# CarbonMatrixLab/AbX

Hardware: AMD Instinct MI355X
Metric: diffusion-steps/sec (100 samples, ~350-res complex) (higher is better)
Workload: dtype f32; 1 GPU; L352: L=352 (Lab 228 + antigen 124), 100 samples of one complex over 1 GPU(s), 1 step = ScoreNetwork (3 passes) + get_prev + reverse, seeded random weights, ESM off; L=352, samples_total=100, chunk=auto, parallelism=sample-shard x1, no collective in the step

## Files before the change

abx_amd/_lib.py:

```python
import ctypes as C
import os

_HERE = os.path.dirname(os.path.abspath(__file__))
LIB_PATH = os.environ.get('ABX_HIP_LIB') or os.path.join(_HERE, 'csrc', 'libabx_hip.so')

c_f = C.c_void_p
LL = C.c_longlong
I = C.c_int
F = C.c_float


class AbxGemm(C.Structure):
    _fields_ = [
        ('A', c_f), ('sAb', LL), ('sAm', LL), ('sAk', LL),
        ('B', c_f), ('sBb', LL), ('sBk', LL), ('sBn', LL),
        ('C', c_f), ('sCb', LL), ('sCm', LL),
        ('M', I), ('N', I), ('K', I), ('batch', I),
        ('c_transposed', I),
        ('ln_stats', c_f), ('sSb', LL),
        ('ln_csum', c_f),
        ('ln_eps', F),
        ('a_relu', I),
        ('bias', c_f),
        ('alpha', F),
        ('act', I),
        ('rowscale', c_f), ('sRSb', LL),
        ('gate', c_f), ('sGb', LL), ('sGm', LL), ('gate_sigmoid', I),
        ('resid', c_f), ('sRb', LL), ('sRm', LL),
        ('B_split', C.c_void_p), ('sB3p', LL), ('sB3n', LL), ('sB3k', LL), ('sB3b', LL),
        ('A_split', C.c_void_p), ('sA3p', LL), ('sA3m', LL), ('sA3k', LL), ('sA3b', LL),
        ('batch_inner', I), ('sA3i', LL), ('sB3i', LL),
        ('c_split_tile', I),
        ('c_split_nA', I),
        ('C_split', C.c_void_p), ('sCp', LL), ('sCk', LL), ('c_split_L', I),
        ('glu', I),
        ('a_pair_transpose', I),
        ('pair_L', I), ('pair_Lp', I), ('a_pair', I), ('c_pair', I),
        ('A2', c_f), ('sA2b', LL), ('sA2m', LL), ('K2', I),
        ('B2_split', C.c_void_p), ('sB23p', LL), ('sB23n', LL), ('sB23k', LL),
        ('ln2_csum', c_f), ('bias2', c_f),
        ('mlp', I), ('N2', I),
        ('out_ln_w', c_f), ('out_ln_b', c_f), ('out_ln_eps', F),
        ('exact', I),
        ('b_f16', I), ('b_exp', I), ('b2_exp', I),
        ('tune', I),
        ('c_planes_from', I), ('c_planes_group', I),
        ('range_flag', c_f), ('range_tag', I),
        ('clock_probe', c_f),
        ('a_vec_ok', I), ('b_vec_ok', I), ('fast_ok', I),
        ('c_vec_ok', I), ('g_vec_ok', I), ('r_vec_ok', I), ('rs_vec_ok', I),
    ]


class AbxIpaTail(C.Structure):
    _fields_ = [
        ('feat', c_f), ('s_feat', LL),
        ('s', c_f), ('s_s', LL),
        ('M', I), ('K1', I), ('C', I),
        ('W_final', C.c_void_p), ('e_final', I), ('b_final', c_f),
        ('ln1_w', c_f), ('ln1_b', c_f),
        ('W_t0', C.c_void_p), ('e_t0', I), ('b_t0', c_f),
        ('W_t2', C.c_void_p), ('e_t2', I), ('b_t2', c_f),
        ('W_t4', C.c_void_p), ('e_t4', I), ('b_t4', c_f),
        ('ln2_w', c_f), ('ln2_b', c_f),
        ('ln_eps', F),
        ('W_aff', c_f), ('b_aff', c_f),
        ('fixed', c_f), ('init_q', c_f), ('init_t', c_f),
        ('cur_q', c_f), ('cur_t', c_f), ('cur_R', c_f), ('delta_q', c_f), ('pscale', F),
        ('range_flag', c_f), ('range_tag', I),
        ('partial', c_f), ('n_partial', I), ('s_partial', LL),
    ]


class AbxHeadsTail(C.Structure):
    _fields_ = [
        ('s', c_f), ('s_s', LL), ('s0', c_f), ('s_s0', LL), ('M', I),
        ('W_act', C.c_void_p), ('e_act', I), ('b_act', c_f),
        ('W_init', C.c_void_p), ('e_init', I), ('b_init', c_f),
        ('W_r0', C.c_void_p), ('e_r0', I), ('b_r0', c_f),
        ('W_r1', C.c_void_p), ('e_r1', I), ('b_r1', c_f),
        ('W_r2', C.c_void_p), ('e_r2', I), ('b_r2', c_f),
        ('W_r3', C.c_void_p), ('e_r3', I), ('b_r3', c_f),
        ('W_proj', C.c_void_p), ('e_proj', I), ('b_proj', c_f),
        ('un', c_f),
        ('lns_w', c_f), ('lns_b', c_f),
        ('W_s1', C.c_void_p), ('e_s1', I), ('b_s1', c_f),
        ('W_s3', C.c_void_p), ('e_s3', I), ('b_s3', c_f),
        ('W_s5', C.c_void_p), ('e_s5', I), ('b_s5', c_f),
        ('logits', c_f),
        ('lnp_w', c_f), ('lnp_b', c_f),
        ('W_p1', C.c_void_p), ('e_p1', I), ('b_p1', c_f),
        ('W_p3', C.c_void_p), ('e_p3', I), ('b_p3', c_f),
        ('W_p5', C.c_void_p), ('e_p5', I), ('b_p5', c_f),
        ('pl', c_f),
        ('ln_eps', F),
        ('range_flag', c_f), ('range_tag', I),
    ]


class AbxTriAttn(C.Structure):
    _fields_ = [
        ('q', c_f), ('k', c_f), ('v', c_f), ('gate', c_f),
        ('sb', LL), ('ss', LL), ('sl', LL),
# ... 180 lines not shown
    'abx_tri_rowpack_bytes': (LL, []),
    'abx_tri_rowpack': (I, [C.POINTER(AbxLinearPack), c_f, C.POINTER(AbxTriRowPack), _S]),
    'abx_tri_attn_rowfused_ok': (I, [I]),
    'abx_tri_attn_rowfused_fwd': (I, [C.POINTER(AbxTriAttn), c_f, LL, LL, LL, C.POINTER(AbxTriRowPack), I, _S]),
    'abx_seq_attn_fwd': (I, [c_f, c_f, c_f, c_f, c_f, I, I, I, I, F, _S]),
    'abx_ipa_pack': (I, [c_f, c_f, c_f, c_f, c_f, c_f, I, I, F, _S]),
    'abx_ipa_attn': (I, [c_f, c_f, c_f, c_f, c_f, c_f, c_f, c_f, c_f, c_f, c_f, I, I, _S]),
    'abx_debug_poison_lds': (I, [C.c_uint, _S]),
    'abx_ipa_weights': (I, [c_f, c_f, c_f, c_f, c_f, c_f, c_f, c_f, c_f, c_f, I, I, _S]),
    'abx_ipa_pair': (I, [c_f, c_f, c_f, I, I, _S]),
    'abx_ipa_attn_workspace_bytes': (C.c_longlong, [I, I]),
    'abx_ipa_qpack_bytes': (C.c_longlong, [I, I]),
    'abx_timestep_embedding': (I, [c_f, c_f, I, I, c_f, _S]),
    'abx_assemble_seq': (I, [c_f, LL, c_f, c_f, I, c_f, c_f, c_f, c_f, c_f, I, I, I, I, _S]),
    'abx_assemble_pair': (I, [c_f, LL, c_f, c_f, c_f, c_f, c_f, c_f, c_f, c_f, I, I, I, I, _S]),
    'abx_opm_features': (I, [c_f, c_f, LL, c_f, I, I, I, _S]),
    'abx_opm_out_fwd': (I, [c_f, LL, c_f, c_f, c_f, I, I, c_f, I, _S]),
    'abx_assemble_pair_bias': (I, [c_f, LL, c_f, c_f, c_f, c_f, c_f, c_f, c_f, C.c_void_p, I, c_f, c_f, F, c_f, I, I, c_f, I, _S]),
    'abx_pair_mask': (I, [c_f, c_f, I, I, I, _S]),
    'abx_transpose_last2': (I, [c_f, c_f, I, I, I, I, _S]),
    'abx_pair_embed_features': (I, [c_f, c_f, c_f, c_f, c_f, c_f, c_f, c_f, c_f, c_f, c_f, c_f, I, I, _S]),
    'abx_relpos_block': (I, [c_f, c_f, c_f, I, I, I, I, I, _S]),
    'abx_gather_rows': (I, [c_f, c_f, c_f, c_f, LL, LL, I, _S]),
    'abx_frames_init': (I, [c_f, I, c_f, c_f, c_f, c_f, c_f, c_f, I, F, _S]),
    'abx_rigid_update': (I, [c_f, c_f, c_f, c_f, c_f, c_f, c_f, c_f, I, F, _S]),
    'abx_scores': (I, [C.POINTER(AbxScoreArgs), _S]),
    'abx_torsion_finalize': (I, [c_f, c_f, c_f, c_f, I, _S]),
    'abx_seq_head_atoms': (I, [c_f, c_f, c_f, c_f, c_f, c_f, c_f, c_f, c_f, c_f, c_f, c_f, I, _S]),
    'abx_prev_pos': (I, [c_f, c_f, I, c_f, I, I, _S]),
    'abx_plddt': (I, [c_f, c_f, I, I, _S]),
    'abx_igso3_tables': (I, [c_f, c_f, I, I, I, c_f, c_f, c_f, _S]),
    'abx_reverse_step': (I, [C.POINTER(AbxReverseArgs), _S]),
    'abx_clash_grad_workspace_bytes': (LL, [I, I]),
    'abx_clash_grad': (I, [C.POINTER(AbxGuidanceArgs), c_f, _S]),
    'abx_design_scores_workspace_bytes': (LL, [I, I]),
    'abx_design_scores': (I, [C.POINTER(AbxDesignScoreArgs), c_f, _S]),
    'abx_relax_workspace_bytes': (LL, [I, I, I]),
    'abx_relax_lds_bytes': (LL, [I, I]),
    'abx_relax': (I, [C.POINTER(AbxRelaxArgs), c_f, _S]),
    'abx_interface_scores_workspace_bytes': (LL, [I, I, I]),
    'abx_interface_scores': (I, [C.POINTER(AbxInterfaceArgs), c_f, _S]),
    'abx_ensemble_pairs_workspace_bytes': (LL, [I, I]),
    'abx_ensemble_pairs': (I, [C.POINTER(AbxEnsemblePairsArgs), c_f, _S]),
    'abx_ensemble_cluster': (I, [C.POINTER(AbxEnsembleClusterArgs), _S]),
    'abx_pack_linear_bytes': (LL, [I, I]),
    'abx_pack_linear': (I, [C.POINTER(AbxLinearSrc), I, I, c_f, c_f, I, c_f, C.POINTER(AbxLinearPack), _S]),
    'abx_transition_workspace_bytes': (LL, [LL, I, I]),
    'abx_transition_fwd': (I, [C.POINTER(AbxLinearPack), C.POINTER(AbxLinearPack), c_f, LL, I, c_f, c_f, I, _S]),
    'abx_tri_mul_workspace_bytes': (LL, [I, I]),
    'abx_tri_mul_workspace_init': (I, [c_f, I, I, _S]),
    'abx_tri_mul_fwd': (I, [C.POINTER(AbxTriMulPack), c_f, c_f, c_f, I, I, I, c_f, c_f, I, _S]),
    'abx_tri_attn_block_workspace_bytes': (LL, [I, I]),
    'abx_tri_attn_block_fwd': (I, [C.POINTER(AbxTriAttnPack), c_f, c_f, I, I, I, I, c_f, c_f, I, _S]),
}

EXPORTED = tuple(_PROTOS)
_lib = None


class AbxHipError(RuntimeError):
    pass


def library_path():
    return LIB_PATH


def load():
    global _lib
    if _lib is not None:
        return _lib
    if not os.path.exists(LIB_PATH):
        raise AbxHipError(f'{LIB_PATH} not found: build it with `make -C abx_amd/csrc` (no CPU fallback exists)')
    lib = C.CDLL(LIB_PATH)
    for name, (res, args) in _PROTOS.items():
        fn = getattr(lib, name)
        fn.restype = res
        fn.argtypes = args
    if lib.abx_version() != 1:
        raise AbxHipError('libabx_hip ABI version mismatch')
    _lib = lib
    return lib


def check(rc, what):
    if rc != 0:
        msg = load().abx_last_error_string()
        raise AbxHipError(f'{what} failed (rc={rc}): {msg.decode() if msg else ""}')
```

abx_amd/csrc/blocks.hip:

```cpp
#include <math.h>
#include <string.h>

#include <stdlib.h>

#include "common.h"
#include "abx_hip.h"

namespace {

constexpr long long ALIGN = 256;
inline long long up(long long x) { return (x + ALIGN - 1) / ALIGN * ALIGN; }

__global__ void pack_rows_kernel(const float* __restrict__ W, const float* __restrict__ b, int rows, int K, int c0, int glu,
                                 float* __restrict__ Wcat, float* __restrict__ bcat) {
    const long long idx = (long long)blockIdx.x * blockDim.x + threadIdx.x;
    if (idx >= (long long)rows * K) return;
    const int r = (int)(idx / K), k = (int)(idx - (long long)r * K);
    const int c = c0 + r;
    const int dst = glu ? (c / 32) * 64 + (glu == 2 ? 32 : 0) + c % 32 : c;
    Wcat[(long long)dst * K + k] = W[idx];
    if (k == 0) bcat[dst] = b ? b[r] : 0.f;
}

__global__ void fold_kernel(const float* __restrict__ Wcat, const float* __restrict__ bcat, const float* __restrict__ gamma,
                            const float* __restrict__ beta, int N, int K, float* __restrict__ Wt, float* __restrict__ csum,
                            float* __restrict__ bias, unsigned* __restrict__ amax) {
    const int n = blockIdx.x * blockDim.x + threadIdx.x;
    if (n >= N) return;
    double cs = 0.0, bs = 0.0;
    float mx = 0.f;
    bool bad = false;
    for (int k = 0; k < K; ++k) {
        const double w = (double)Wcat[(long long)n * K + k];
        const double ws = gamma ? (double)gamma[k] * w : w;
        const float wf = (float)ws;
        Wt[(long long)k * N + n] = wf;
        cs += ws;
        if (beta) bs += (double)beta[k] * w;
        mx = fmaxf(mx, fabsf(wf));
        bad |= !(fabsf(wf) <= 3.0e38f);
    }
    csum[n] = (float)cs;
    bias[n] = (float)(bs + (double)bcat[n]);
    atomicMax(amax, bad ? 0x7f800000u : __float_as_uint(mx));
}

__global__ void permute_k16_kernel(const float* __restrict__ Wt, int K, int N, float* __restrict__ out) {
    const long long idx = (long long)blockIdx.x * blockDim.x + threadIdx.x;
    if (idx >= (long long)K * N) return;
    const int k = (int)(idx / N), n = (int)(idx - (long long)k * N);
    const int j = k & 15;
    const int src = (k & ~15) | ((j & 3) | ((j & 4) << 1) | ((j & 8) >> 1));
    out[idx] = Wt[(long long)src * N + n];
}

inline void set_weights(AbxGemm& g, const AbxLinearPack& p, bool ln, int exact) {
    g.B = p.Wt; g.sBb = 0; g.sBk = p.N; g.sBn = 1;
    g.N = p.N; g.K = p.K;
    g.bias = p.bias;
    if (ln) { g.ln_csum = p.csum; g.ln_eps = 1e-5f; }
    g.B_split = p.planes; g.sB3k = 2LL * p.N * 16; g.sB3p = (long long)p.N * 16; g.sB3n = 16; g.sB3b = 0;
    g.b_f16 = 1; g.b_exp = p.b_exp;
    g.exact = exact ? 1 : 2;
    g.alpha = 1.0f;
}
inline void set_range(AbxGemm& g, int* flag, int tag, int exact) {
    if (!exact) { g.range_flag = flag; g.range_tag = tag; }
}

}

extern "C" long long abx_pack_linear_bytes(int K, int N) {
    if (K <= 0 || N <= 0) return -1;
    const long long Kp = (K + 15) / 16 * 16;
    return up(4LL * K * N) + 2 * up(4LL * N) + up(2LL * Kp * 2 * N) + up(4LL * K * N) + up(4LL * N) + up(4);
}

extern "C" int abx_pack_linear(const AbxLinearSrc* src, int nsrc, int K, const float* gamma, const float* beta, int flags, void* buf,
                               AbxLinearPack* out, hipStream_t st) {
    ABX_REQUIRE(src && nsrc > 0 && nsrc <= 8 && K > 0 && buf && out, "abx_pack_linear: bad args");
    ABX_REQUIRE((reinterpret_cast<uintptr_t>(buf) & (ALIGN - 1)) == 0, "abx_pack_linear: buf must be 256-byte aligned");
    ABX_REQUIRE((gamma == nullptr) == (beta == nullptr), "abx_pack_linear: gamma and beta come together");
    int N = 0, nv = 0, ng = 0;
    bool any_b = false;
    for (int i = 0; i < nsrc; ++i) {
        ABX_REQUIRE(src[i].W && src[i].rows > 0 && src[i].glu >= 0 && src[i].glu <= 2, "abx_pack_linear: bad source");
        N += src[i].rows;
        nv += src[i].glu == 1 ? src[i].rows : 0;
        ng += src[i].glu == 2 ? src[i].rows : 0;
        any_b |= src[i].b != nullptr;
    }
    ABX_REQUIRE((nv == 0 && ng == 0) || (nv == ng && nv + ng == N && nv % 32 == 0),
                "abx_pack_linear: glu sources need as many value as gate rows, in multiples of 32, and nothing else");
    ABX_REQUIRE(!(flags & ABX_PACK_PERMUTE_K16) || K % 16 == 0, "abx_pack_linear: ABX_PACK_PERMUTE_K16 needs K % 16 == 0");
    const long long Kp = (K + 15) / 16 * 16;
    char* p = static_cast<char*>(buf);
    float* Wt = reinterpret_cast<float*>(p); p += up(4LL * K * N);
    float* csum = reinterpret_cast<float*>(p); p += up(4LL * N);
    float* bias = reinterpret_cast<float*>(p); p += up(4LL * N);
    unsigned short* planes = reinterpret_cast<unsigned short*>(p); p += up(2LL * Kp * 2 * N);
    float* Wcat = reinterpret_cast<float*>(p); p += up(4LL * K * N);
    float* bcat = reinterpret_cast<float*>(p); p += up(4LL * N);
    unsigned* amax = reinterpret_cast<unsigned*>(p);
    int cv = 0, cg = 0, c0 = 0;
    for (int i = 0; i < nsrc; ++i) {
        const long long tot = (long long)src[i].rows * K;
        const int base = src[i].glu == 1 ? cv : (src[i].glu == 2 ? cg : c0);
        hipLaunchKernelGGL(pack_rows_kernel, dim3((unsigned)((tot + 255) / 256)), dim3(256), 0, st, src[i].W, src[i].b, src[i].rows, K, base,
                           src[i].glu, Wcat, bcat);
        (src[i].glu == 1 ? cv : (src[i].glu == 2 ? cg : c0)) += src[i].rows;
    }
    if (hipMemsetAsync(amax, 0, 4, st) != hipSuccess) { abx_set_error("abx_pack_linear: memset failed"); return ABX_ERR_ARG; }
    hipLaunchKernelGGL(fold_kernel, dim3((N + 63) / 64), dim3(64), 0, st, Wcat, bcat, gamma, beta, N, K, Wt, csum, bias, amax);
    if (int rc = abx_check_launch("abx_pack_linear")) return rc;
    unsigned bits = 0;
    if (hipMemcpyAsync(&bits, amax, 4, hipMemcpyDeviceToHost, st) != hipSuccess || hipStreamSynchronize(st) != hipSuccess) {
        abx_set_error("abx_pack_linear: reading max |w| failed");
        return ABX_ERR_ARG;
    }
    float mx;
    memcpy(&mx, &bits, 4);
// ... 38 lines not shown
        g.mlp = 1; g.N2 = C; g.b2_exp = l2->b_exp;
        g.B2_split = l2->planes; g.sB23k = 2LL * C * 16; g.sB23p = (long long)C * 16; g.sB23n = 16;
        g.bias2 = l2->bias;
        g.resid = z; g.sRm = C;
        set_range(g, range_flag, range_tag, 0);
        return abx_gemm(&g, st);
    }
    ABX_REQUIRE(workspace, "abx_transition_fwd: the exact path needs its workspace (abx_transition_workspace_bytes)");
    float* hid = static_cast<float*>(workspace);
    AbxGemm g = {};
    g.A = z; g.sAm = C; g.sAk = 1;
    g.C = hid; g.sCm = Hd;
    g.M = (int)M; g.batch = 1;
    set_weights(g, *l1, true, 1);
    g.act = 1;
    if (int rc = abx_gemm(&g, st)) return rc;
    AbxGemm h = {};
    h.A = hid; h.sAm = Hd; h.sAk = 1;
    h.C = z; h.sCm = C;
    h.M = (int)M; h.batch = 1;
    set_weights(h, *l2, false, 1);
    h.B_split = nullptr; h.b_f16 = 0;
    h.resid = z; h.sRm = C;
    return abx_gemm(&h, st);
}

namespace {
struct TriMulWs { unsigned short* lrp; float* pm; float* tt; long long lrp_bytes; };
inline TriMulWs tri_mul_ws(void* ws, int B, int L) {
    const long long Lp = (L + 3) / 4 * 4, KT = (Lp + 15) / 16;
    TriMulWs w;
    char* p = static_cast<char*>(ws);
    w.lrp_bytes = 2LL * B * 256 * KT * 2 * L * 16;
    w.lrp = reinterpret_cast<unsigned short*>(p); p += up(w.lrp_bytes);
    w.pm = reinterpret_cast<float*>(p); p += up(4LL * B * L * Lp);
    w.tt = reinterpret_cast<float*>(p);
    return w;
}
}

extern "C" long long abx_tri_mul_workspace_bytes(int B, int L) {
    if (B <= 0 || L <= 0) return -1;
    const long long Lp = (L + 3) / 4 * 4, KT = (Lp + 15) / 16;
    return up(2LL * B * 256 * KT * 2 * L * 16) + up(4LL * B * L * Lp) + up(4LL * B * 128 * L * Lp);
}

extern "C" int abx_tri_mul_workspace_init(void* workspace, int B, int L, hipStream_t st) {
    ABX_REQUIRE(workspace && B > 0 && L > 0, "abx_tri_mul_workspace_init: bad args");
    const TriMulWs w = tri_mul_ws(workspace, B, L);
    if (hipMemsetAsync(w.lrp, 0, (size_t)w.lrp_bytes, st) != hipSuccess) { abx_set_error("abx_tri_mul_workspace_init: memset failed"); return ABX_ERR_ARG; }
    return ABX_OK;
}

extern "C" int abx_tri_mul_fwd(const AbxTriMulPack* wp, const float* z_in, float* z_out, const float* mask, int B, int L, int outgoing,
                               void* workspace, int* range_flag, int range_tag, hipStream_t st) {
    ABX_REQUIRE(wp && z_in && z_out && z_in != z_out && mask && workspace && B > 0 && L > 0, "abx_tri_mul_fwd: bad args (z_out must not alias z_in)");
    const AbxLinearPack &glu = wp->glu, &out = wp->out, &gate = wp->gate;
    ABX_REQUIRE(glu.csum && out.csum && gate.csum && glu.N == 512 && out.K == 128 && gate.K == glu.K && out.N == gate.N && glu.K == out.N,
                "abx_tri_mul_fwd: packs: glu = LN-folded C -> 2 x 256 (value, gate) pairs, out = LN-folded 128 -> C, gate = LN-folded C -> C");
    const int C = glu.K;
    const long long LL = (long long)L * L;
    const int Lp = (L + 3) / 4 * 4, KT = (Lp + 15) / 16;
    const long long LLp = (long long)L * Lp;
    const TriMulWs w = tri_mul_ws(workspace, B, L);
    if (int rc = abx_pair_mask(mask, w.pm, B, L, Lp, st)) return rc;
    {
        AbxGemm g = {};
        g.A = z_in; g.sAb = LL * C; g.sAm = C; g.sAk = 1;
        g.M = (int)(((long long)(L + 7) / 8 * 8) * ((long long)(Lp + 15) / 16 * 16));
        g.batch = B;
        set_weights(g, glu, true, 0);
        g.C_split = w.lrp; g.sCb = 256LL * KT * 2 * L * 16; g.sCm = (long long)KT * 2 * L * 16; g.sCk = 2LL * L * 16; g.sCp = (long long)L * 16;
        g.c_split_L = Lp; g.c_transposed = 1; g.c_split_nA = 128; g.c_split_tile = 1;
        g.pair_L = L; g.pair_Lp = Lp; g.a_pair = 1; g.a_pair_transpose = outgoing ? 0 : L;
        g.glu = 1;
        g.rowscale = w.pm; g.sRSb = LLp;
        set_range(g, range_flag, range_tag, 0);
        if (int rc = abx_gemm(&g, st)) return rc;
    }
    {
        AbxGemm g = {};
        const long long per_ch = (long long)KT * 2 * L * 16;
        g.A_split = w.lrp; g.sA3b = 256 * per_ch; g.sA3i = per_ch; g.sA3k = 2LL * L * 16; g.sA3p = (long long)L * 16; g.sA3m = 16;
        g.B_split = w.lrp + 128 * per_ch; g.sB3b = 256 * per_ch; g.sB3i = per_ch; g.sB3k = 2LL * L * 16; g.sB3p = (long long)L * 16; g.sB3n = 16;
        g.batch_inner = 128;
        g.C = w.tt; g.sCb = LLp; g.sCm = Lp;
        g.M = L; g.N = L; g.K = KT * 16; g.batch = B * 128;
        g.exact = 2; g.alpha = 1.0f;
        set_range(g, range_flag, range_tag, 0);
        if (int rc = abx_gemm(&g, st)) return rc;
    }
    {
        AbxGemm g = {};
        g.A = w.tt; g.sAb = 128 * LLp; g.sAm = 1; g.sAk = LLp;
        g.M = (int)LLp; g.batch = B;
        set_weights(g, out, true, 0);
        g.C = z_out; g.sCb = LL * C; g.sCm = C;
        if (Lp != L) { g.pair_L = L; g.pair_Lp = Lp; g.c_pair = 1; }
        g.A2 = z_in; g.sA2b = LL * C; g.sA2m = C; g.K2 = C;
        g.B2_split = gate.planes; g.sB23k = 2LL * gate.N * 16; g.sB23p = (long long)gate.N * 16; g.sB23n = 16; g.b2_exp = gate.b_exp;
        g.ln2_csum = gate.csum; g.bias2 = gate.bias;
        g.resid = z_in; g.sRb = LL * C; g.sRm = C;
        set_range(g, range_flag, range_tag, 0);
        return abx_gemm(&g, st);
    }
}

namespace {
struct TriAttnWs { float* qkv; float* hid; float* bT; float* bT2; float* o; };
inline TriAttnWs tri_attn_ws(void* ws, int B, int L) {
    const long long LL = (long long)L * L, Lp = (L + 3) / 4 * 4;
    TriAttnWs w;
    char* p = static_cast<char*>(ws);
    w.qkv = reinterpret_cast<float*>(p);
    w.hid = w.qkv + (long long)B * LL * 576;
    p += up(4LL * B * LL * 768);
    w.bT = reinterpret_cast<float*>(p); p += up(4LL * B * 4 * LL);
    w.bT2 = reinterpret_cast<float*>(p); p += up(4LL * B * 4 * L * Lp);
    w.o = reinterpret_cast<float*>(p);
    return w;
}
}

extern "C" long long abx_tri_attn_block_workspace_bytes(int B, int L) {
    if (B <= 0 || L <= 0) return -1;
    const long long LL = (long long)L * L, Lp = (L + 3) / 4 * 4;
    return up(4LL * B * LL * 768) + up(4LL * B * 4 * LL) + up(4LL * B * 4 * L * Lp) + up(4LL * B * LL * 192);
}

extern "C" int abx_tri_attn_block_fwd(const AbxTriAttnPack* wp, float* z, const float* mask, int B, int L, int per_row, int exact,
                                      void* workspace, int* range_flag, int range_tag, hipStream_t st) {
    ABX_REQUIRE(wp && z && mask && workspace && B > 0 && L > 0, "abx_tri_attn_block_fwd: bad args");
    const AbxLinearPack &qkv = wp->qkv, &gate = wp->gate, &pair = wp->pair, &out = wp->out;
    ABX_REQUIRE(qkv.csum && gate.csum && pair.csum && qkv.N == 576 && gate.N == 192 && pair.N == 4 && qkv.K == 192 && gate.K == 192 && pair.K == 192 &&
                    out.K == 192 && out.N == 192,
                "abx_tri_attn_block_fwd: packs: qkv = LN-folded 192 -> 576, gate = LN-folded 192 -> 192, pair = LN-folded 192 -> 4, out = 192 -> 192 "
                "(ABX_PACK_PERMUTE_K16)");
    const long long LL = (long long)L * L, M2 = (long long)B * LL;
    ABX_REQUIRE(M2 < (1LL << 31), "abx_tri_attn_block_fwd: too many pair rows for one launch");
    ABX_REQUIRE(exact >= 0 && exact <= 3, "abx_tri_attn_block_fwd: exact is a 2-bit field");
    const int attn_exact = (exact >> 1) & 1;
    exact &= 1;
    const int Lp = (L + 3) / 4 * 4, C = 192;
    const TriAttnWs w = tri_attn_ws(workspace, B, L);
    static const bool kv_planes_on = getenv("ABX_KV_PLANES") != nullptr;
    const int planes = (kv_planes_on && !exact && !attn_exact && abx_gemm_planes_ok(M2)) ? 1 : 0;
    const bool rowfused = !exact && !attn_exact && !planes && wp->row.planes && abx_tri_attn_rowfused_ok(L);
    if (rowfused) {
        AbxGemm s2 = {};
        s2.A = z; s2.sAb = LL * C; s2.sAm = C; s2.sAk = 1;
        s2.C = w.bT; s2.sCb = 4 * LL; s2.sCm = LL; s2.c_transposed = 1;
        s2.M = (int)LL; s2.batch = B;
        set_weights(s2, pair, true, 0);
        set_range(s2, range_flag, range_tag, 0);
        s2.alpha = ABX_TRI_BIAS_LOG2;
        if (int rc = abx_gemm(&s2, st)) return rc;
    } else {
        AbxGemm g = {};
        g.A = z; g.sAm = C; g.sAk = 1;
        g.C = w.qkv; g.sCm = 576;
        g.M = (int)M2; g.batch = 1;
        set_weights(g, qkv, true, exact);
        set_range(g, range_flag, range_tag, exact);
        if (planes) { g.c_planes_from = 192; g.c_planes_group = 48; }
        AbxGemm s2 = {};
        s2.A = z; s2.sAb = LL * C; s2.sAm = C; s2.sAk = 1;
        s2.C = w.bT; s2.sCb = 4 * LL; s2.sCm = LL; s2.c_transposed = 1;
        s2.M = (int)LL; s2.batch = B;
        set_weights(s2, pair, true, exact);
        set_range(s2, range_flag, range_tag, exact);
        if (!attn_exact) s2.alpha = ABX_TRI_BIAS_LOG2;
        if (int rc = abx_gemm_side(&g, &s2, st)) return rc;
    }
    const float* bias = w.bT;
    if (!per_row || Lp != L) {
        if (int rc = abx_transpose_last2(w.bT, w.bT2, B * 4, L, Lp, per_row ? 0 : 1, st)) return rc;
        bias = w.bT2;
    }
    {
        AbxTriAttn a = {};
        a.q = w.qkv; a.k = w.qkv + 192; a.v = w.qkv + 384; a.gate = nullptr;
        a.sb = LL * 576;
        a.ss = per_row ? (long long)L * 576 : 576;
        a.sl = per_row ? 576 : (long long)L * 576;
        a.bias = bias; a.bias_sb = 4LL * L * Lp; a.bias_sh = (long long)L * Lp; a.bias_sq = Lp; a.bias_sk = 1;
        a.keymask = mask; a.km_sb = L;
        a.out = w.o; a.ob = LL * C;
        a.os = per_row ? (long long)L * C : C;
        a.ol = per_row ? C : (long long)L * C;
        a.B = B; a.S = L; a.L = L; a.H = 4; a.D = 48;
        a.scale = 0.14433756729740643f;
        a.exact = attn_exact;
        a.bias_log2 = attn_exact ? 0 : 1;
        a.kv_planes = planes;
        if (!attn_exact) { a.range_flag = range_flag; a.range_tag = range_tag; }
        if (rowfused) {
            if (int rc = abx_tri_attn_rowfused_fwd(&a, z, LL * C, per_row ? (long long)L * C : C, per_row ? C : (long long)L * C, &wp->row, -1, st)) return rc;
        } else if (int rc = abx_tri_attn_fwd(&a, st)) return rc;
    }
    if (!exact) {
        AbxGemm g = {};
        g.A = z; g.sAm = C; g.sAk = 1;
        g.C = z; g.sCm = C;
        g.M = (int)M2; g.batch = 1;
        set_weights(g, gate, true, 0);
        g.act = 2;
        g.gate = w.o; g.sGm = C;
        g.mlp = 2; g.N2 = C; g.b2_exp = out.b_exp;
        g.B2_split = out.planes; g.sB23k = 2LL * C * 16; g.sB23p = (long long)C * 16; g.sB23n = 16;
        g.bias2 = out.bias;
        g.resid = z; g.sRm = C;
        set_range(g, range_flag, range_tag, 0);
        return abx_gemm(&g, st);
    }
    {
        AbxGemm g = {};
        g.A = z; g.sAm = C; g.sAk = 1;
        g.C = w.hid; g.sCm = C;
        g.M = (int)M2; g.batch = 1;
        set_weights(g, gate, true, 1);
        g.act = 2;
        g.gate = w.o; g.sGm = C; g.gate_sigmoid = 0;
        if (int rc = abx_gemm(&g, st)) return rc;
    }
    {
        AbxGemm g = {};
        g.A = w.hid; g.sAm = C; g.sAk = 1;
        g.C = z; g.sCm = C;
        g.M = (int)M2; g.batch = 1;
        set_weights(g, out, false, 1);
        g.B_split = nullptr; g.b_f16 = 0;
        g.resid = z; g.sRm = C;
        return abx_gemm(&g, st);
    }
}
```

abx_amd/csrc/gemm.hip:

```cpp
#include <stdlib.h>
#include "common.h"
#include "abx_hip.h"
#include "gemm_epilogue.h"

int abx_gemm3_dispatch(const AbxGemm& g, hipStream_t st, int* rc);

namespace {

template <int BMN, int BK, bool KC, bool EDGE>
struct TileLoader {
    static constexpr int NVEC = BMN * BK / 4;
    static constexpr int NV = (NVEC + 255) / 256;
    static constexpr int LD = BMN + 4;
    f32x4 v[NV];

    __device__ __forceinline__ void load(const float* __restrict__ base, long long s_mn, long long s_k, int mn0, int k0,
                                         int MN, int K, bool vec_ok) {
        const int tid = threadIdx.x;
#pragma unroll
        for (int i = 0; i < NV; ++i) {
            const int idx = tid + i * 256;
            f32x4 r = {0.f, 0.f, 0.f, 0.f};
            if (NVEC % 256 == 0 || idx < NVEC) {
                if (KC) {
// ... 397 lines not shown
    ABX_REQUIRE(!on[A_SPLIT] || (!g.ln_csum && !g.a_relu), "abx_gemm: a_split (plane x plane contraction) takes no LayerNorm and no relu-on-load");
    return ABX_OK;
}

static int gemm_prepare(const AbxGemm* gp, AbxGemm& g) {
    if (int rc = abx_gemm_check_modes(gp)) return rc;
    g = *gp;
    ABX_REQUIRE((g.A || g.A_split) && (g.B || g.B_split) && (g.C || g.C_split), "abx_gemm: null operand");
    ABX_REQUIRE(!g.glu || (g.c_transposed && g.N % 128 == 0 && !g.gate), "abx_gemm: glu needs a transposed store, N % 128 == 0, no gate");
    const long long tile_rows = ((long long)(g.pair_L + 7) / 8 * 8) * ((long long)(g.pair_Lp + 15) / 16 * 16);
    ABX_REQUIRE(!g.c_split_tile || (g.C_split && g.a_pair && g.pair_Lp > 0 && g.M == tile_rows && !g.gate && !g.resid),
                "abx_gemm: c_split_tile needs C_split, a_pair, pair_L / pair_Lp, M == ceil8(pair_L) * ceil16(pair_Lp), no gate / resid");
    ABX_REQUIRE(!g.C_split || (g.c_transposed && g.c_split_L > 0 && g.c_split_L % 4 == 0 && (g.c_split_tile || g.M % g.c_split_L == 0)),
                "abx_gemm: C_split needs the transposed store of a (padded) pair tensor (M = rows * c_split_L, c_split_L % 4 == 0)");
    ABX_REQUIRE(g.M > 0 && g.N > 0 && g.K > 0 && g.batch > 0, "abx_gemm: empty problem");
    ABX_REQUIRE(g.pair_Lp == 0 || (g.pair_L > 0 && g.pair_Lp >= g.pair_L && g.pair_Lp % 4 == 0 &&
                                   (g.c_split_tile || g.M == (long long)g.pair_L * g.pair_Lp) && (!g.C_split || g.c_split_L == g.pair_Lp)),
                "abx_gemm: padded pair rows need M == pair_L * pair_Lp, pair_Lp % 4 == 0 (and c_split_L == pair_Lp)");
    ABX_REQUIRE((!g.a_pair && !g.c_pair) || g.pair_Lp > 0, "abx_gemm: a_pair / c_pair need pair_L / pair_Lp");
    ABX_REQUIRE(!g.A || g.sAk == 1 || g.sAm == 1, "abx_gemm: A must be k- or m-contiguous");
    ABX_REQUIRE(!g.B || g.sBn == 1 || g.sBk == 1, "abx_gemm: B must be n- or k-contiguous");
    ABX_REQUIRE(!g.ln_stats || g.ln_csum, "abx_gemm: LayerNorm needs the column sums of the gamma-scaled weights");
    ABX_REQUIRE(!(g.ln_csum && g.a_relu), "abx_gemm: LayerNorm and relu-on-load are exclusive");
    if (g.ln_csum && !g.ln_stats && g.ln_eps <= 0.f) g.ln_eps = 1e-5f;
    if (g.out_ln_w && g.out_ln_eps <= 0.f) g.out_ln_eps = 1e-5f;
    const bool akc = g.sAk == 1;
    auto al16 = [](const void* p) { return (reinterpret_cast<uintptr_t>(p) & 15) == 0; };
    g.a_vec_ok = al16(g.A) && (g.sAb % 4 == 0) && (akc ? (g.sAm % 4 == 0) : (g.sAk % 4 == 0));
    g.b_vec_ok = al16(g.B) && (g.sBb % 4 == 0) && (g.sBn == 1 ? (g.sBk % 4 == 0) : (g.sBn % 4 == 0));
    g.fast_ok = g.a_vec_ok && g.b_vec_ok;
    g.c_vec_ok = g.C_split ? ((reinterpret_cast<uintptr_t>(g.C_split) & 7) == 0 && g.sCb % 4 == 0 && g.sCm % 4 == 0 && g.sCp % 4 == 0)
                           : (al16(g.C) && (g.sCb % 4 == 0) && (g.sCm % 4 == 0));
    g.g_vec_ok = g.gate && al16(g.gate) && (g.sGb % 4 == 0) && (g.sGm % 4 == 0);
    g.r_vec_ok = g.resid && al16(g.resid) && (g.sRb % 4 == 0) && (g.sRm % 4 == 0);
    g.rs_vec_ok = g.rowscale && al16(g.rowscale) && (g.sRSb % 4 == 0);
    ABX_REQUIRE(g.c_planes_from == 0 || (g.c_planes_from > 0 && g.c_planes_from % 4 == 0 && g.c_planes_group > 0 && g.c_planes_group % 4 == 0 &&
                                         g.N % 4 == 0 && g.c_planes_from < g.N && (g.N - g.c_planes_from) % g.c_planes_group == 0 && g.C && g.c_vec_ok &&
                                         !g.c_transposed && !g.C_split && !g.glu && !g.gate && !g.resid && !g.mlp && !g.A2 && !g.out_ln_w && !g.c_pair &&
                                         g.act == 0 && g.exact != 1),
                "abx_gemm: c_planes_from needs a plain, 16-byte aligned fp32 store without gate / resid / activation on the split-f16 path, from, "
                "group and N multiples of 4, (N - from) % group == 0");
    return ABX_OK;
}

int abx_gemm3_side_dispatch(const AbxGemm& g, const AbxGemm& s2, hipStream_t st, int* rc);
int abx_gemm_as_dispatch(const AbxGemm& g, const AbxGemm* side, hipStream_t st, int* rc);

extern "C" int abx_gemm_planes_ok(long long M) {
    static const bool off = getenv("ABX_NO_GEMM_AS") != nullptr || getenv("ABX_NO_GEMM_SIDE") != nullptr;
    return (!off && (M + 63) / 64 >= 1024) ? 1 : 0;
}

extern "C" int abx_gemm_side(const AbxGemm* main_gemm, const AbxGemm* side_gemm, hipStream_t st) {
    ABX_REQUIRE(main_gemm && side_gemm, "abx_gemm_side: null descriptor");
    AbxGemm g, s2;
    if (int rc = gemm_prepare(main_gemm, g)) return rc;
    if (int rc = gemm_prepare(side_gemm, s2)) return rc;
    int rc = 0;
    static const bool off = getenv("ABX_NO_GEMM_SIDE") != nullptr;
    if (!off && !abx_gemm_as_dispatch(g, &s2, st, &rc)) return rc;
    ABX_REQUIRE(g.c_planes_from == 0, "abx_gemm_side: c_planes_from is served by the A-stationary kernel only (>= 65 536 rows, K = 192, N % 128 == 64, "
                                      "planes in groups of 48 from a multiple of 32, a side projection): ask abx_gemm_planes_ok first");
    if (!off && !abx_gemm3_side_dispatch(g, s2, st, &rc)) return rc;
    if (int r1 = abx_gemm(main_gemm, st)) return r1;
    return abx_gemm(side_gemm, st);
}

extern "C" int abx_gemm(const AbxGemm* gp, hipStream_t st) {
    AbxGemm g;
    if (int rc = gemm_prepare(gp, g)) return rc;
    ABX_REQUIRE(g.c_planes_from == 0, "abx_gemm: c_planes_from is served through abx_gemm_side by the A-stationary kernel only (abx_gemm_planes_ok)");
    auto al16 = [](const void* p) { return (reinterpret_cast<uintptr_t>(p) & 15) == 0; };
    (void)al16;
    const bool akc = g.sAk == 1;
    if (g.exact != 1) {
        int rc = 0;
        if (!abx_gemm_as_dispatch(g, nullptr, st, &rc)) return rc;
        if (!abx_gemm3_dispatch(g, st, &rc)) return rc;
    }
    g.range_flag = nullptr;
    ABX_REQUIRE(g.A && g.B, "abx_gemm: split-f16 operands given but the problem does not qualify for the split kernels "
                            "(K % 16, alignment, size) and no fp32 operands were passed for the exact kernel");
    ABX_REQUIRE(g.a_pair_transpose <= 0 && g.pair_Lp == 0, "abx_gemm: pair-row remapping is served by the split-f16 kernels only");
    ABX_REQUIRE(g.batch <= 65535, "abx_gemm: batch > 65535 (exact fp32 kernels)");
    ABX_REQUIRE(!g.glu, "abx_gemm: glu is served by the split-f16 kernels only (large problems, K % 16 == 0)");
    ABX_REQUIRE(!g.A2, "abx_gemm: the dual GEMM is served by the split-f16 kernels only");
    ABX_REQUIRE(!g.out_ln_w, "abx_gemm: out_ln is served by the split-f16 kernels only");
    ABX_REQUIRE(!g.mlp, "abx_gemm: the fused transition (mlp) is served by the split-f16 kernels only (exact = 2, K % 16 == 0)");
    const long long mt128 = ((long long)g.M + 127) / 128;
    if (g.N <= 32) return launch_cfg<128, 32, 32, 32>(g, st);
    if (g.N <= 64) return launch_cfg<128, 64, 32, 64>(g, st);
    if (mt128 * (((long long)g.N + 127) / 128) * g.batch < 512) return launch_cfg<64, 64, 32, 32>(g, st);
    if (g.tune >> 1) {
        ABX_REQUIRE(!g.c_transposed && akc && g.sBn == 1, "abx_gemm: tuning variants exist for the plain weight GEMM only");
        switch (g.tune >> 1) {
            case 1: return launch_main_variant<16, 2>(g, st);
            case 2: return launch_main_variant<16, 4>(g, st);
            case 3: return launch_cfg<128, 128, 64, 64, 16, 3>(g, st);
            default: break;
        }
    }
    const long long pad128 = ((g.N + 127) / 128) * 128, pad192 = ((g.N + 191) / 192) * 192;
    if (pad192 <= pad128 && !(g.tune >> 1)) return launch_cfg<128, 192, 64, 96, 16, 2>(g, st);
    return launch_cfg<128, 128, 64, 64>(g, st);
}

extern "C" int abx_row_stats(const float* x, long long s_b, long long s_row, long long s_k, int batch, int rows, int K,
                             float eps, float* stats, hipStream_t st) {
    ABX_REQUIRE(x && stats && rows > 0 && K > 0 && batch > 0, "abx_row_stats: bad args");
    if (s_k == 1) {
        ABX_REQUIRE(batch == 1 || s_b == (long long)rows * s_row, "abx_row_stats: k-contiguous rows must be dense over batch");
        const long long total = (long long)batch * rows;
        hipLaunchKernelGGL(row_stats_kc, dim3((unsigned)((total + 3) / 4)), dim3(256), 0, st, x, s_row, (int)total, K, eps, stats);
    } else {
        ABX_REQUIRE(s_row == 1, "abx_row_stats: rows must be contiguous when k is strided");
        hipLaunchKernelGGL(row_stats_mc, dim3((unsigned)((rows + 255) / 256), (unsigned)batch), dim3(256), 0, st, x, s_b, s_k,
                           rows, K, eps, stats);
    }
    return abx_check_launch("abx_row_stats");
}

extern "C" int abx_layernorm(const float* x, long long s_row, long long rows, int K, const float* gamma, const float* beta,
                             float eps, float* out, long long s_out, const float* res, long long s_res, hipStream_t st) {
    ABX_REQUIRE(x && out && gamma && beta && rows > 0 && K > 0, "abx_layernorm: bad args");
    auto al16v = [](const void* p) { return (reinterpret_cast<uintptr_t>(p) & 15) == 0; };
    if (K == 128 && s_row % 4 == 0 && s_out % 4 == 0 && al16v(x) && al16v(out) && al16v(gamma) && al16v(beta) &&
        (!res || (al16v(res) && s_res % 4 == 0))) {
// ... 9 lines not shown
```

abx_amd/csrc/gemm3.hip:

```cpp
#include "common.h"
#include "abx_hip.h"
#include "gemm_epilogue.h"
#include "rigid_dev.h"

namespace {

constexpr int BK = 16;
#ifndef ABX_SPLIT_MIN_TILES
#define ABX_SPLIT_MIN_TILES 256
#endif
typedef __attribute__((address_space(3))) void* lds_ptr_t;
typedef const __attribute__((address_space(1))) void* glb_ptr_t;

__device__ __forceinline__ void glds16(const void* src, char* dst_wave_base) {
    __builtin_amdgcn_global_load_lds((glb_ptr_t)src, (lds_ptr_t)dst_wave_base, 16, 0, 0);
}

__device__ __forceinline__ unsigned vgpr32(unsigned o) {
    asm volatile("" : "+v"(o));
    return o;
}

template <int N> __device__ __forceinline__ void wait_vm_and_barrier() {
    asm volatile("s_waitcnt vmcnt(%0) lgkmcnt(0)\n\ts_barrier" ::"n"(N) : "memory");
// ... 750 lines not shown
                }
                const char* ws = W2s + (kg & 1) * B2_IMG + offB2;
                if (rows_live && kg * 16 < g.N) {
#pragma unroll
                    for (int t0 = 0; t0 < TN2; t0 += TG2) {
                        u32x4 wb[TG2][2];
#pragma unroll
                        for (int t = 0; t < TG2; ++t)
#pragma unroll
                            for (int p = 0; p < 2; ++p) wb[t][p] = *reinterpret_cast<const u32x4*>(ws + (t0 + t) * 1024 + p * (BN2 * 32));
                        constexpr int TA[3] = {1, 0, 0}, TB[3] = {0, 1, 0};
#pragma unroll
                        for (int term = 0; term < 3; ++term)
#pragma unroll
                            for (int t = 0; t < TG2; ++t)
                                acc2[0][t0 + t] = mfma_split(hf[TA[term]], wb[t][TB[term]], acc2[0][t0 + t]);
                    }
                }
                if (kl + 1 < KC && (kg + 1) * 16 < g.N) wait_vm_and_barrier<2>();
                else wait_vm_and_barrier<0>();
            }
        }
    }
    {
        const float cs2 = __builtin_ldexpf(1.0f, -4 - g.b2_exp);
#pragma unroll
        for (int t = 0; t < TN2; ++t) acc2[0][t] *= cs2;
    }
    AbxGemm g2 = g;
    g2.N = g.N2; g2.bias = g.bias2; g2.ln_csum = nullptr; g2.ln_stats = nullptr; g2.act = 0; g2.alpha = 1.0f; g2.gate = nullptr;
    __syncthreads();
    gemm_epilogue<BM, BN2, WM, BN2, EDGE, false>(g2, smem, smem + 2 * BM, acc2, mt * BM, 0, b, false);
}

constexpr int GT_LDS = 2 * 128 * 64 + 2 * 2 * 96 * 32 + 2 * 2 * 192 * 32 + 3 * 128 * 64 + 2 * GT_NG * 4;

__global__ __launch_bounds__(256, 2) void gemm3_gtail2w_kernel(const AbxGemm g) {
    extern __shared__ __attribute__((aligned(16))) float gt_smem[];
    const int ntm = (g.M + 127) / 128;
    const unsigned nwg = gridDim.x, bid = blockIdx.x;
    const unsigned q = nwg >> 3, r = nwg & 7, xcd = bid & 7, loc = bid >> 3;
    const unsigned wgid = (xcd < r ? xcd * (q + 1) : r * (q + 1) + (xcd - r) * q) + loc;
    const int b = (int)(wgid / (unsigned)ntm), mt = (int)(wgid - (unsigned)b * (unsigned)ntm);
    const ClockProbe probe(g.clock_probe);
    if ((mt + 1) * 128 <= g.M && g.N2 == 192) gemm3_gtail2w_block<false>(g, gt_smem, mt, b);
    else gemm3_gtail2w_block<true>(g, gt_smem, mt, b);
    probe.finish();
}

constexpr int GT1_G1 = 2 * 128 * 64 + 2 * 2 * 192 * 32;
constexpr int GT1_W2 = 2 * 96 * 32;
constexpr int GT1_OFF_G = GT1_G1, GT1_OFF_W2 = GT1_OFF_G + 3 * 128 * 64, GT1_OFF_CST = GT1_OFF_W2 + 2 * GT1_W2;
constexpr int GT1_LDS = GT1_OFF_CST + 2 * GT_NG * 4;
template <bool EDGE>
__device__ __forceinline__ void gemm3_gtail_block(const AbxGemm& g, float* smem, int mt, int b) {
    constexpr int BM = 128, BN = 192, WM = 32, BH = 96, TH = BH / 32, NKT = BN / 16;
    char* lds = reinterpret_cast<char*>(smem);
    char* Gs = lds + GT1_OFF_G;
    char* W2s = lds + GT1_OFF_W2;
    float* cst = reinterpret_cast<float*>(lds + GT1_OFF_CST);
    for (int i = threadIdx.x; i < GT_NG; i += 256) {
        cst[i] = i < g.N ? g.ln_csum[i] : 0.f;
        cst[GT_NG + i] = (i < g.N && g.bias) ? g.bias[i] : 0.f;
    }
    const int lane = threadIdx.x & 63, wave = __builtin_amdgcn_readfirstlane(threadIdx.x >> 6), h = lane >> 5;
    const int m0 = mt * BM;
    unsigned offs2[2][2];
#pragma unroll
    for (int half = 0; half < 2; ++half) plane_sources<BH, 2>(g.sB23p, g.sB23n, half * BH, g.N2, offs2[half]);
    const char* base2 = reinterpret_cast<const char*>(g.B2_split);
    const long long step2 = g.sB23k * 2;
    auto issue_w2 = [&](int half, int ktile) {
        if (wave == 3) return;
        char* dst = W2s + (ktile & 1) * GT1_W2 + wave * 2048;
        const char* src = base2 + ktile * step2;
#pragma unroll
        for (int i = 0; i < 2; ++i) glds16(src + vgpr32(offs2[half][i]), dst + i * 1024);
    };
    unsigned offsG[2];
    const char* baseG = reinterpret_cast<const char*>(g.gate + (long long)b * g.sGb + (long long)m0 * g.sGm);
#pragma unroll
    for (int i = 0; i < 2; ++i) {
        const int r = (wave * 2 + i) * 16 + (lane >> 2), p = lane & 3;
        const int kq = p ^ ((r >> 2) & 3);
        const int gri = min(m0 + r, g.M - 1) - m0;
        offsG[i] = (unsigned)(((long long)gri * g.sGm + kq * 4) * 4);
    }
    const int nkt2 = g.N / 16;
    auto issue_g = [&](int ktile) {
        const int kt = min(ktile, nkt2 - 1);
        char* dg = Gs + (ktile % 3) * (BM * 64) + wave * 2048;
        const char* sg = baseG + kt * 64;
#pragma unroll
        for (int i = 0; i < 2; ++i) glds16(sg + vgpr32(offsG[i]), dg + i * 1024);
    };
    const int offB2 = plane_off<BH>(0, lane & 31, h);
    const int grow = wave * WM + (lane & 31), gx = (grow >> 2) & 3;
    const int offG0 = grow * 64 + ((h ^ gx) << 4), offG1 = grow * 64 + (((2 + h) ^ gx) << 4);
    const bool rows_live = m0 + wave * WM < g.M;

    issue_w2(0, 0);
    issue_g(0);
    issue_g(1);
    float ls[1], lq[1], lsh[1] = {0.f};
    f32x16 acc1[1][BN / 32];
    gemm3_mainloop<BM, BN, WM, BN, 0, true, true>(g, smem, mt, 0, b, acc1, ls, lq, lsh);
    const float invK = 1.0f / (float)g.K;
    const float sm = ls[0] + __shfl_xor(ls[0], 32, 64), sq = lq[0] + __shfl_xor(lq[0], 32, 64);
    const float dmean = sm * invK;
    const float rstd = 1.0f / sqrtf(fmaxf(sq * invK - dmean * dmean, 0.f) + g.ln_eps);

    AbxGemm g2 = g;
    g2.N = g.N2; g2.bias = g.bias2; g2.ln_csum = nullptr; g2.ln_stats = nullptr; g2.act = 0; g2.alpha = 1.0f; g2.gate = nullptr;
    const float cs2 = __builtin_ldexpf(1.0f, -4 - g.b2_exp);
    u32x4 hfa[NKT][2];
    constexpr int TA[3] = {1, 0, 0}, TB[3] = {0, 1, 0};
#pragma unroll
    for (int half = 0; half < 2; ++half) {
        f32x16 acc2[1][TH];
#pragma unroll
        for (int t = 0; t < TH; ++t)
#pragma unroll
            for (int r = 0; r < 16; ++r) acc2[0][t][r] = 0.f;
        if (half == 1) issue_w2(1, 0);
#pragma unroll
        for (int kg = 0; kg < NKT; ++kg) {
            const bool more = (kg + 1) * 16 < g.N && kg + 1 < NKT;
            if (half == 1 && kg == 0) wait_vm_and_barrier<0>();
            if (more) {
                issue_w2(half, kg + 1);
                if (half == 0) issue_g(kg + 2);
            }
            if (half == 0) {
                const int j = kg >> 1, s2 = kg & 1;
                const char* gs = Gs + (kg % 3) * (BM * 64);
                const f32x4 o0 = *reinterpret_cast<const f32x4*>(gs + offG0), o1 = *reinterpret_cast<const f32x4*>(gs + offG1);
                float v[8];
#pragma unroll
                for (int q = 0; q < 2; ++q) {
                    const int hc = j * 32 + 8 * (2 * s2 + q) + 4 * h;
                    const int hcl = min(hc, GT_NG - 4);
                    const f32x4 cs = *reinterpret_cast<const f32x4*>(cst + hcl), bi = *reinterpret_cast<const f32x4*>(cst + GT_NG + hcl);
                    const f32x4 ov = q ? o1 : o0;
#pragma unroll
                    for (int e = 0; e < 4; ++e) {
                        const float x = rstd * (acc1[0][j][8 * s2 + 4 * q + e] - dmean * cs[e]) + bi[e];
                        v[4 * q + e] = (hc + e < g.N) ? ov[e] * sigmoidf_(x) : 0.f;
                    }
                }
                unsigned q0[4], q1[4];
#pragma unroll
                for (int e = 0; e < 4; ++e) split2b(v[2 * e], v[2 * e + 1], q0[e], q1[e]);
                hfa[kg][0] = u32x4{q0[0], q0[1], q0[2], q0[3]};
                hfa[kg][1] = u32x4{q1[0], q1[1], q1[2], q1[3]};
            }
            const char* ws = W2s + (kg & 1) * GT1_W2 + offB2;
            if (rows_live && kg * 16 < g.N) {
                u32x4 wb[TH][2];
#pragma unroll
                for (int t = 0; t < TH; ++t)
#pragma unroll
                    for (int p = 0; p < 2; ++p) wb[t][p] = *reinterpret_cast<const u32x4*>(ws + t * 1024 + p * (BH * 32));
#pragma unroll
                for (int term = 0; term < 3; ++term)
#pragma unroll
                    for (int t = 0; t < TH; ++t) acc2[0][t] = mfma_split(hfa[kg][TA[term]], wb[t][TB[term]], acc2[0][t]);
            }
            if (more && half == 0) wait_vm_and_barrier<2>();
            else wait_vm_and_barrier<0>();
        }
#pragma unroll
        for (int t = 0; t < TH; ++t) acc2[0][t] *= cs2;
        gemm_epilogue<BM, BH, WM, BH, EDGE, false>(g2, smem, smem + 2 * BM, acc2, m0, half * BH, b, false);
        if (half == 0) __syncthreads();
    }
}

__global__ __launch_bounds__(256, 2) void gemm3_gtail_kernel(const AbxGemm g) {
    extern __shared__ __attribute__((aligned(16))) float gt_smem[];
    const int ntm = (g.M + 127) / 128;
    const unsigned nwg = gridDim.x, bid = blockIdx.x;
    const unsigned q = nwg >> 3, r = nwg & 7, xcd = bid & 7, loc = bid >> 3;
    const unsigned wgid = (xcd < r ? xcd * (q + 1) : r * (q + 1) + (xcd - r) * q) + loc;
    const int b = (int)(wgid / (unsigned)ntm), mt = (int)(wgid - (unsigned)b * (unsigned)ntm);
    const ClockProbe probe(g.clock_probe);
    if ((mt + 1) * 128 <= g.M && g.N2 == 192 && g.N == 192) gemm3_gtail_block<false>(g, gt_smem, mt, b);
    else gemm3_gtail_block<true>(g, gt_smem, mt, b);
    probe.finish();
}

constexpr int IT_C = 256;
constexpr int IT_ASTR = IT_C * 4 + 16;
constexpr int IT_RING = 4;
constexpr int IT_OPER = IT_RING * (4096 + 2 * IT_C * 32);
constexpr int IT_LDS = IT_OPER + 2 * 32 * IT_ASTR + 2 * 4 * 32 * 4;

__global__ __launch_bounds__(256, 1) void ipa_tail_kernel(const AbxIpaTail a) {
    constexpr int BM = 32, BN = IT_C, WM = 32, WN = 64, TN = 2;
    extern __shared__ __attribute__((aligned(16))) float it_smem[];
    char* lds = reinterpret_cast<char*>(it_smem);
    char* act[2] = {lds + IT_OPER, lds + IT_OPER + 32 * IT_ASTR};
    float* red = reinterpret_cast<float*>(lds + IT_OPER + 2 * 32 * IT_ASTR);
    const int mt = blockIdx.x, m0 = mt * BM;
    const int lane = threadIdx.x & 63, wave = threadIdx.x >> 6, h = lane >> 5, row = lane & 31;
    const int grc = min(m0 + row, a.M - 1);
    const int colb = wave * WN + 4 * h;

    AbxGemm g = {};
    g.M = a.M; g.N = IT_C; g.batch = 1; g.b_f16 = 1;
    g.sB3k = 2 * IT_C * 16; g.sB3p = IT_C * 16; g.sB3n = 16;
    f32x16 acc[1][TN];
    float ls[1], lq[1], lsh[1];
    float x[TN][16];

    auto for_groups = [&](auto&& fn) {
#pragma unroll
        for (int j = 0; j < TN; ++j)
#pragma unroll
            for (int q = 0; q < 4; ++q) fn(j, q, colb + j * 32 + 8 * q);
    };
    auto layer_norm = [&](const float* gamma, const float* beta) {
        float sm = 0.f;
#pragma unroll
        for (int j = 0; j < TN; ++j)
#pragma unroll
            for (int r = 0; r < 16; ++r) sm += x[j][r];
        sm += __shfl_xor(sm, 32, 64);
        if (h == 0) red[wave * 32 + row] = sm;
// ... 232 lines not shown
            bias_to(br[2 * blk + 1], false, true, x);
            to_lds(T1, HT_HSTR, x);
            __syncthreads();
        }
    }
    run(a.W_proj, a.e_proj, HT_H, T1, HT_HSTR, 1);
    bias_to(a.b_proj, false, false, y);
    store_cols(a.un, 14, y);
    layer_norm_s(a.lns_w, a.lns_b);
    __syncthreads();
    head(a.W_s1, a.e_s1, a.b_s1, a.W_s3, a.e_s3, a.b_s3, a.W_s5, a.e_s5, a.b_s5, a.logits, 20);
    if (a.W_p1) {
        layer_norm_s(a.lnp_w, a.lnp_b);
        __syncthreads();
        head(a.W_p1, a.e_p1, a.b_p1, a.W_p3, a.e_p3, a.b_p3, a.W_p5, a.e_p5, a.b_p5, a.pl, 50);
    }
    if (a.range_flag && __any(bad) && lane == 0) atomicOr(a.range_flag, a.range_tag);
}

template <int BM, int BN, int WM, int WN, int MINW>
int launch3(const AbxGemm& g, hipStream_t st) {
    const long long mt = ((long long)g.M + BM - 1) / BM, ntn = ((long long)g.N + BN - 1) / BN;
    dim3 grid((unsigned)(mt * ntn * g.batch), 1, 1), block(256);
#ifdef ABX_PERSIST
    if ((g.tune & 256) && grid.x > 256u * MINW) grid.x = 256u * MINW;
#endif
    const int amode = g.A_split ? 2 : (g.sAk == 1 ? 0 : 1);
    if (g.c_transposed) {
        if (amode != 0) { abx_set_error("abx_gemm: transposed store needs a k-contiguous fp32 A"); return ABX_ERR_ARG; }
        hipLaunchKernelGGL((gemm3_kernel<BM, BN, WM, WN, 0, true, MINW>), grid, block, 0, st, g);
    } else if (amode == 0) hipLaunchKernelGGL((gemm3_kernel<BM, BN, WM, WN, 0, false, MINW>), grid, block, 0, st, g);
    else if (amode == 1) hipLaunchKernelGGL((gemm3_kernel<BM, BN, WM, WN, 1, false, MINW>), grid, block, 0, st, g);
    else hipLaunchKernelGGL((gemm3_kernel<BM, BN, WM, WN, 2, false, MINW>), grid, block, 0, st, g);
    return abx_check_launch("abx_gemm");
}

__global__ __launch_bounds__(256) void split_weights_f16_kernel(const float* __restrict__ w, long long s_n, long long s_k, int N, int K,
                                                                int Kp, float scale, unsigned short* __restrict__ out) {
    const long long idx = (long long)blockIdx.x * 256 + threadIdx.x;
    if (idx >= (long long)N * Kp) return;
    const int n = (int)(idx / Kp), k = (int)(idx % Kp);
    const float x = k < K ? w[n * s_n + k * s_k] * scale : 0.f;
    const _Float16 h0 = (_Float16)x;
    const _Float16 h1 = (_Float16)(x - (float)h0);
    const long long o = ((long long)(k >> 4) * 2 * N + n) * 16 + (k & 15);
    out[o] = __builtin_bit_cast(unsigned short, h0);
    out[o + (long long)N * 16] = __builtin_bit_cast(unsigned short, h1);
}

}

int abx_gemm3_dispatch(const AbxGemm& g, hipStream_t st, int* rc) {
    auto al16 = [](const void* p) { return (reinterpret_cast<uintptr_t>(p) & 15) == 0; };
    const bool narrow = g.B_split && g.N <= 32 && !g.A_split && g.sAk == 1 && !g.glu && !g.C_split && !g.A2 && !g.out_ln_w &&
                        g.a_pair_transpose <= 0 && g.pair_Lp == 0;
    if (!g.B_split || g.K % 16 != 0 || (g.N <= 64 && !narrow)) return 1;
    if ((g.A_split != nullptr) == (g.b_f16 != 0) || g.b_exp < -100 || g.b_exp > 100 || g.b2_exp < -100 || g.b2_exp > 100) {
        abx_set_error("abx_gemm: B_split must be float16 weight planes (abx_split_weights_f16, b_f16 = 1, |b_exp| <= 100) with an fp32 A "
                      "and activation images (b_f16 = 0) with A_split");
        *rc = ABX_ERR_ARG;
        return 0;
    }
    const long long mt128 = ((long long)g.M + 127) / 128;
    if (g.exact != 2 && mt128 * (((long long)g.N + 127) / 128) * g.batch < ABX_SPLIT_MIN_TILES) return 1;
    if (!al16(g.B_split) || g.sB3n % 8 != 0 || g.sB3p % 8 != 0 || g.sB3b % 8 != 0 || g.sB3k % 8 != 0) return 1;
    if (g.A_split) {
        if (!al16(g.A_split) || g.sA3m % 8 != 0 || g.sA3p % 8 != 0 || g.sA3b % 8 != 0 || g.sA3k % 8 != 0 || g.c_transposed) return 1;
        if (g.batch_inner > 0 && (g.sA3i % 8 != 0 || g.sB3i % 8 != 0)) return 1;
    } else if (g.sAk == 1) {
        if (!al16(g.A) || g.sAm % 4 != 0 || g.sAb % 4 != 0) return 1;
        if (g.a_pair_transpose > 0 && !g.a_pair && (long long)g.a_pair_transpose * g.a_pair_transpose != g.M) return 1;
    } else {
        if (!al16(g.A) || g.sAk % 4 != 0 || g.sAb % 4 != 0 || g.M % 4 != 0 || g.M < 4 || g.a_pair_transpose > 0) return 1;
    }
    if (!g.A_split && g.sAk == 1 && ((g.a_pair_transpose > 0 || g.a_pair) ? (long long)g.M * g.sAm : 128LL * g.sAm) >= (1LL << 30)) return 1;
    if (g.pair_Lp > 0 && g.c_pair && g.c_transposed) return 1;
    if (g.a_pair && (g.A_split || g.sAk != 1)) return 1;
    if (!g.A_split && g.sAk != 1 && 16LL * g.sAk + g.M >= (1LL << 30)) return 1;
    if (((long long)g.M + 127) / 128 * (((long long)g.N + 127) / 128) * g.batch >= (1LL << 31)) return 1;
    if (g.A_split && (long long)(g.K / 16) * g.sA3k >= (1LL << 31)) return 1;
    if ((long long)(g.K / 16) * g.sB3k >= (1LL << 31)) return 1;
    if (g.out_ln_w) {
        if (g.N > 128 || g.c_transposed || g.C_split || g.A2 || g.A_split || g.sAk != 1 || !g.out_ln_b) {
            abx_set_error("abx_gemm: out_ln needs N <= 128, a k-contiguous fp32 A and a plain store (split-f16 path)");
            *rc = ABX_ERR_ARG;
            return 0;
        }
        const long long mt = ((long long)g.M + 127) / 128;
        hipLaunchKernelGGL((gemm3_oln_kernel<128, 128, 32, 128, 4>), dim3((unsigned)(mt * g.batch)), dim3(256), 0, st, g);
        *rc = abx_check_launch("abx_gemm(out_ln)");
        return 0;
    }
    if (g.mlp == 2) {
        if (g.A_split || g.sAk != 1 || g.c_transposed || g.C_split || g.glu || g.A2 || g.out_ln_w || !g.B2_split || g.N2 <= 0 || g.N2 > 192 ||
            g.N % 16 != 0 || g.N > GT_NG || g.act != 2 || g.alpha != 1.0f || g.rowscale || !g.gate || !g.ln_csum || g.ln_stats || g.a_relu ||
            g.a_pair_transpose > 0 || g.pair_Lp > 0 || !al16(g.B2_split) || g.sB23n % 8 != 0 || g.sB23p % 8 != 0 || g.sB23k % 8 != 0 ||
            (long long)(g.N / 16) * g.sB23k >= (1LL << 31) || !al16(g.ln_csum) || (g.bias && !al16(g.bias)) || !al16(g.gate) || g.sGm % 4 != 0 ||
            g.sGb % 4 != 0 || 128LL * g.sGm >= (1LL << 30)) {
            abx_set_error("abx_gemm: mlp = 2 (gated tail) needs a k-contiguous fp32 A with folded LayerNorm, act = 2, a 16-byte aligned gate "
                          "operand [M][N], N % 16 == 0, N2 <= 192, plain store, B2_split planes in the permuted k order");
            *rc = ABX_ERR_ARG;
            return 0;
        }
        const long long mt = ((long long)g.M + 127) / 128;
        if (g.tune & 64) {
            if (int e = abx_ensure_dynamic_lds(reinterpret_cast<const void*>(&gemm3_gtail2w_kernel), GT_LDS, "abx_gemm(gated tail)")) { *rc = e; return 0; }
            hipLaunchKernelGGL(gemm3_gtail2w_kernel, dim3((unsigned)(mt * g.batch)), dim3(256), GT_LDS, st, g);
            *rc = abx_check_launch("abx_gemm(gated tail, two walks)");
            return 0;
        }
        if (int e = abx_ensure_dynamic_lds(reinterpret_cast<const void*>(&gemm3_gtail_kernel), GT1_LDS, "abx_gemm(gated tail)")) { *rc = e; return 0; }
        hipLaunchKernelGGL(gemm3_gtail_kernel, dim3((unsigned)(mt * g.batch)), dim3(256), GT1_LDS, st, g);
        *rc = abx_check_launch("abx_gemm(gated tail)");
        return 0;
    }
    if (g.mlp) {
        if (g.A_split || g.sAk != 1 || g.c_transposed || g.C_split || g.glu || g.A2 || g.out_ln_w || !g.B2_split || g.N2 <= 0 || g.N2 > 192 ||
            g.N % 16 != 0 || g.N > MLP_NH || g.act != 1 || g.alpha != 1.0f || g.rowscale || g.gate || !g.ln_csum || g.ln_stats || g.a_relu ||
            g.a_pair_transpose > 0 || g.pair_Lp > 0 || !al16(g.B2_split) || g.sB23n % 8 != 0 || g.sB23p % 8 != 0 || g.sB23k % 8 != 0 ||
            (long long)(g.N / 16) * g.sB23k >= (1LL << 31) || !al16(g.ln_csum) || (g.bias && !al16(g.bias))) {
            abx_set_error("abx_gemm: mlp needs a k-contiguous fp32 A with folded LayerNorm, relu, N % 16 == 0, N <= 768, N2 <= 192, plain store, "
                          "B2_split planes in the permuted k order");
            *rc = ABX_ERR_ARG;
            return 0;
        }
        const long long mt = ((long long)g.M + 127) / 128;
        if ((g.tune >> 5) & 1) {
            if (int e = abx_ensure_dynamic_lds(reinterpret_cast<const void*>(&gemm3_mlp3_kernel), MLP3_LDS, "abx_gemm(mlp)")) { *rc = e; return 0; }
            hipLaunchKernelGGL(gemm3_mlp3_kernel, dim3((unsigned)(mt * g.batch)), dim3(256), MLP3_LDS, st, g);
        } else if ((g.tune >> 4) & 1) hipLaunchKernelGGL(gemm3_mlp_kernel<1>, dim3((unsigned)(mt * g.batch)), dim3(256), 0, st, g);
        else hipLaunchKernelGGL(gemm3_mlp_kernel<2>, dim3((unsigned)(mt * g.batch)), dim3(256), 0, st, g);
        *rc = abx_check_launch("abx_gemm(mlp)");
        return 0;
    }
    if (g.A2) {
        if (g.A_split || g.c_transposed || g.glu || !g.B2_split || g.K2 % 16 != 0 || !al16(g.A2) || g.sA2m % 4 != 0 || g.sA2b % 4 != 0 ||
            !al16(g.B2_split) || g.sB23n % 8 != 0 || g.sB23p % 8 != 0 || g.sB23k % 8 != 0 || !g.ln2_csum ||
            (g.pair_Lp > 0 ? (long long)g.pair_L * g.pair_L * g.sA2m : 128LL * g.sA2m) >= (1LL << 30) ||
            (long long)(g.K2 / 16) * g.sB23k >= (1LL << 31)) {
            abx_set_error("abx_gemm: dual (A2 / B2_split) operands do not qualify for the split-f16 dual kernel");
            *rc = ABX_ERR_ARG;
            return 0;
        }
        const long long mt = ((long long)g.M + 127) / 128, ntn = ((long long)g.N + 95) / 96;
        if (g.N > 96 && g.N <= 192 && (g.tune & 128)) hipLaunchKernelGGL(gemm3_dual1_kernel, dim3((unsigned)(mt * g.batch)), dim3(256), 0, st, g);
        else if (g.tune & 1024) hipLaunchKernelGGL((gemm3_dual_kernel<128, 96, 32, 96, 4>), dim3((unsigned)(mt * ntn * g.batch)), dim3(256), 0, st, g);
        else hipLaunchKernelGGL((gemm3_dual_kernel<128, 96, 32, 96, 3>), dim3((unsigned)(mt * ntn * g.batch)), dim3(256), 0, st, g);
        *rc = abx_check_launch("abx_gemm(dual)");
        return 0;
    }
    if (narrow) {
        const long long mt = ((long long)g.M + 127) / 128;
        dim3 grid((unsigned)(mt * g.batch), 1, 1), block(256);
        if ((g.tune >> 9) & 3) {
            const int v = (g.tune >> 9) & 3;
            if (g.c_transposed) { if (v == 1) hipLaunchKernelGGL((gemm3_narrow_ring_kernel<true, 3, 4>), grid, block, 0, st, g); else hipLaunchKernelGGL((gemm3_narrow_ring_kernel<true, 4, 3>), grid, block, 0, st, g); }
            else { if (v == 1) hipLaunchKernelGGL((gemm3_narrow_ring_kernel<false, 3, 4>), grid, block, 0, st, g); else hipLaunchKernelGGL((gemm3_narrow_ring_kernel<false, 4, 3>), grid, block, 0, st, g); }
            *rc = abx_check_launch("abx_gemm(narrow, ring)");
            return 0;
        }
        if (g.c_transposed) hipLaunchKernelGGL((gemm3_kernel<128, 32, 32, 32, 0, true, 6>), grid, block, 0, st, g);
// ... 102 lines not shown
```

abx_amd/csrc/gemm_as.hip:

```cpp
#include <stdlib.h>

#include <type_traits>

#include "common.h"
#include "abx_hip.h"

namespace {

typedef __attribute__((address_space(3))) void* lds_ptr_t;
typedef const __attribute__((address_space(1))) void* glb_ptr_t;

constexpr int AS_BM = 64, AS_BN = 128, AS_NK = 12, AS_RING = 3;
constexpr int AS_KT = 4096;
constexpr int AS_A = AS_NK * AS_KT;
constexpr int AS_STAGE = 2 * AS_BN * 32;
constexpr int AS_HALF = AS_KT / 2;
constexpr int AS_OFF_RING = AS_A;
constexpr int AS_OFF_ST = AS_OFF_RING + AS_RING * AS_STAGE;
constexpr int AS_OFF_CONST = AS_OFF_ST + 4 * 64 * 4;
constexpr int AS_LDS = AS_OFF_CONST + 2 * 1024;

__device__ __forceinline__ void as_glds16(const void* src, char* dst_wave_base) {
    __builtin_amdgcn_global_load_lds((glb_ptr_t)src, (lds_ptr_t)dst_wave_base, 16, 0, 0);
}
// ... 508 lines not shown
        else if (SIDE || !ragged || role == 0) {
            read_consts();
            if constexpr (EPI == AS_EPI_PLAIN) as_static_for<0, 8>([&](auto q_) { plain_slice(q_); });
            else {
                as_static_for<0, 4>([&](auto q_) { glu_value(q_); });
                as_static_for<0, 2>([&](auto q_) { glu_round(q_); });
            }
        }
    };
    if (wn == 0) walk(IC<0>{});
    else walk(IC<1>{});
    if (g.range_flag && __any(bad) && lane == 0) atomicOr(g.range_flag, g.range_tag);
#ifdef ABX_AS_STAMP
    if (g.clock_probe && threadIdx.x == 0) {
        asm volatile("s_waitcnt vmcnt(0)" ::: "memory");
        const unsigned long long t_end = __builtin_amdgcn_s_memtime();
        unsigned long long* rec = g.clock_probe + 16 + (size_t)blockIdx.x * 8;
        rec[0] = t_wait; rec[1] = t_walk1 - t_walk0; rec[2] = t_walk0 - t_begin; rec[3] = t_end - t_walk1;
        rec[4] = t_issued - t_begin; rec[5] = as_t_landed - t_issued; rec[6] = t_end - t_begin; rec[7] = 1ull;
    }
    if (g.clock_probe && threadIdx.x == 64) {
        unsigned long long* rec = g.clock_probe + 16 + ((size_t)gridDim.x + blockIdx.x) * 8;
        rec[0] = t_vm; rec[1] = t_bar; rec[7] = 1ull;
    }
#endif
}

template <int EPI, bool SIDE, int ABL = 0, bool PL = false>
__global__ __launch_bounds__(256, 2) void gemm_as_kernel(const AbxGemm g, const AbxGemm s2) {
    extern __shared__ __attribute__((aligned(16))) float as_smem[];
    char* lds = reinterpret_cast<char*>(as_smem);
    const ClockProbe probe(g.clock_probe);
    const unsigned ntm = (unsigned)((g.M + AS_BM - 1) / AS_BM);
    const unsigned nwg = gridDim.x, bid = blockIdx.x;
    const unsigned q = nwg >> 3, r = nwg & 7, xcd = bid & 7, loc = bid >> 3;
    const unsigned wgid = (xcd < r ? xcd * (q + 1) : r * (q + 1) + (xcd - r) * q) + loc;
    const int b = (int)(wgid / ntm), mt = (int)(wgid - (unsigned)b * ntm);
    bool edge = (mt + 1) * AS_BM > g.M;
    if (EPI == AS_EPI_GLU) edge = edge || (g.pair_L & 7) != 0 || (g.c_split_L & 15) != 0;
    if (edge) as_block<EPI, SIDE, true, ABL, PL>(g, s2, lds, mt, b);
    else as_block<EPI, SIDE, false, ABL, PL>(g, s2, lds, mt, b);
    probe.finish();
}


constexpr int AD_BN = 192, AD_NK2 = 12, AD_NK1 = 8, AD_NS = AD_NK2 + AD_NK1;
constexpr int AD_PLANE = AD_BN * 32;
constexpr int AD_STAGE = 2 * AD_PLANE;
constexpr int AD_OFF_RING = AS_A;
constexpr int AD_OFF_ST = AD_OFF_RING + 2 * AD_STAGE;
constexpr int AD_OFF_CONST = AD_OFF_ST + 4 * 64 * 4;
constexpr int AD_LDS = AD_OFF_CONST + 4 * AD_BN * 4;
static_assert(AD_LDS <= 81920, "two blocks per CU");
constexpr int AD_P0 = 4;
constexpr int ad_wslot(int t) { return t < 4 ? AD_OFF_RING + (t & 1) * AD_STAGE : ((t - 4) % 3 == 0 ? AD_OFF_RING : ((t - 4) % 3 == 1 ? 0 : AD_OFF_RING + AD_STAGE)); }

__device__ __forceinline__ void ad_issue_z(const AbxGemm& g, char* lds, int m0, int b, int wm) {
    const int lane = threadIdx.x & 63;
    const bool remap = g.pair_Lp > 0;
    const long long row0 = remap ? 0 : m0;
    const char* baseA = reinterpret_cast<const char*>(g.A2 + (long long)b * g.sA2b + row0 * g.sA2m);
    unsigned offA[2];
#pragma unroll
    for (int i = 0; i < 2; ++i) {
        const int r = 16 * i + (lane >> 2), p = lane & 3;
        const int kq = p ^ ((r >> 2) & 3);
        const int gri = min(m0 + wm * 32 + r, g.M - 1);
        long long gr = gri;
        if (remap) {
            const int pi = gri / g.pair_Lp, pj = min(gri - pi * g.pair_Lp, g.pair_L - 1);
            gr = (long long)pi * g.pair_L + pj;
        }
        offA[i] = (unsigned)(((gr - row0) * g.sA2m + kq * 4) * 4);
    }
    char* dst = lds + wm * AS_HALF;
#pragma unroll
    for (int kt = 0; kt < AD_NK2; ++kt)
#pragma unroll
        for (int i = 0; i < 2; ++i) as_glds16(baseA + kt * 64 + as_vgpr32(offA[i]), dst + kt * AS_KT + i * 1024);
}

template <bool FIRST>
__device__ __forceinline__ void ad_conv_ptile(AsConv& c, char* img) {
    const int lane = threadIdx.x & 63, r = lane & 31, h = lane >> 5;
    float xv[8];
#pragma unroll
    for (int e = 0; e < 8; ++e) xv[e] = *reinterpret_cast<const float*>(img + (8 * h + e) * 128 + r * 4);
    as_conv_values<FIRST>(c, xv, img);
}

__device__ __forceinline__ void ad_rendezvous(u32x4 (&fa)[2], u32x4 (&fb)[3][2]) {
    asm volatile("s_waitcnt lgkmcnt(0)\n\ts_barrier"
                 : "+v"(fa[0]), "+v"(fa[1]), "+v"(fb[0][0]), "+v"(fb[0][1]), "+v"(fb[1][0]), "+v"(fb[1][1]), "+v"(fb[2][0]), "+v"(fb[2][1])
                 :
                 : "memory");
}
template <int N>
__device__ __forceinline__ void ad_rendezvous_vm(u32x4 (&fa)[2], u32x4 (&fb)[3][2]) {
    asm volatile("s_waitcnt vmcnt(%8) lgkmcnt(0)\n\ts_barrier"
                 : "+v"(fa[0]), "+v"(fa[1]), "+v"(fb[0][0]), "+v"(fb[0][1]), "+v"(fb[1][0]), "+v"(fb[1][1]), "+v"(fb[2][0]), "+v"(fb[2][1])
                 : "n"(N)
                 : "memory");
}

template <bool EDGE>
__device__ __forceinline__ void as_dual_block(const AbxGemm& g, char* lds, int mt, int b) {
    const int lane = threadIdx.x & 63, wave = __builtin_amdgcn_readfirstlane(threadIdx.x >> 6);
    const int wm = wave >> 1, wn = wave & 1, h = lane >> 5;
    const int m0 = mt * AS_BM;
    float* st = reinterpret_cast<float*>(lds + AD_OFF_ST);
    const float* cc = reinterpret_cast<const float*>(lds + AD_OFF_CONST);

    const char* wbase2 = reinterpret_cast<const char*>(g.B2_split);
    const char* wbase1 = reinterpret_cast<const char*>(g.B_split + (long long)b * g.sB3b);
    const long long wk2 = g.sB23k * 2, wk1 = g.sB3k * 2;
    const unsigned wchunk2 = (unsigned)(32 * g.sB23n * 2), wchunk1 = (unsigned)(32 * g.sB3n * 2);
    unsigned woff2, woff1;
    {
        const int row = lane >> 1, half = (lane & 1) ^ ((row >> 3) & 1);
        woff2 = (unsigned)((wm * g.sB23p + (long long)row * g.sB23n + 8 * half) * 2);
        woff1 = (unsigned)((wm * g.sB3p + (long long)row * g.sB3n + 8 * half) * 2);
    }
    auto issue_w = [&](auto s_) __attribute__((always_inline)) {
        constexpr int s = decltype(s_)::value;
        char* dst = lds + ad_wslot(s) + wm * AD_PLANE;
        if constexpr (s < AD_NK2) {
            const char* src = wbase2 + s * wk2;
#pragma unroll
            for (int i = 0; i < 6; ++i) as_glds16(src + i * wchunk2 + as_vgpr32(woff2), dst + i * 1024);
        } else {
            const char* src = wbase1 + (s - AD_NK2) * wk1;
#pragma unroll
            for (int i = 0; i < 6; ++i) as_glds16(src + i * wchunk1 + as_vgpr32(woff1), dst + i * 1024);
        }
    };

    const char* pbase = reinterpret_cast<const char*>(g.A + (long long)b * g.sAb + m0);
    const long long pk = 16LL * g.sAk * 4;
    unsigned poff[2];
#pragma unroll
    for (int i = 0; i < 2; ++i) {
        const int kl = 8 * i + (lane >> 3);
        const int gm = min(m0 + wm * 32 + 4 * (lane & 7), g.M - 4) - m0;
        poff[i] = (unsigned)(((long long)kl * g.sAk + gm) * 4);
    }
    auto issue_p = [&](int kt) __attribute__((always_inline)) {
        char* dst = lds + (AD_P0 + kt) * AS_KT + wm * AS_HALF;
        const char* src = pbase + kt * pk;
#pragma unroll
        for (int i = 0; i < 2; ++i) as_glds16(src + as_vgpr32(poff[i]), dst + i * 1024);
    };

    const float cs2 = __builtin_ldexpf(1.0f, -ABX_F16_A_EXP - g.b2_exp), inv_cs2 = __builtin_ldexpf(1.0f, ABX_F16_A_EXP + g.b2_exp);
    const float cs1 = __builtin_ldexpf(1.0f, -ABX_F16_A_EXP - g.b_exp), inv_cs1 = __builtin_ldexpf(1.0f, ABX_F16_A_EXP + g.b_exp);
    AsConv cz, cp;
    char* a_half = lds + wm * AS_HALF;
    if (wn == 0) {
        ad_issue_z(g, lds, m0, b, wm);
        as_conv_init(cz, g);
        cz.ln = true;
        cz.relu = false;
        cp = cz;
        as_wait_vm<20>();
        as_conv_ktile<true>(cz, a_half);
        as_conv_ktile<false>(cz, a_half + AS_KT);
    } else {
        const float* c0 = wm ? g.ln_csum : g.ln2_csum;
        const float* c1 = wm ? g.bias : g.bias2;
#pragma unroll
        for (int a = 0; a < 2; ++a)
#pragma unroll
            for (int i = 0; i < 3; ++i) {
                char* dst = lds + AD_OFF_CONST + (2 * wm + a) * (AD_BN * 4) + i * 256;
                __builtin_amdgcn_global_load_lds((glb_ptr_t)((a ? c1 : c0) + i * 64 + lane), (lds_ptr_t)dst, 4, 0, 0);
            }
        issue_w(IC<0>{});
        issue_w(IC<1>{});
        as_wait_vm<6>();
    }
    __syncthreads();

    const int offAf = wm * AS_HALF + as_plane_off<32>(0, lane & 31, h);
    const int offBf = as_plane_off<AD_BN>(0, wn * 96 + (lane & 31), h);
    u32x4 fa[2][2], fb[2][3][2];
    auto read_frags = [&](int set, int kt, int wslot) __attribute__((always_inline)) {
#pragma unroll
        for (int p = 0; p < 2; ++p) fa[set][p] = *reinterpret_cast<const u32x4*>(lds + kt * AS_KT + offAf + p * 1024);
#pragma unroll
        for (int j = 0; j < 3; ++j)
#pragma unroll
            for (int p = 0; p < 2; ++p) fb[set][j][p] = *reinterpret_cast<const u32x4*>(lds + offBf + wslot + p * AD_PLANE + j * 1024);
    };

    f32x16 gatev[3], acc[3];
    const float* st_w = st + wm * 32 + 4 * h;
    auto gate_values = [&]() __attribute__((always_inline)) {
#pragma unroll
        for (int j = 0; j < 3; ++j) {
            const int n = wn * 96 + j * 32 + (lane & 31);
            const float csum2 = cc[n] * inv_cs2, bias2 = cc[AD_BN + n];
#pragma unroll
            for (int rq = 0; rq < 4; ++rq) {
                const f32x4 dm4 = *reinterpret_cast<const f32x4*>(st_w + 8 * rq), rs4 = *reinterpret_cast<const f32x4*>(st_w + 64 + 8 * rq);
#pragma unroll
                for (int c = 0; c < 4; ++c) {
                    const float gv = rs4[c] * (gatev[j][4 * rq + c] - dm4[c] * csum2) + bias2;
                    gatev[j][4 * rq + c] = sigmoidf_(gv);
                }
            }
        }
    };

    f32x4 rv[4][3];
    long long row_off_c[4];
    bool row_ok[4];
    auto load_resid = [&]() __attribute__((always_inline)) {
        const float* rd = g.resid + (long long)b * g.sRb;
#pragma unroll
        for (int rq = 0; rq < 4; ++rq) {
            const int m = m0 + wm * 32 + 8 * rq + 4 * h + (lane & 3);
            bool ok = !EDGE || m < g.M;
            long long mo = m;
            if (g.c_pair) {
                const int pi = m / g.pair_Lp, pj = m - pi * g.pair_Lp;
                ok = ok && pj < g.pair_L;
                mo = (long long)pi * g.pair_L + pj;
            }
            row_ok[rq] = ok;
            row_off_c[rq] = mo * g.sCm;
#pragma unroll
            for (int j = 0; j < 3; ++j) {
                const int n = wn * 96 + j * 32 + ((lane & 31) >> 2) * 4;
                rv[rq][j] = (f32x4){0.f, 0.f, 0.f, 0.f};
                if (ok) rv[rq][j] = *reinterpret_cast<const f32x4*>(rd + mo * g.sRm + n);
            }
        }
    };

    auto step = [&](auto s_, auto role_) __attribute__((always_inline)) {
        constexpr int s = decltype(s_)::value, role = decltype(role_)::value, set = s & 1;
        if constexpr (role == 0) ad_rendezvous(fa[set], fb[set]);
        else ad_rendezvous_vm<(s >= 3 && s + 2 < AD_NS) ? 6 : 0>(fa[set], fb[set]);
        if constexpr (role == 1) {
            if constexpr (s < 2) issue_w(IC<s + 2>{});
            else if constexpr (s == 2) { issue_w(IC<4>{}); issue_w(IC<5>{}); }
            else if constexpr (s + 3 < AD_NS) issue_w(IC<s + 3>{});
        } else {
            constexpr int np = s < AD_P0 ? 0 : (s - AD_P0 + 1 < AD_NK1 ? s - AD_P0 + 1 : AD_NK1);
            if constexpr (s >= AD_P0 && s < AD_P0 + AD_NK1) issue_p(s - AD_P0);
            if constexpr (s < AD_NK2 - 2) {
                as_wait_vm<(24 - 2 * (s + 3)) + 2 * np>();
                as_conv_ktile<false>(cz, a_half + (s + 2) * AS_KT);
                if constexpr (s == AD_NK2 - 3) as_conv_finish(cz, st, wm, g.ln_eps, cs2);
            } else if constexpr (s < AD_NK2) {
                as_wait_vm<2 * (np - 1 - (s - 10))>();
                ad_conv_ptile<s == 10>(cp, a_half + (AD_P0 + s - 10) * AS_KT);
            } else if constexpr (s - AD_NK2 + 2 < AD_NK1) {
                constexpr int kp = s - AD_NK2 + 2;
                as_wait_vm<2 * (AD_NK1 - 1 - kp)>();
                ad_conv_ptile<false>(cp, a_half + (AD_P0 + kp) * AS_KT);
                if constexpr (kp == AD_NK1 - 1) as_conv_finish(cp, st + 128, wm, g.ln_eps, cs1, 1.0f / (float)(AD_NK1 * 16));
            }
        }
        if constexpr (s + 1 < AD_NS) read_frags((s + 1) & 1, (s + 1) < AD_NK2 ? s + 1 : s + 1 - AD_NK2 + AD_P0, ad_wslot(s + 1));
        u32x4 p2[3];
#pragma unroll
        for (int j = 0; j < 3; ++j) p2[j] = f16x8_lo(fb[set][j][0]);
        if constexpr (s < AD_NK2) {
            if constexpr (s == 0) {
                const f32x16 z = {0.f, 0.f, 0.f, 0.f, 0.f, 0.f, 0.f, 0.f, 0.f, 0.f, 0.f, 0.f, 0.f, 0.f, 0.f, 0.f};
#pragma unroll
                for (int j = 0; j < 3; ++j) gatev[j] = mfma_split(fa[set][1], p2[j], z);
            } else {
#pragma unroll
                for (int j = 0; j < 3; ++j) gatev[j] = mfma_split(fa[set][1], p2[j], gatev[j]);
            }
#pragma unroll
            for (int j = 0; j < 3; ++j) gatev[j] = mfma_split(fa[set][0], fb[set][j][1], gatev[j]);
#pragma unroll
            for (int j = 0; j < 3; ++j) gatev[j] = mfma_split(fa[set][0], fb[set][j][0], gatev[j]);
        } else {
            if constexpr (s == AD_NK2) {
                const f32x16 z = {0.f, 0.f, 0.f, 0.f, 0.f, 0.f, 0.f, 0.f, 0.f, 0.f, 0.f, 0.f, 0.f, 0.f, 0.f, 0.f};
#pragma unroll
                for (int j = 0; j < 3; ++j) acc[j] = mfma_split(fa[set][1], p2[j], z);
            } else {
#pragma unroll
                for (int j = 0; j < 3; ++j) acc[j] = mfma_split(fa[set][1], p2[j], acc[j]);
            }
#pragma unroll
            for (int j = 0; j < 3; ++j) acc[j] = mfma_split(fa[set][0], fb[set][j][1], acc[j]);
#pragma unroll
            for (int j = 0; j < 3; ++j) acc[j] = mfma_split(fa[set][0], fb[set][j][0], acc[j]);
        }
        if constexpr (s == AD_NK2) gate_values();
    };

    read_frags(0, 0, ad_wslot(0));
    auto walk = [&](auto role_) __attribute__((always_inline)) { as_static_for<0, AD_NS>([&](auto s_) { step(s_, role_); }); };
    if (wn == 0) walk(IC<0>{});
    else walk(IC<1>{});

    float* Cb = g.C + (long long)b * g.sCb;
    bool bad = false;
    load_resid();
#pragma unroll
    for (int j = 0; j < 3; ++j) {
        const int nl = wn * 96 + j * 32 + (lane & 31);
        const float csum1 = cc[2 * AD_BN + nl] * inv_cs1, bias1 = cc[3 * AD_BN + nl];
        const int n = wn * 96 + j * 32 + ((lane & 31) >> 2) * 4;
#pragma unroll
        for (int rq = 0; rq < 4; ++rq) {
            const f32x4 dm4 = *reinterpret_cast<const f32x4*>(st_w + 128 + 8 * rq), rs4 = *reinterpret_cast<const f32x4*>(st_w + 192 + 8 * rq);
            float x[4], o[4];
#pragma unroll
            for (int c = 0; c < 4; ++c) {
                float v = rs4[c] * (acc[j][4 * rq + c] - dm4[c] * csum1);
                v = v + bias1;
                x[c] = v * gatev[j][4 * rq + c];
            }
            as_quad_transpose(x, o);
            f32x4 ov;
#pragma unroll
            for (int c = 0; c < 4; ++c) {
                ov[c] = o[c] + rv[rq][j][c];
                bad |= row_ok[rq] && __builtin_amdgcn_classf(ov[c], 0x207);
            }
            if (row_ok[rq]) *reinterpret_cast<f32x4*>(Cb + row_off_c[rq] + n) = ov;
        }
    }
    if (g.range_flag && __any(bad) && lane == 0) atomicOr(g.range_flag, g.range_tag);
}

__global__ __launch_bounds__(256, 2) void gemm_as_dual_kernel(const AbxGemm g) {
    extern __shared__ __attribute__((aligned(16))) float as_smem[];
    char* lds = reinterpret_cast<char*>(as_smem);
    const ClockProbe probe(g.clock_probe);
    const unsigned ntm = (unsigned)((g.M + AS_BM - 1) / AS_BM);
    const unsigned nwg = gridDim.x, bid = blockIdx.x;
    const unsigned q = nwg >> 3, r = nwg & 7, xcd = bid & 7, loc = bid >> 3;
    const unsigned wgid = (xcd < r ? xcd * (q + 1) : r * (q + 1) + (xcd - r) * q) + loc;
    const int b = (int)(wgid / ntm), mt = (int)(wgid - (unsigned)b * ntm);
    if ((mt + 1) * AS_BM > g.M) as_dual_block<true>(g, lds, mt, b);
    else as_dual_block<false>(g, lds, mt, b);
    probe.finish();
}

int as_dual_dispatch(const AbxGemm& g, hipStream_t st, int* rc) {
    auto al16 = [](const void* p) { return (reinterpret_cast<uintptr_t>(p) & 15) == 0; };
    static const bool off = [] {
        const char* e = getenv("ABX_NO_DUAL_AS");
        return e != nullptr && !(e[0] == '0' && e[1] == 0);
    }();
    if (off) return 1;
    if (g.exact == 1 || g.K != AD_NK1 * 16 || g.K2 != AD_NK2 * 16 || g.N != AD_BN) return 1;
    if (!g.A || g.A_split || g.sAm != 1 || g.M % 4 != 0 || g.M < 4 || !g.B_split || !g.B2_split || !g.b_f16) return 1;
    if (!g.ln_csum || g.ln_stats || !g.ln2_csum || !g.bias || !g.bias2 || !g.resid || !g.C) return 1;
    if (g.act != 0 || g.alpha != 1.0f || g.gate || g.mlp || g.glu || g.rowscale || g.out_ln_w || g.C_split || g.c_transposed || g.a_relu ||
        g.a_pair_transpose > 0 || g.a_pair || g.c_split_tile || g.batch_inner || g.c_planes_from)
        return 1;
    if (!g.c_vec_ok || !g.r_vec_ok) return 1;
    const long long rows_c = g.c_pair ? (long long)g.pair_L * g.pair_L : g.M;
    auto overlaps = [&](const float* p, long long sb, long long sm) {
        const float* c1 = g.C + (g.batch - 1) * g.sCb + (rows_c - 1) * g.sCm + AD_BN;
        const float* p1 = p + (g.batch - 1) * sb + (rows_c - 1) * sm + AD_BN;
        return g.C < p1 && p < c1;
    };
    if (overlaps(g.A2, g.sA2b, g.sA2m) || overlaps(g.resid, g.sRb, g.sRm)) return 1;
    if (!al16(g.A) || g.sAk % 4 != 0 || g.sAb % 4 != 0 || !al16(g.A2) || g.sA2m % 4 != 0 || g.sA2b % 4 != 0) return 1;
    if (!al16(g.B_split) || g.sB3n % 8 != 0 || g.sB3p % 8 != 0 || g.sB3k % 8 != 0 || g.sB3b % 8 != 0) return 1;
    if (!al16(g.B2_split) || g.sB23n % 8 != 0 || g.sB23p % 8 != 0 || g.sB23k % 8 != 0) return 1;
    if (g.b_exp < -100 || g.b_exp > 100 || g.b2_exp < -100 || g.b2_exp > 100) return 1;
    if ((g.pair_Lp > 0 ? (long long)g.pair_L * g.pair_L * g.sA2m : 64LL * g.sA2m) >= (1LL << 30)) return 1;
    if (16LL * g.sAk + g.M >= (1LL << 30)) return 1;
    if (g.sB3p + AD_BN * g.sB3n >= (1LL << 30) || g.sB23p + AD_BN * g.sB23n >= (1LL << 30)) return 1;
    if ((long long)AD_NK1 * g.sB3k >= (1LL << 31) || (long long)AD_NK2 * g.sB23k >= (1LL << 31)) return 1;
    const long long ntm = ((long long)g.M + AS_BM - 1) / AS_BM;
    if (ntm * g.batch >= (1LL << 31)) return 1;
    if (!(g.tune & 16384) && ntm * g.batch < 1024) return 1;
    if (int e = abx_ensure_dynamic_lds(reinterpret_cast<const void*>(&gemm_as_dual_kernel), AD_LDS, "abx_gemm(as, dual)")) {
        *rc = e;
        return 0;
    }
    hipLaunchKernelGGL(gemm_as_dual_kernel, dim3((unsigned)(ntm * g.batch)), dim3(256), AD_LDS, st, g);
    *rc = abx_check_launch("abx_gemm(as, dual)");
    return 0;
}

}

int abx_gemm_as_dispatch(const AbxGemm& g, const AbxGemm* side, hipStream_t st, int* rc) {
    auto al16 = [](const void* p) { return (reinterpret_cast<uintptr_t>(p) & 15) == 0; };
    static const bool off = getenv("ABX_NO_GEMM_AS") != nullptr;
    if (off || (g.tune & 2048)) return 1;
    if (g.A2) return side ? 1 : as_dual_dispatch(g, st, rc);
    if (g.exact == 1 || !g.B_split || !g.b_f16 || g.A_split || !g.A || g.sAk != 1 || g.K != AS_NK * 16) return 1;
    if (g.A2 || g.out_ln_w || g.mlp || g.ln_stats || g.gate || g.resid || g.batch_inner || !g.ln_csum || !g.bias) return 1;
    if (g.act != 0 || g.alpha != 1.0f) return 1;
    if (!al16(g.A) || g.sAm % 4 != 0 || g.sAb % 4 != 0 || !al16(g.B_split) || g.sB3n % 8 != 0 || g.sB3p % 8 != 0 || g.sB3k % 8 != 0) return 1;
    if (g.b_exp < -100 || g.b_exp > 100) return 1;
    if (((g.a_pair_transpose > 0 || g.a_pair) ? (long long)g.M * g.sAm : 64LL * g.sAm) >= (1LL << 30)) return 1;
    if ((long long)(g.K / 16) * g.sB3k >= (1LL << 31)) return 1;
    const long long ntm = ((long long)g.M + AS_BM - 1) / AS_BM;
    if (ntm * g.batch >= (1LL << 31)) return 1;
    if (g.N < 256 || ntm * g.batch < 1024) return 1;
    const bool glu = g.glu != 0;
    if (glu) {
        if (side || !g.C_split || !g.c_split_tile || !g.c_transposed || g.N % 128 != 0 || !g.a_pair || g.pair_Lp <= 0 || g.c_split_L != g.pair_Lp || g.c_split_nA % 32 != 0) return 1;
        if (!g.c_vec_ok || (reinterpret_cast<uintptr_t>(g.C_split) & 15) != 0 || g.sCb % 8 != 0 || g.sCm % 8 != 0 || g.sCk % 8 != 0 || g.sCp % 8 != 0) return 1;
        if (g.sB3b != 0) return 1;
    } else {
        if (g.c_transposed || g.C_split || g.rowscale || g.a_pair_transpose > 0 || g.pair_Lp != 0 || g.batch != 1) return 1;
        if (!g.c_vec_ok || g.N % 64 != 0) return 1;
        if (g.c_planes_from > 0 && (!side || g.c_planes_group != 48 || g.c_planes_from % 32 != 0 || (g.N - g.c_planes_from) % 48 != 0 || g.N >= (1 << 16))) return 1;
        if (side) {
            const AbxGemm& s = *side;
            if (g.N % 128 != 64) return 1;
            if (!s.B_split || !s.b_f16 || s.A_split || s.A != g.A || s.sAk != 1 || s.K != g.K || s.sAm != g.sAm || !s.c_transposed || s.N > 32 ||
                s.exact == 1 || (long long)s.M * s.batch != (long long)g.M || (s.batch > 1 && s.sAb != (long long)s.M * s.sAm) ||
                (s.ln_csum == nullptr) != (g.ln_csum == nullptr) || s.ln_stats || s.gate || s.resid || s.rowscale || s.act != 0 || s.glu || s.C_split ||
                s.A2 || s.out_ln_w || s.mlp || s.a_pair_transpose > 0 || s.pair_Lp != 0 || s.a_relu != g.a_relu ||
                !al16(s.B_split) || s.sB3n % 8 != 0 || s.sB3p % 8 != 0 || s.sB3k % 8 != 0 || s.b_exp < -100 || s.b_exp > 100 ||
                (long long)(s.K / 16) * s.sB3k >= (1LL << 31) || (g.ln_csum && s.ln_eps != g.ln_eps))
                return 1;
        }
    }
    static const AbxGemm none = {};
    const dim3 grid((unsigned)(ntm * g.batch)), block(256);
#define AS_LAUNCH(EPI, SIDE, ABL, ...)                                                                                                   \
    do {                                                                                                                                 \
        if (int e = abx_ensure_dynamic_lds(reinterpret_cast<const void*>(&gemm_as_kernel<EPI, SIDE, ABL, ##__VA_ARGS__>), AS_LDS, "abx_gemm(as)")) { \
            *rc = e;                                                                                                                     \
// ... 20 lines not shown
```

abx_amd/csrc/gemm_epilogue.h:

```cpp
#pragma once
#include "common.h"
#include "abx_hip.h"

template <int BM, int BN, int WM, int WN, bool EDGE, bool TS, bool OLN = false, bool PROBE = true, int TGO = 0>
__device__ __forceinline__ void gemm_epilogue(const AbxGemm& g, const float* __restrict__ st_lds, float* __restrict__ scratch,
                                              f32x16 (&acc)[WM / 32][WN / 32], int m0, int n0, int b, bool stats,
                                              f32x16 (*acc2)[WM / 32][WN / 32] = nullptr, const float* __restrict__ st2_lds = nullptr,
                                              const f32x16 (*gatev)[WM / 32][WN / 32] = nullptr) {
    constexpr int TM = WM / 32, TN = WN / 32;
    constexpr int WAVES_N = BN / WN;
    const int lane = threadIdx.x & 63, wave = threadIdx.x >> 6;
    const int wm = wave / WAVES_N, wn = wave % WAVES_N;
    float* Cb = g.C + (long long)b * g.sCb;
    const float* rs = g.rowscale ? g.rowscale + (long long)b * g.sRSb : nullptr;
    const float* gt = g.gate ? g.gate + (long long)b * g.sGb : nullptr;
    const float* rd = g.resid ? g.resid + (long long)b * g.sRb : nullptr;
    const bool c_vec = g.c_vec_ok != 0, g_vec = g.g_vec_ok != 0, r_vec = g.r_vec_ok != 0, gsig = g.gate_sigmoid != 0;
    bool bad = false;
    float bias[TN], csum[TN], bias2[TN], csum2[TN];
#pragma unroll
    for (int j = 0; j < TN; ++j) {
        const int n = n0 + wn * WN + j * 32 + (lane & 31);
        const bool nok = !EDGE || n < g.N;
        bias[j] = (g.bias && nok) ? g.bias[n] : 0.f;
        csum[j] = (stats && nok) ? g.ln_csum[n] : 0.f;
        bias2[j] = (acc2 && g.bias2 && nok) ? g.bias2[n] : 0.f;
        csum2[j] = (acc2 && nok) ? g.ln2_csum[n] : 0.f;
    }
    auto epi1 = [&](float v, int ml, int j) -> float {
        if (stats) v = st_lds[2 * ml + 1] * (v - st_lds[2 * ml] * csum[j]);
        v = (v + bias[j]) * g.alpha;
        if (g.act == 1) v = relu_keep_nan(v);
        else if (g.act == 2) v = sigmoidf_(v);
        return v;
    };
    auto load4 = [&](const float* p, bool vec, int cnt) -> f32x4 {
        f32x4 r = {0.f, 0.f, 0.f, 0.f};
        if (vec && cnt == 4) r = *reinterpret_cast<const f32x4*>(p);
        else {
#pragma unroll
            for (int c = 0; c < 4; ++c) if (c < cnt) r[c] = p[c];
        }
        return r;
    };
    auto epi2_store = [&](f32x4 v, long long off_c, long long off_g, long long off_r, int cnt, int m_idx, int n_idx) {
        if (gt) {
            f32x4 gv = load4(gt + off_g, g_vec, cnt);
            if (gsig) {
#pragma unroll
                for (int c = 0; c < 4; ++c) gv[c] = sigmoidf_(gv[c]);
            }
#pragma unroll
            for (int c = 0; c < 4; ++c) v[c] *= gv[c];
        }
        if (rd) {
            const f32x4 rv = load4(rd + off_r, r_vec, cnt);
#pragma unroll
            for (int c = 0; c < 4; ++c) v[c] += rv[c];
        }
        if constexpr (PROBE) {
#pragma unroll
            for (int c = 0; c < 4; ++c) bad |= __builtin_amdgcn_classf(v[c], 0x207) && c < cnt;
        }
        if (g.C_split) {
            unsigned a0, a1, b0, b1;
            if (n_idx < g.c_split_nA) {
                split2h(v[0], v[1], a0, a1);
                split2h(v[2], v[3], b0, b1);
            } else {
                split2b(v[0], v[1], a0, a1);
                split2b(v[2], v[3], b0, b1);
            }
            int ii, kk;
            if (g.c_split_tile) {
                pair_tile_decode(m_idx, g.c_split_L, ii, kk);
                if (ii >= g.pair_L || kk >= g.c_split_L) return;
            } else {
                ii = m_idx / g.c_split_L;
                kk = m_idx - ii * g.c_split_L;
            }
            unsigned short* cs = g.C_split + (long long)b * g.sCb + (long long)n_idx * g.sCm + (kk >> 4) * g.sCk + ii * 16 + (kk & 15);
            if (c_vec && cnt == 4) {
                *reinterpret_cast<u32x2*>(cs) = u32x2{a0, b0};
                *reinterpret_cast<u32x2*>(cs + g.sCp) = u32x2{a1, b1};
            } else {
                const unsigned pa[2] = {a0, a1}, pb[2] = {b0, b1};
#pragma unroll
                for (int p = 0; p < 2; ++p) {
                    unsigned short* o = cs + p * g.sCp;
                    if (cnt > 0) o[0] = (unsigned short)(pa[p] & 0xffffu);
                    if (cnt > 1) o[1] = (unsigned short)(pa[p] >> 16);
                    if (cnt > 2) o[2] = (unsigned short)(pb[p] & 0xffffu);
                    if (cnt > 3) o[3] = (unsigned short)(pb[p] >> 16);
                }
            }
        }
#ifdef ABX_EPI_NT_STORE
        else if (c_vec && cnt == 4) __builtin_nontemporal_store(v, reinterpret_cast<f32x4*>(Cb + off_c));
// ... 57 lines not shown
    if constexpr (!TS) {
        constexpr int TG = TGO > 0 ? TGO : (TN > 3 ? (TN % 3 == 0 ? 3 : 2) : TN);
        static_assert(TN % TG == 0, "column groups");
        constexpr int GW = TG * 32, LW = GW + 4, C4 = GW / 4, NQ = 32 * C4 / 64;
        float* wsc = scratch + wave * (32 * LW);
#pragma unroll
        for (int i = 0; i < TM; ++i) {
#pragma unroll
            for (int jg = 0; jg < TN; jg += TG) {
#pragma unroll
                for (int rq = 0; rq < 4; ++rq) {
#pragma unroll
                    for (int c = 0; c < 4; ++c) {
                        const int mloc = 8 * rq + 4 * (lane >> 5) + c;
                        const int ml = wm * WM + i * 32 + mloc;
#pragma unroll
                        for (int j = 0; j < TG; ++j) {
                            float v = pre ? acc[i][jg + j][rq * 4 + c] : epi1(acc[i][jg + j][rq * 4 + c], ml, jg + j);
                            if (acc2 && !pre) {
                                const float gv = st2_lds[2 * ml + 1] * ((*acc2)[i][jg + j][rq * 4 + c] - st2_lds[2 * ml] * csum2[jg + j]) + bias2[jg + j];
                                v *= sigmoidf_(gv);
                            }
                            if (gatev && !pre) v *= (*gatev)[i][jg + j][rq * 4 + c];
                            wsc[mloc * LW + j * 32 + (lane & 31)] = v;
                        }
                    }
                }
                __builtin_amdgcn_fence(__ATOMIC_RELEASE, "wavefront");
                __builtin_amdgcn_wave_barrier();
#pragma unroll 6
                for (int q = 0; q < NQ; ++q) {
                    const int f = lane + 64 * q;
                    const int row = f / C4, c4 = f % C4;
                    const int m = m0 + wm * WM + i * 32 + row;
                    const int n = n0 + wn * WN + jg * 32 + c4 * 4;
                    f32x4 v = *reinterpret_cast<const f32x4*>(&wsc[row * LW + c4 * 4]);
                    int cnt = 4;
                    if (EDGE) {
                        if (m >= g.M || n >= g.N) continue;
                        cnt = min(4, g.N - n);
                    }
                    if (rs) {
                        const float s = rs[m];
#pragma unroll
                        for (int c = 0; c < 4; ++c) v[c] *= s;
                    }
                    long long mo = m;
                    if (g.c_pair) {
                        const int pi = m / g.pair_Lp, pj = m - pi * g.pair_Lp;
                        if (pj >= g.pair_L) continue;
                        mo = (long long)pi * g.pair_L + pj;
                    }
                    epi2_store(v, mo * g.sCm + n, mo * g.sGm + n, mo * g.sRm + n, cnt, m, n);
                }
                __builtin_amdgcn_wave_barrier();
                __builtin_amdgcn_fence(__ATOMIC_ACQUIRE, "wavefront");
            }
        }
    } else {
        constexpr int LWT = WM + 4, M4 = WM / 4, NQ = 32 * M4 / 64;
        float* wsc = scratch + wave * (32 * LWT);
        const bool rs_vec = g.rs_vec_ok != 0;
        const bool glu = g.glu != 0;
        const int jstep = glu ? 2 : 1;
        const int Nout = glu ? g.N / 2 : g.N;
#pragma unroll
        for (int j = 0; j < TN; ++j) {
            if (glu && (j & 1)) continue;
#pragma unroll
            for (int i = 0; i < TM; ++i) {
#pragma unroll
                for (int rq = 0; rq < 4; ++rq) {
                    const int mloc = i * 32 + 8 * rq + 4 * (lane >> 5);
                    f32x4 v;
#pragma unroll
                    for (int c = 0; c < 4; ++c) v[c] = epi1(acc[i][j][rq * 4 + c], wm * WM + mloc + c, j);
                    if (glu) {
                        if constexpr (TN % 2 == 0) {
#pragma unroll
                            for (int c = 0; c < 4; ++c) {
                                const float gv = epi1(acc[i][(j | 1) < TN ? (j | 1) : j][rq * 4 + c], wm * WM + mloc + c, (j | 1) < TN ? (j | 1) : j);
                                v[c] *= sigmoidf_(gv);
                            }
                        }
                    }
                    *reinterpret_cast<f32x4*>(&wsc[(lane & 31) * LWT + mloc]) = v;
                }
            }
            __builtin_amdgcn_fence(__ATOMIC_RELEASE, "wavefront");
            __builtin_amdgcn_wave_barrier();
#pragma unroll
            for (int q = 0; q < NQ; ++q) {
                const int f = lane + 64 * q;
                const int nl = f / M4, m4 = f % M4;
                const int n = (n0 + wn * WN + j * 32) / jstep + nl;
                const int m = m0 + wm * WM + m4 * 4;
                f32x4 v = *reinterpret_cast<const f32x4*>(&wsc[nl * LWT + m4 * 4]);
                int cnt = 4;
                if (EDGE) {
                    if (m >= g.M || n >= Nout) continue;
                    cnt = min(4, g.M - m);
                }
                if (rs) {
                    long long rsi = m;
                    if (g.c_split_tile) {
                        int pi, pj;
// ... 19 lines not shown
```

abx_amd/model/forward.py:

```python
import math

import numpy as np
import torch

from abx_amd import ops
from abx_amd import residue_constants as rc

_NO_ASSEMBLE_BIAS = not bool(__import__('os').environ.get('ABX_ASSEMBLE_BIAS'))
_NO_OPM_FUSED = bool(__import__('os').environ.get('ABX_NO_OPM_FUSED'))
P_SEQF = 'impl.seqformer.'
P_BLK = 'impl.seqformer.seqformer.blocks.0.'
P_IPA = 'impl.diffusion_module.ScoreNetwork.'


class Packed:

    def __init__(self, sd, device):
        f = lambda k: sd[k].detach().to(device=device, dtype=torch.float32).contiguous()
        self.sd = {k: f(k) for k in sd}
        g = self.sd
        self.wt, self.b = {}, {}
        self._ln_cache = {}
        self._split_cache = {}
        self.gemm_mode = 0
# ... 321 lines not shown
                ops.assemble_pair_bias(pstat, temb, prev_pair, *P.ln(P_SEQF + 'prev_pair_norm'), prev_pos, P.sd[P_SEQF + 'proj_prev_pos.weight'],
                                       pair_act, bw3, bcs, bbias, biasT, Bc, L, range_class=P.plain_class)
                fused_bias = True
        if not fused_bias:
            ops.assemble_pair(pstat, temb, prev_pair, *P.ln(P_SEQF + 'prev_pair_norm'), prev_pos,
                              P.sd[P_SEQF + 'proj_prev_pos.weight'], pair_act, Bc, L, CZ, E)
        if st.get('esm_embed') is not None:
            e = st['esm_embed'][b0:b1]
            wl = torch.softmax(P.sd[P_SEQF + 'esm_embed_weights'], dim=-1)
            mixed = torch.einsum('blcn,n->blc', e.to(wl.dtype), wl).reshape(Bc * Lab, -1).contiguous()
            h1 = ws.get('esm_h', (Bc * Lab, CS))
            _ln_lin(P, P_SEQF + 'proj_esm_embed.1', P_SEQF + 'proj_esm_embed.0', None, mixed, h1, act=1)
            tgt = seq_act[:, :Lab, :CS]
            _lin(P, P_SEQF + 'proj_esm_embed.3', h1.view(Bc, Lab, CS), tgt, resid=tgt)
        s2 = seq_act.view(M1, WS_)
        z2 = pair_act.view(M2, WZ)
        z3 = pair_act.view(Bc, LL, WZ)
        if self.block_api:
            attn_ws = self._block_workspace('attn', Bc, L)
            w768 = attn_ws[:M2 * 768 * 4].view(torch.float32).view(M2, 768)
        else:
            w768 = ws.get('w768', (M2, 768))
        w384 = ws.get('w384', (M2 * 384,))
        pmask = ws.get('pmask', (M2,))
        ops.pair_mask(mask_f, pmask, Bc, L)

        pre = P_BLK + 'seq_attn.'
        if not fused_bias:
            _ln_lin(P, pre + 'proj_pair', pre + 'pair_norm', None, z3, biasT.transpose(1, 2), narrow=True)
        qkv = ws.get('s_a', (M1, 3 * WS_))
        sgate = ws.get('s_b', (M1, WS_))
        so = ws.get('s_c', (M1, WS_))
        _ln_lin(P, pre + 'attn.proj_in', pre + 'seq_norm', None, s2, qkv)
        _ln_lin(P, pre + 'attn.gate', pre + 'seq_norm', None, s2, sgate)
        ops.seq_attn(qkv, biasT, mask_f, sgate, so, Bc, L, H, WS_ // H)
        _lin(P, pre + 'attn.proj_out', so, s2, resid=s2)
        pre = P_BLK + 'seq_transition.transition.'
        hid = ws.get('s_a', (M1, 4 * WS_))
        _ln_lin(P, pre + '1', pre + '0', None, s2, hid, act=1)
        _lin(P, pre + '3', hid, s2, resid=s2)
        pre = P_BLK + 'outer_product_mean.'
        lr = ws.get('s_b', (M1, 128))
        _ln_lin(P, pre + 'lr', pre + 'norm', None, s2, lr, rowscale=mask_f.reshape(-1))
        if not P.exact(P.plain_class) and tuple(P.wt[pre + 'out_proj'].shape) == (128, 192) and not _NO_OPM_FUSED:
            ops.opm_out(lr, P.wt[pre + 'out_proj'], P.b.get(pre + 'out_proj'), z2, Bc, L, range_class=P.plain_class)
        else:
            feat = w384[:M2 * 128].view(M2, 128)
            ops.opm_features(lr, feat, Bc, L, 64)
            _lin(P, pre + 'out_proj', feat, z2, resid=z2)
        planes = not P.exact('plane_projection', 'contraction', 'tri_mul_tail')
        Lp = (L + 3) // 4 * 4
        LLp = L * Lp
        pad = (L, Lp) if Lp != L else None
        for name, outgoing in (('triangle_multiplication_outgoing', True), ('triangle_multiplication_incoming', False)):
            pre = P_BLK + name + '.'
            if blocks is not None and planes:
                zb = w768.view(-1)[:Bc * LL * 192].view(Bc, LL, 192)
                zin, zout = (z3, zb) if outgoing else (zb, z3)
                ops.tri_mul_fwd(blocks[name], zin, zout, mask_f, Bc, L, outgoing, self._block_workspace('mul', Bc, L))
                continue
            GT = w768.view(-1)[:Bc * 256 * LL].view(Bc, 256, LL)
            Gf = w768.view(-1)[Bc * 256 * LL:Bc * 448 * LL].view(Bc, LL, 192)
            if planes:
                zb = w768.view(-1)[:Bc * LL * 192].view(Bc, LL, 192)
                zin, zout = (z3, zb) if outgoing else (zb, z3)
                KT = (Lp + 15) // 16
                lrp = ws.get('tm_lr', (Bc, 256, KT, 2, L, 16), torch.int16, zero=(Lp % 16 != 0))
                if pad is None:
                    pm = pmask
                else:
                    pm = ws.get('pmask_p', (Bc * LLp,))
                    ops.pair_mask(mask_f, pm, Bc, L, Lp)
                _ln_lin(P, pre + 'lr_glu', pre + 'norm', None, zin, lrp, rowscale=pm, glu=True, c_split_nA=128, c_split_tile=True,
                        a_pair_transpose=0 if outgoing else L, pair=(L, Lp), a_pair=True)
                tt = w384[:Bc * 128 * LLp].view(Bc, 128, LLp)
                tz = tt.as_strided((Bc * 128, L, L), (LLp, Lp, 1))
                ops.gemm(lrp[:, 0:128], lrp[:, 128:256], tz, exact=2)
                gw, gcs, gb, gw3 = P.ln_linear(pre + 'final_gate', pre + 'norm')
                _ln_lin(P, pre + 'proj_out', pre + 'final_norm', None, tt.transpose(1, 2), zout, resid=zin, pair=pad, c_pair=pad is not None,
                        dual=(zin, gw3, gcs, gb))
            else:
                _ln_lin(P, pre + 'final_gate', pre + 'norm', None, z3, Gf, act=2)
                tt = w384[2 * Bc * 128 * LL:3 * Bc * 128 * LL].view(Bc, 128, LL)
                tz = tt.view(Bc * 128, L, L)
                _ln_lin(P, pre + 'lr_gates', pre + 'norm', None, z3, GT.transpose(1, 2), act=2)
                left = w384[0:Bc * 128 * LL].view(Bc, 128, LL)
                right = w384[Bc * 128 * LL:2 * Bc * 128 * LL].view(Bc, 128, LL)
                _ln_lin(P, pre + 'left_proj', pre + 'norm', None, z3, left.transpose(1, 2), rowscale=pmask,
                        gate=GT[:, 0:128].transpose(1, 2), gate_sigmoid=False)
                _ln_lin(P, pre + 'right_proj', pre + 'norm', None, z3, right.transpose(1, 2), rowscale=pmask,
                        gate=GT[:, 128:256].transpose(1, 2), gate_sigmoid=False)
                lz = left.view(Bc * 128, L, L)
                rz = right.view(Bc * 128, L, L)
                if outgoing:
                    ops.gemm(lz, rz.transpose(1, 2), tz, exact=1)
                else:
                    ops.gemm(lz.transpose(1, 2), rz, tz, exact=1)
                tcm = tt.transpose(1, 2)
                _ln_lin(P, pre + 'proj_out', pre + 'final_norm', None, tcm, z3, gate=Gf, gate_sigmoid=False, resid=z3)
        for name, per_row in (('triangle_attention_starting_node', True), ('triangle_attention_ending_node', False)):
            pre = P_BLK + name + '.'
            ax = P.exact('tri_attn')
            if blocks is not None:
                flagged = bool(P.exact_tags & ops.RANGE_TAGS['tri_attn'])
                ops.tri_attn_block_fwd(blocks[name], z2, mask_f, Bc, L, per_row, attn_ws, exact=ax, attn_exact=ops.GEMM_EXACT or flagged)
                continue
            am = 1 if ax else 2
            ae = True if (P.exact_tags & ops.RANGE_TAGS['tri_attn']) else None
            bT = ws.get('biasT', (Bc, 4, LL))
            qkv = w768.view(-1)[:M2 * 576].view(M2, 576)
            bl2 = not (ops.GEMM_EXACT if ae is None else ae)
            kvp = ops.KV_PLANES and am == 2 and bl2 and ops.kv_planes_ok(M2)
            rowp = getattr(P.block_packs()[name], '_row', None) if (am == 2 and bl2 and not kvp) else None
            if rowp is not None and ops._tri_rowfused_ok(L):
                _ln_lin(P, pre + 'proj_pair', pre + 'norm', None, z3, bT.transpose(1, 2), narrow=True, exact=am, alpha=ops.TRI_BIAS_LOG2,
                        range_class='tri_attn')
            else:
                rowp = None
                ops.gemm_side(_ln_lin(P, pre + 'qkv', pre + 'norm', None, z2, qkv, defer=True, exact=am, range_class='tri_attn',
                                      c_plane_cols=(192, 48) if kvp else None),
                              _ln_lin(P, pre + 'proj_pair', pre + 'norm', None, z3, bT.transpose(1, 2), narrow=True, defer=True, exact=am,
                                      alpha=ops.TRI_BIAS_LOG2 if bl2 else 1.0, range_class='tri_attn'))
            o = w384[:M2 * 192].view(M2, 192)
            if not per_row or Lp != L:
                bT2 = ws.get('biasT2', (Bc, 4, L, Lp))
                ops.transpose_last2(bT.view(Bc * 4, L, L), bT2.view(Bc * 4, L, Lp), transpose=not per_row)
                bT = bT2
            else:
                bT = bT.view(Bc, 4, L, L)
            if rowp is not None:
                ops.tri_attn(z2, bT, mask_f, o, Bc, L, per_row, bias_is_qk=True, exact=ae, bias_log2=True, rowpack=rowp)
            else:
                ops.tri_attn(qkv, bT, mask_f, o, Bc, L, per_row, bias_is_qk=True, exact=ae, bias_log2=bl2, kv_planes=kvp)
            if not ax:
                _ln_lin(P, pre + 'attn.gate', pre + 'norm', None, z2, z2, act=2, gate=o, resid=z2, mlp=P.mlp_second(pre + 'attn.proj_out'), exact=2)
            else:
                hid = w768.view(-1)[M2 * 576:M2 * 768].view(M2, 192)
                _ln_lin(P, pre + 'attn.gate', pre + 'norm', None, z2, hid, act=2, gate=o, gate_sigmoid=False, exact=1)
                _lin(P, pre + 'attn.proj_out', hid, z2, resid=z2, exact=1)
        pre = P_BLK + 'pair_transition.transition.'
        tx = P.exact('pair_transition')
        if blocks is not None:
            ops.transition_fwd(*blocks['pair_transition'], z2, exact=tx, workspace=w768)
        elif not tx:
            _ln_lin(P, pre + '1', pre + '0', None, z2, z2, act=1, resid=z2, mlp=P.mlp_second(pre + '3'), exact=2)
        else:
            _ln_lin(P, pre + '1', pre + '0', None, z2, w768, act=1, exact=1)
            _lin(P, pre + '3', w768, z2, resid=z2, exact=1)

        P.plain_class = 'gemm_late'
        ic = cfg.heads.diffusion_module.IPA
        NC = ic.num_channel
        s_pre = ws.get('i_a', (M1, NC))
        _lin(P, P_IPA + 'proj_init_seq_act', s2, s_pre)
        s0 = ws.get('i_s0', (M1, NC))
        ops.layernorm(s_pre, *P.ln(P_IPA + 'init_seq_layer_norm'), out=s0)
        s = ws.get('i_s', (M1, NC))
        _lin(P, P_IPA + 'proj_seq', s0, s)
        zi = w384[:M2 * 128].view(M2, 128)
        if not P.exact('ipa_pair_init'):
            _lin(P, P_IPA + 'proj_init_pair_act', z2, zi, out_ln=P.ln(P_IPA + 'init_pair_layer_norm'), exact=2)
        else:
            _lin(P, P_IPA + 'proj_init_pair_act', z2, zi, exact=1)
            ops.layernorm(zi, *P.ln(P_IPA + 'init_pair_layer_norm'), out=zi)
        bias2d = w384[M2 * 128:M2 * 140].view(M2, 12)
        _lin(P, P_IPA + 'attention_module.proj_pair', zi, bias2d, alpha=P.ipa_w2d, narrow=True)
        attn_ws = w384[M2 * 140:M2 * 152].view(M2, 12)
        init_q = ws.get('f_iq', (M1, 4)); init_t = ws.get('f_it', (M1, 3))
        cur_q = ws.get('f_q', (M1, 4)); cur_t = ws.get('f_t', (M1, 3)); cur_R = ws.get('f_R', (M1, 9))
        delta_q = ws.get('f_dq', (M1, 4))
        rig_in = st['rigids_t'][b0:b1].contiguous()
        ops.frames_init(rig_in, init_q, init_t, cur_q, cur_t, cur_R, delta_q, M1, ic.position_scale)
        proj = ws.get('i_proj', (M1, 1152))
        qpack = ws.get('i_qp', (ops.ipa_qpack_numel(Bc, L),)); kpack = ws.get('i_kp', (M1 * 12 * 28,)); vpack = ws.get('i_vp', (M1 * 12 * 40,))
        ifeat = ws.get('i_feat', (M1, 2112))
        h1 = ws.get('i_h1', (M1, NC)); h2 = ws.get('i_h2', (M1, NC))
        upd = ws.get('i_upd', (M1, 6))
        tail = None
        if not P.exact('ipa_tail', 'gemm_late') and NC == 256:
            wb = lambda n: (P.split(P_IPA + n), P.b[P_IPA + n])
            tail = (wb('attention_module.final_proj'), P.ln(P_IPA + 'attention_layer_norm'), wb('transition_module.0'),
                    wb('transition_module.2'), wb('transition_module.4'), P.ln(P_IPA + 'transition_layer_norm'))
        for _ in range(ic.num_layer):
            _lin(P, P_IPA + 'attention_module.proj', s, proj)
            ops.ipa_pack(proj, cur_R, cur_t, qpack, kpack, vpack, Bc, L, P.ipa_ws)
            ops.ipa_weights(qpack, kpack, vpack, bias2d, mask_f, cur_R, cur_t, P.ipa_pw, attn_ws, ifeat, Bc, L)
            ops.ipa_pair(attn_ws, zi, ifeat, Bc, L)
            if tail is not None:
# ... 64 lines not shown
```

abx_amd/ops.py:

```python
import ctypes as C
import math

import torch

from abx_amd import _lib
from abx_amd._lib import (AbxGemm, AbxTriAttn, AbxIpaTail, AbxHeadsTail, AbxScoreArgs, AbxReverseArgs, AbxGuidanceArgs, AbxDesignScoreArgs, AbxRelaxArgs, AbxInterfaceArgs, AbxEnsemblePairsArgs, AbxEnsembleClusterArgs, AbxLinearPack, AbxLinearSrc,
                           AbxTriMulPack, AbxTriAttnPack, AbxTriRowPack, check)


def _stream():
    return C.c_void_p(torch.cuda.current_stream().cuda_stream)


def _p(t):
    if t is None:
        return None
    assert t.is_cuda, 'libabx_hip works on device memory only'
    return t.data_ptr()


def _f32(t):
    assert t.dtype == torch.float32, t.dtype
    return t

# ... 121 lines not shown
    b = None
    if bv is not None or bg is not None:
        z = torch.zeros(C_, device=Wv.device, dtype=Wv.dtype)
        b = torch.stack([(bv if bv is not None else z).reshape(C_ // 32, 32), (bg if bg is not None else z).reshape(C_ // 32, 32)],
                        dim=1).reshape(2 * C_).contiguous()
    return W, b


_PERM16 = (0, 1, 2, 3, 8, 9, 10, 11, 4, 5, 6, 7, 12, 13, 14, 15)


def permute_k16(Wt):
    K, N = Wt.shape
    assert K % 16 == 0
    idx = torch.tensor(_PERM16, device=Wt.device)
    return Wt.reshape(K // 16, 16, N)[:, idx, :].reshape(K, N).contiguous()


class WeightPlanes(torch.Tensor):
    w_exp = 0
    __torch_function__ = torch._C._disabled_torch_function_impl


def split_weights(Wt):
    K, N = Wt.shape
    _f32(Wt)
    Kp = (K + 15) // 16 * 16
    amax = float(Wt.abs().max())
    if not math.isfinite(amax):
        raise ValueError('split_weights: non-finite weight')
    w_exp = 14 - math.frexp(amax)[1] if amax > 0 else 0
    w_exp = max(-100, min(100, w_exp))
    out = torch.empty(Kp // 16, 2, N, 16, device=Wt.device, dtype=torch.float16)
    check(_lib.load().abx_split_weights_f16(_p(Wt), Wt.stride(1), Wt.stride(0), N, K, w_exp, _p(out), _stream()), 'abx_split_weights_f16')
    out = out.as_subclass(WeightPlanes)
    out.w_exp = w_exp
    return out


def weights_to_float(w3):
    v = (w3[:, 0].float() + w3[:, 1].float()) * 2.0 ** (-w3.w_exp)
    return v.permute(0, 2, 1).reshape(-1, w3.shape[2])


def _weight_planes(w3, N, K=None, what='B3'):
    assert isinstance(w3, WeightPlanes) and w3.dtype == torch.float16 and w3.is_contiguous() and w3.shape[1:] == (2, N, 16), \
        f'{what}: WeightPlanes (ops.split_weights) of N = {N} expected'
    assert K is None or w3.shape[0] * 16 >= K
    return w3


def gemm(A, B, Cout, *, ln=None, a_relu=False, bias=None, alpha=1.0, act=0, rowscale=None, gate=None, gate_sigmoid=True,
         resid=None, tune=None, B3=None, exact=None, a_pair_transpose=0, glu=False, pair=None, a_pair=False, c_pair=False, dual=None, out_ln=None, clock_probe=None, mlp=None, c_split_nA=0, c_split_tile=False,
         defer=False, range_class=None, c_plane_cols=None):
    lib = _lib.load()
    g = AbxGemm()
    a_planes, b_planes, c_planes = A.dtype == torch.int16, B.dtype == torch.int16, Cout.dtype == torch.int16
    if a_planes and A.dim() == 6:
        assert B.dtype == torch.int16 and B.dim() == 6 and B.shape[:2] == A.shape[:2]
        g.batch_inner, g.sA3i, g.sB3i = A.shape[1], A.stride(1), B.stride(1)
        bo_a, bo_b = A.stride(0), B.stride(0)
        A = A.as_strided((A.shape[0] * A.shape[1],) + tuple(A.shape[2:]), (0,) + tuple(A.stride()[2:]), A.storage_offset())
        B = B.as_strided((B.shape[0] * B.shape[1],) + tuple(B.shape[2:]), (0,) + tuple(B.stride()[2:]), B.storage_offset())
    else:
        bo_a = bo_b = None
    if a_planes:
        assert A.dim() == 5 and A.shape[2] == 2 and A.shape[4] == 16 and A.stride(4) == 1
        nb, KT, _, M, _ = A.shape
        K = KT * 16
        g.A_split, g.sA3b, g.sA3k, g.sA3p, g.sA3m = _p(A), (A.stride(0) if nb > 1 else 0), A.stride(1), A.stride(2), A.stride(3)
        if bo_a is not None:
            g.sA3b = bo_a
    else:
        if A.dim() == 2:
            A = A.unsqueeze(0)
        nb, M, K = A.shape
        _f32(A)
        g.A, g.sAb, g.sAm, g.sAk = _p(A), A.stride(0) if nb > 1 else 0, A.stride(1), A.stride(2)
        if a_pair:
            assert pair is not None and M == pair[0] * pair[0], (A.shape, pair)
            M = pair[0] * pair[1]
            if c_split_tile:
                M = ((pair[0] + 7) // 8 * 8) * ((pair[1] + 15) // 16 * 16)
    if b_planes:
        assert B.dim() == 5 and B.shape[2] == 2 and B.shape[4] == 16 and B.stride(4) == 1 and B.shape[1] * 16 == K and B.shape[0] == nb
        N = B.shape[3]
        g.B_split, g.sB3b, g.sB3k, g.sB3p, g.sB3n = _p(B), (B.stride(0) if nb > 1 else 0), B.stride(1), B.stride(2), B.stride(3)
        if bo_b is not None:
            g.sB3b = bo_b
    else:
        if B.dim() == 2:
            B = B.unsqueeze(0)
        assert B.shape[1] == K, (A.shape, B.shape)
        N = B.shape[2]
        _f32(B)
        g.B, g.sBb, g.sBk, g.sBn = _p(B), (B.stride(0) if B.shape[0] > 1 else 0), B.stride(1), B.stride(2)
    No = N // 2 if glu else N
    if mlp is not None:
        B32m, bias2m = mlp
        No = B32m.shape[2]
        _weight_planes(B32m, No, what='mlp B3_2')
        assert B32m.shape[0] * 16 == N
        g.mlp, g.N2, g.b2_exp = (2 if gate is not None else 1), No, B32m.w_exp
        g.B2_split, g.sB23k, g.sB23p, g.sB23n = _p(B32m), B32m.stride(0), B32m.stride(1), B32m.stride(2)
        g.bias2 = _p(bias2m)
        assert act == (2 if gate is not None else 1) and ln is not None and ln[0] is None
    if c_planes:
# ... 35 lines not shown
    if B3 is not None:
        _weight_planes(B3, N, K)
        assert not a_planes, 'weight planes go with an fp32 A (the plane x plane contraction takes activation images on both sides)'
        g.B_split, g.sB3k, g.sB3p, g.sB3n, g.sB3b = _p(B3), B3.stride(0), B3.stride(1), B3.stride(2), 0
        g.b_f16, g.b_exp = 1, B3.w_exp
    g.tune = GEMM_TUNE if tune is None else tune
    if c_plane_cols is not None:
        g.c_planes_from, g.c_planes_group = int(c_plane_cols[0]), int(c_plane_cols[1])
    if RANGE_CHECK and g.exact != 1:
        g.range_flag = range_ptr(Cout.device)
        g.range_tag = RANGE_TAGS[('tri_attn' if gate is not None else 'pair_transition') if mlp is not None else 'tri_mul_tail' if dual is not None else 'ipa_pair_init' if out_ln is not None
                                 else 'plane_projection' if c_planes else 'contraction' if a_planes else (range_class or 'gemm')]
    if dual is not None:
        A2, B32, csum2, bias2 = dual
        if A2.dim() == 2:
            A2 = A2.unsqueeze(0)
        _f32(A2)
        assert A2.stride(2) == 1 and A2.shape[0] == nb and A2.shape[1] == (pair[0] * pair[0] if pair is not None else M)
        K2 = A2.shape[2]
        _weight_planes(B32, N, what='dual B3_2')
        assert B32.shape[0] * 16 == K2 and csum2.numel() == N
        g.b2_exp = B32.w_exp
        g.A2, g.sA2b, g.sA2m, g.K2 = _p(A2), (A2.stride(0) if nb > 1 else 0), A2.stride(1), K2
        g.B2_split, g.sB23k, g.sB23p, g.sB23n = _p(B32), B32.stride(0), B32.stride(1), B32.stride(2)
        g.ln2_csum, g.bias2 = _p(_f32(csum2)), _p(bias2)
        if g.ln_eps == 0:
            g.ln_eps = 1e-5
    if out_ln is not None:
        assert out_ln[0].numel() == N and out_ln[1].numel() == N
        g.out_ln_w, g.out_ln_b = _p(_f32(out_ln[0])), _p(_f32(out_ln[1]))
        g.out_ln_eps = float(out_ln[2]) if len(out_ln) > 2 else 1e-5
    if clock_probe is not None:
        assert clock_probe.dtype == torch.int64 and clock_probe.numel() >= 2
        g.clock_probe = _p(clock_probe)
    g.bias = _p(bias)
    g.alpha = float(alpha)
    g.act = int(act)
    if rowscale is not None:
        rs_rows = pair[0] * pair[1] if c_split_tile else M
        assert rowscale.numel() == nb * rs_rows and rowscale.is_contiguous()
        g.rowscale, g.sRSb = _p(_f32(rowscale)), rs_rows
    if gate is not None:
        if gate.dim() == 2:
            gate = gate.unsqueeze(0)
        cd, sd = (1, 2) if g.c_transposed else (2, 1)
        assert gate.shape == (nb, M if c_planes else Cout.shape[1], N) and gate.stride(cd) == 1, 'gate must be laid out like Cout (mlp: (M, N) rows)'
        g.gate, g.sGb, g.sGm, g.gate_sigmoid = _p(_f32(gate)), (gate.stride(0) if nb > 1 else 0), gate.stride(sd), int(gate_sigmoid)
    if resid is not None:
        if resid.dim() == 2:
            resid = resid.unsqueeze(0)
        cd, sd = (1, 2) if g.c_transposed else (2, 1)
        assert resid.shape == (nb, M if c_planes else Cout.shape[1], No if mlp is not None else N) and resid.stride(cd) == 1, 'resid must be laid out like Cout'
        g.resid, g.sRb, g.sRm = _p(_f32(resid)), (resid.stride(0) if nb > 1 else 0), resid.stride(sd)
    if defer:
        return g
    check(lib.abx_gemm(C.byref(g), _stream()), 'abx_gemm')
    return Cout


def gemm_side(g_main, g_side):
    check(_lib.load().abx_gemm_side(C.byref(g_main), C.byref(g_side), _stream()), 'abx_gemm_side')


def planes_to_float(p, a_side, dim=0):
    h = p.view(torch.float16).float()
    p0, p1 = h.select(dim, 0), h.select(dim, 1)
    return (p0 + p1 / 2048.0) * 16.0 if a_side else (p0 + p1) / 16.0


def row_stats(x, out=None, eps=1e-5):
    lib = _lib.load()
    _f32(x)
    if x.dim() == 2:
        rows, K = x.shape
        assert x.stride(1) == 1
        if out is None:
            out = torch.empty(rows, 2, device=x.device, dtype=torch.float32)
        check(lib.abx_row_stats(_p(x), 0, x.stride(0), 1, 1, rows, K, eps, _p(out), _stream()), 'abx_row_stats')
    else:
        nb, rows, K = x.shape
        assert x.stride(1) == 1, 'channel-major layout expected'
        if out is None:
            out = torch.empty(nb * rows, 2, device=x.device, dtype=torch.float32)
        check(lib.abx_row_stats(_p(x), x.stride(0), 1, x.stride(2), nb, rows, K, eps, _p(out), _stream()), 'abx_row_stats')
    return out


def layernorm(x, gamma, beta, out=None, res=None, eps=1e-5):
    lib = _lib.load()
    rows, K = x.shape
    assert x.stride(1) == 1
    if out is None:
        out = torch.empty(rows, K, device=x.device, dtype=torch.float32)
    check(lib.abx_layernorm(_p(_f32(x)), x.stride(0), rows, K, _p(gamma), _p(beta), eps, _p(out), out.stride(0),
                            _p(res), res.stride(0) if res is not None else 0, _stream()), 'abx_layernorm')
    return out


def transpose_last2(x, out, transpose=True):
    L, Lp = x.shape[-1], out.shape[-1]
    assert x.shape[-2] == L and x.is_contiguous() and out.is_contiguous() and out.shape[:-1] == x.shape[:-1] and Lp >= L
    check(_lib.load().abx_transpose_last2(_p(_f32(x)), _p(out), x.numel() // (L * L), L, Lp, int(bool(transpose)), _stream()),
          'abx_transpose_last2')
    return out


# ... 28 lines not shown

        def view(ptr, numel, dtype):
            if not ptr:
                return None
            o = ptr - base.data_ptr()
            return base[o:o + numel * torch.empty(0, dtype=dtype).element_size()].view(dtype)

        Kp = (K + 15) // 16 * 16
        self.Wt = view(self.c.Wt, K * N, torch.float32).view(K, N)
        self.csum = view(self.c.csum, N, torch.float32)
        self.bias = view(self.c.bias, N, torch.float32)
        pl = view(self.c.planes, Kp * 2 * N, torch.float16).view(Kp // 16, 2, N, 16).as_subclass(WeightPlanes)
        pl.w_exp = self.w_exp
        self.planes = pl


def _range_args(exact, name):
    if RANGE_CHECK and not exact:
        return range_ptr(torch.device('cuda', torch.cuda.current_device())), RANGE_TAGS[name]
    return None, 0


def transition_fwd(l1, l2, z, exact=False, workspace=None):
    lib = _lib.load()
    M = z.shape[0]
    assert z.is_contiguous() and z.shape[1] == l1.K
    if exact:
        need = int(lib.abx_transition_workspace_bytes(M, l1.N, 1))
        assert workspace is not None and workspace.numel() * workspace.element_size() >= need
    rf, rt = _range_args(exact, 'pair_transition')
    check(lib.abx_transition_fwd(C.byref(l1.c), C.byref(l2.c), _p(z), M, int(bool(exact)), _p(workspace), rf, rt, _stream()), 'abx_transition_fwd')
    return z


def tri_mul_pack(glu, out, gate):
    p = AbxTriMulPack()
    p.glu, p.out, p.gate = glu.c, out.c, gate.c
    p._keep = (glu, out, gate)
    return p


def tri_mul_workspace(B, L, device):
    lib = _lib.load()
    ws = torch.empty(int(lib.abx_tri_mul_workspace_bytes(B, L)) + 256, dtype=torch.uint8, device=device)
    ws = ws[(-ws.data_ptr()) % 256:]
    check(lib.abx_tri_mul_workspace_init(_p(ws), B, L, _stream()), 'abx_tri_mul_workspace_init')
    return ws


def tri_mul_workspace_init(ws, B, L):
    check(_lib.load().abx_tri_mul_workspace_init(_p(ws), B, L, _stream()), 'abx_tri_mul_workspace_init')


def tri_mul_fwd(pack, z_in, z_out, mask_f, B, L, outgoing, workspace):
    lib = _lib.load()
    assert z_in.is_contiguous() and z_out.is_contiguous() and z_in.data_ptr() != z_out.data_ptr()
    rf, rt = _range_args(False, 'contraction')
    check(lib.abx_tri_mul_fwd(C.byref(pack), _p(z_in), _p(z_out), _p(_f32(mask_f)), B, L, int(bool(outgoing)), _p(workspace), rf, rt, _stream()),
          'abx_tri_mul_fwd')
    return z_out


class TriRowPack:

    def __init__(self, qkv):
        lib = _lib.load()
        nbytes = int(lib.abx_tri_rowpack_bytes())
        self.buf = torch.empty(nbytes + 256, dtype=torch.uint8, device=qkv.buf.device)
        off = (-self.buf.data_ptr()) % 256
        self.c = AbxTriRowPack()
        check(lib.abx_tri_rowpack(C.byref(qkv.c), self.buf[off:].data_ptr(), C.byref(self.c), _stream()), 'abx_tri_rowpack')
        self.qkv = qkv


def tri_attn_pack(qkv, gate, pair, out):
    p = AbxTriAttnPack()
    p.qkv, p.gate, p.pair, p.out = qkv.c, gate.c, pair.c, out.c
    p._keep = (qkv, gate, pair, out)
    p._row = None
    if qkv.buf.is_cuda and qkv.K == 192 and qkv.N == 576 and qkv.c.csum:
        p._row = TriRowPack(qkv)
        p.row = p._row.c
    return p


def tri_attn_block_workspace(B, L, device):
    ws = torch.empty(int(_lib.load().abx_tri_attn_block_workspace_bytes(B, L)) + 256, dtype=torch.uint8, device=device)
    return ws[(-ws.data_ptr()) % 256:]


def tri_attn_block_fwd(pack, z, mask_f, B, L, per_row, workspace, exact=False, attn_exact=None):
    lib = _lib.load()
    ax = bool(GEMM_EXACT if attn_exact is None else attn_exact)
    ex = int(bool(exact)) | (2 if ax else 0)
    rf, rt = _range_args(ex == 3, 'tri_attn')
    check(lib.abx_tri_attn_block_fwd(C.byref(pack), _p(z), _p(_f32(mask_f)), B, L, int(bool(per_row)), ex, _p(workspace), rf, rt, _stream()),
          'abx_tri_attn_block_fwd')
    return z


def _tri_rowfused_ok(L):
    return bool(_lib.load().abx_tri_attn_rowfused_ok(int(L)))


_TRI_ATTN_LAST = None


def tri_attn_kernel_name(L, exact=None, bias_vec=True, rowfused=None):
    ex = bool(GEMM_EXACT if exact is None else exact)
    if ex:
        return 'tri_attn_kernel'
    if rowfused is None:
        if _TRI_ATTN_LAST is not None and _TRI_ATTN_LAST[:2] == (int(L), ex):
            rowfused = _TRI_ATTN_LAST[2]
        else:
            rowfused = _tri_rowfused_ok(L) and gemm_mode(L) == 2 and not KV_PLANES
    if rowfused:
        return 'tri_attn8_rowfused_kernel'
    kc = 128 if (L + 127) // 128 == (L + 191) // 192 else 192
    return 'tri_attn8_kernel<%d, 768, %s>' % (kc, 'true' if bias_vec else 'false')


TRI_BIAS_LOG2 = float(__import__('numpy').float32(1.4426950408889634) * __import__('numpy').float32(128.0))


KV_PLANES = bool(__import__('os').environ.get('ABX_KV_PLANES'))


def kv_planes_ok(M):
    return bool(_lib.load().abx_gemm_planes_ok(int(M))) and not GEMM_EXACT and not (GEMM_TUNE & 2048)


def tri_attn(qkvg, biasT, keymask, out, B, L, per_row, H=4, D=48, bias_is_qk=False, exact=None, clock_probe=None, tune=0, bias_log2=False, kv_planes=False,
             rowpack=None, slot_order=-1):
    lib = _lib.load()
    W = qkvg.shape[1]
    fused = rowpack is not None
    assert (W == H * D) if fused else (W in (3 * H * D, 4 * H * D)), 'z rows (H*D wide) go with rowpack=, projected rows are 3 or 4 x H*D wide'
    assert qkvg.is_contiguous() and out.is_contiguous() and biasT.is_contiguous()
    a = AbxTriAttn()
    es = qkvg.element_size()
    base = qkvg.data_ptr()
    if not fused:
        a.q, a.k, a.v = base, base + H * D * es, base + 2 * H * D * es
    if W == 4 * H * D:
        a.gate = base + 3 * H * D * es
    a.sb = L * L * W
    a.ss, a.sl = (L * W, W) if per_row else (W, L * W)
    a.bias = _p(biasT)
    Lp = biasT.shape[-1] if (biasT.dim() == 4 and bias_is_qk) else L
    assert biasT.numel() == B * H * L * Lp
# ... 565 lines not shown
```

include/abx_hip.h:

```cpp
#ifndef ABX_HIP_H
#define ABX_HIP_H

#include <stdint.h>
#ifdef __HIPCC__
#include <hip/hip_runtime.h>
#else
typedef struct ihipStream_t* hipStream_t;
#endif

#ifdef __cplusplus
extern "C" {
#endif

#define ABX_HIP_ABI_VERSION 1

int abx_version(void);
const char* abx_last_error_string(void);
int abx_init(int device);
int abx_debug_poison_lds(unsigned pattern, hipStream_t stream);

typedef struct AbxGemm {
    const float* A; long long sAb, sAm, sAk;
    const float* B; long long sBb, sBk, sBn;
    float* C;       long long sCb, sCm;
    int M, N, K, batch;
    int c_transposed;
    const float* ln_stats; long long sSb;
    const float* ln_csum;
    float ln_eps;
    int a_relu;
    const float* bias;
    float alpha;
    int act;
    const float* rowscale; long long sRSb;
    const float* gate; long long sGb, sGm; int gate_sigmoid;
    const float* resid; long long sRb, sRm;
    const unsigned short* B_split; long long sB3p, sB3n, sB3k, sB3b;
    const unsigned short* A_split; long long sA3p, sA3m, sA3k, sA3b;
    int batch_inner; long long sA3i, sB3i;
    int c_split_tile;
    int c_split_nA;
    unsigned short* C_split; long long sCp, sCk; int c_split_L;
    int glu;
    int a_pair_transpose;
    int pair_L, pair_Lp;
    int a_pair;
    int c_pair;
    const float* A2; long long sA2b, sA2m; int K2;
    const unsigned short* B2_split; long long sB23p, sB23n, sB23k;
    const float* ln2_csum; const float* bias2;
    int mlp, N2;
    const float* out_ln_w; const float* out_ln_b; float out_ln_eps;
    int exact;
    int b_f16, b_exp, b2_exp;
    int tune;
    int c_planes_from, c_planes_group;
    int* range_flag; int range_tag;
    unsigned long long* clock_probe;
    int a_vec_ok, b_vec_ok, fast_ok;
    int c_vec_ok, g_vec_ok, r_vec_ok, rs_vec_ok;
} AbxGemm;
int abx_gemm(const AbxGemm* desc, hipStream_t stream);
int abx_gemm_side(const AbxGemm* main_gemm, const AbxGemm* side_gemm, hipStream_t stream);
int abx_gemm_planes_ok(long long M);
int abx_gemm_check_modes(const AbxGemm* desc);
int abx_split_weights_f16(const float* w, long long s_n, long long s_k, int N, int K, int scale_exp, unsigned short* out, hipStream_t stream);
typedef struct AbxIpaTail {
    const float* feat; long long s_feat;
    float* s; long long s_s;
    int M, K1, C;
    const unsigned short* W_final; int e_final; const float* b_final;
    const float* ln1_w; const float* ln1_b;
    const unsigned short* W_t0; int e_t0; const float* b_t0;
    const unsigned short* W_t2; int e_t2; const float* b_t2;
    const unsigned short* W_t4; int e_t4; const float* b_t4;
    const float* ln2_w; const float* ln2_b;
    float ln_eps;
    const float* W_aff; const float* b_aff;
    const int* fixed; const float* init_q; const float* init_t;
    float* cur_q; float* cur_t; float* cur_R; float* delta_q; float pscale;
    int* range_flag; int range_tag;
    const float* partial; int n_partial; long long s_partial;
} AbxIpaTail;
int abx_ipa_tail(const AbxIpaTail* desc, hipStream_t stream);
typedef struct AbxHeadsTail {
    const float* s; long long s_s;
    const float* s0; long long s_s0;
    int M;
    const unsigned short* W_act; int e_act; const float* b_act;
    const unsigned short* W_init; int e_init; const float* b_init;
    const unsigned short* W_r0; int e_r0; const float* b_r0;
    const unsigned short* W_r1; int e_r1; const float* b_r1;
    const unsigned short* W_r2; int e_r2; const float* b_r2;
    const unsigned short* W_r3; int e_r3; const float* b_r3;
    const unsigned short* W_proj; int e_proj; const float* b_proj;
    float* un;
    const float* lns_w; const float* lns_b;
    const unsigned short* W_s1; int e_s1; const float* b_s1;
    const unsigned short* W_s3; int e_s3; const float* b_s3;
    const unsigned short* W_s5; int e_s5; const float* b_s5;
    float* logits;
    const float* lnp_w; const float* lnp_b;
    const unsigned short* W_p1; int e_p1; const float* b_p1;
    const unsigned short* W_p3; int e_p3; const float* b_p3;
    const unsigned short* W_p5; int e_p5; const float* b_p5;
    float* pl;
    float ln_eps;
    int* range_flag; int range_tag;
} AbxHeadsTail;
int abx_heads_tail(const AbxHeadsTail* desc, hipStream_t stream);
int abx_gemm3_occupancy(int which);

int abx_row_stats(const float* x, long long s_b, long long s_row, long long s_k, int batch, int rows, int K, float eps,
// ... 195 lines not shown
#define ABX_ENS_MAX_POINTS 512
#define ABX_ENS_MAX_N 1024
#define ABX_ENS_COLS 10
typedef struct AbxEnsemblePairsArgs {
    const float* pred_atom14; long long pred_sb; int Lpred;
    const long long* pred_seq; long long pred_seq_sb;
    const unsigned char* region;
    int atoms, M;
    double* planes; long long plane_stride;
    int N;
} AbxEnsemblePairsArgs;
long long abx_ensemble_pairs_workspace_bytes(int N, int P);
int abx_ensemble_pairs(const AbxEnsemblePairsArgs* a, void* workspace, hipStream_t stream);
typedef struct AbxEnsembleClusterArgs {
    const double* planes; long long plane_stride;
    int metric;
    double cutoff;
    double* out; long long out_stride;
    int* centres; int* n_clusters;
    int N;
} AbxEnsembleClusterArgs;
int abx_ensemble_cluster(const AbxEnsembleClusterArgs* a, hipStream_t stream);

typedef struct AbxLinearPack {
    const float* Wt;
    const float* csum;
    const float* bias;
    const unsigned short* planes;
    int b_exp;
    int K, N;
} AbxLinearPack;
typedef struct AbxLinearSrc { const float* W; const float* b; int rows; int glu; } AbxLinearSrc;
#define ABX_PACK_PERMUTE_K16 1
long long abx_pack_linear_bytes(int K, int N);
int abx_pack_linear(const AbxLinearSrc* src, int nsrc, int K, const float* gamma, const float* beta, int flags, void* buf,
                    AbxLinearPack* out, hipStream_t stream);

long long abx_transition_workspace_bytes(long long M, int hidden, int exact);
int abx_transition_fwd(const AbxLinearPack* l1, const AbxLinearPack* l2, float* z, long long M, int exact, void* workspace,
                       int* range_flag, int range_tag, hipStream_t stream);

typedef struct AbxTriMulPack { AbxLinearPack glu, out, gate; } AbxTriMulPack;
long long abx_tri_mul_workspace_bytes(int B, int L);
int abx_tri_mul_workspace_init(void* workspace, int B, int L, hipStream_t stream);
int abx_tri_mul_fwd(const AbxTriMulPack* w, const float* z_in, float* z_out, const float* mask, int B, int L, int outgoing,
                    void* workspace, int* range_flag, int range_tag, hipStream_t stream);

int abx_tri_rowpack(const AbxLinearPack* qkv, void* buf, AbxTriRowPack* out, hipStream_t stream);
typedef struct AbxTriAttnPack { AbxLinearPack qkv, gate, pair, out; AbxTriRowPack row; } AbxTriAttnPack;
long long abx_tri_attn_block_workspace_bytes(int B, int L);
int abx_tri_attn_block_fwd(const AbxTriAttnPack* w, float* z, const float* mask, int B, int L, int per_row, int exact, void* workspace,
                           int* range_flag, int range_tag, hipStream_t stream);

#ifdef __cplusplus
}
#endif
#endif
```

Baseline: 168.9 sample-steps/s.

## Fold triangle-attention pair-bias projection into preceding block epilogues

Computes the LayerNorm-folded 192->4 pair-bias projection for the next triangle attention inside the epilogue of the preceding GEMM (tri-mul output tail or the attention gated tail). The attention block can then skip its own pass over z that produces the bias. The aim is to remove one full read of the L^2 x 192 pair tensor and a kernel launch per attention block. The cost is more epilogue work, extra LDS for the side weights, and a new path that is on by default and can be turned off with ABX_NO_BIAS_FOLD.

```diff
diff --git a/abx_amd/_lib.py b/abx_amd/_lib.py
--- a/abx_amd/_lib.py
+++ b/abx_amd/_lib.py
@@ -49,6 +49,10 @@
         ('clock_probe', c_f),
         ('a_vec_ok', I), ('b_vec_ok', I), ('fast_ok', I),
         ('c_vec_ok', I), ('g_vec_ok', I), ('r_vec_ok', I), ('rs_vec_ok', I),
+        ('side_Wt', c_f), ('side_csum', c_f), ('side_bias', c_f),
+        ('side_eps', F), ('side_alpha', F),
+        ('side_n', I),
+        ('side_out', c_f), ('side_sb', LL), ('side_sn', LL), ('side_rows', LL),
     ]
 
 
@@ -335,6 +339,10 @@
     'abx_tri_mul_fwd': (I, [C.POINTER(AbxTriMulPack), c_f, c_f, c_f, I, I, I, c_f, c_f, I, _S]),
     'abx_tri_attn_block_workspace_bytes': (LL, [I, I]),
     'abx_tri_attn_block_fwd': (I, [C.POINTER(AbxTriAttnPack), c_f, c_f, I, I, I, I, c_f, c_f, I, _S]),
+    'abx_tri_bias_fold_ok': (I, [I]),
+    'abx_tri_attn_block_bias_offset': (LL, [I, I]),
+    'abx_tri_mul_bias_fwd': (I, [C.POINTER(AbxTriMulPack), c_f, c_f, c_f, I, I, I, c_f, C.POINTER(AbxLinearPack), c_f, c_f, I, _S]),
+    'abx_tri_attn_block_bias_fwd': (I, [C.POINTER(AbxTriAttnPack), c_f, c_f, I, I, I, I, c_f, I, C.POINTER(AbxLinearPack), c_f, c_f, I, _S]),
 }
 
 EXPORTED = tuple(_PROTOS)
diff --git a/abx_amd/csrc/blocks.hip b/abx_amd/csrc/blocks.hip
--- a/abx_amd/csrc/blocks.hip
+++ b/abx_amd/csrc/blocks.hip
@@ -67,6 +67,13 @@
 inline void set_range(AbxGemm& g, int* flag, int tag, int exact) {
     if (!exact) { g.range_flag = flag; g.range_tag = tag; }
 }
+inline void set_bias_side(AbxGemm& g, const AbxLinearPack& pair, float* out, long long LL) {
+    g.side_Wt = pair.Wt; g.side_csum = pair.csum; g.side_bias = pair.bias;
+    g.side_eps = 1e-5f; g.side_alpha = ABX_TRI_BIAS_LOG2;
+    g.side_n = pair.N;
+    g.side_out = out; g.side_sb = (long long)pair.N * LL; g.side_sn = LL; g.side_rows = LL;
+}
+inline bool pair_pack_ok(const AbxLinearPack* p) { return p && p->Wt && p->csum && p->bias && p->N == 4 && p->K == 192; }
 
 }
 
@@ -211,8 +218,17 @@
     return ABX_OK;
 }
 
-extern "C" int abx_tri_mul_fwd(const AbxTriMulPack* wp, const float* z_in, float* z_out, const float* mask, int B, int L, int outgoing,
-                               void* workspace, int* range_flag, int range_tag, hipStream_t st) {
+extern "C" int abx_tri_bias_fold_ok(int L) {
+    static const bool off = [] {
+        const char* e = getenv("ABX_NO_BIAS_FOLD");
+        return e != nullptr && !(e[0] == '0' && e[1] == 0);
+    }();
+    return (!off && abx_tri_attn_rowfused_ok(L)) ? 1 : 0;
+}
+
+namespace {
+int tri_mul_fwd(const AbxTriMulPack* wp, const float* z_in, float* z_out, const float* mask, int B, int L, int outgoing,
+                void* workspace, const AbxLinearPack* next_pair, float* bias_out, int* range_flag, int range_tag, hipStream_t st) {
     ABX_REQUIRE(wp && z_in && z_out && z_in != z_out && mask && workspace && B > 0 && L > 0, "abx_tri_mul_fwd: bad args (z_out must not alias z_in)");
     const AbxLinearPack &glu = wp->glu, &out = wp->out, &gate = wp->gate;
     ABX_REQUIRE(glu.csum && out.csum && gate.csum && glu.N == 512 && out.K == 128 && gate.K == glu.K && out.N == gate.N && glu.K == out.N,
@@ -261,8 +277,28 @@
         g.ln2_csum = gate.csum; g.bias2 = gate.bias;
         g.resid = z_in; g.sRb = LL * C; g.sRm = C;
         set_range(g, range_flag, range_tag, 0);
+        if (next_pair) {
+            set_bias_side(g, *next_pair, bias_out, LL);
+            g.tune |= 16384;
+        }
         return abx_gemm(&g, st);
     }
+}
+}
+
+extern "C" int abx_tri_mul_fwd(const AbxTriMulPack* wp, const float* z_in, float* z_out, const float* mask, int B, int L, int outgoing,
+                               void* workspace, int* range_flag, int range_tag, hipStream_t st) {
+    return tri_mul_fwd(wp, z_in, z_out, mask, B, L, outgoing, workspace, nullptr, nullptr, range_flag, range_tag, st);
+}
+
+extern "C" int abx_tri_mul_bias_fwd(const AbxTriMulPack* wp, const float* z_in, float* z_out, const float* mask, int B, int L, int outgoing,
+                                    void* workspace, const AbxLinearPack* next_pair, float* bias_out, int* range_flag, int range_tag,
+                                    hipStream_t st) {
+    if (!next_pair) return tri_mul_fwd(wp, z_in, z_out, mask, B, L, outgoing, workspace, nullptr, nullptr, range_flag, range_tag, st);
+    ABX_REQUIRE(pair_pack_ok(next_pair) && bias_out, "abx_tri_mul_bias_fwd: next_pair = a LayerNorm-folded 192 -> 4 pack, with its destination");
+    ABX_REQUIRE(abx_tri_attn_rowfused_ok(L), "abx_tri_mul_bias_fwd: the bias fold needs the row-fused attention route (abx_tri_bias_fold_ok)");
+    if (!abx_tri_bias_fold_ok(L)) next_pair = nullptr;
+    return tri_mul_fwd(wp, z_in, z_out, mask, B, L, outgoing, workspace, next_pair, bias_out, range_flag, range_tag, st);
 }
 
 namespace {
@@ -281,14 +317,20 @@
 }
 }
 
+extern "C" long long abx_tri_attn_block_bias_offset(int B, int L) {
+    if (B <= 0 || L <= 0) return -1;
+    return up(4LL * B * L * L * 768);
+}
+
 extern "C" long long abx_tri_attn_block_workspace_bytes(int B, int L) {
     if (B <= 0 || L <= 0) return -1;
     const long long LL = (long long)L * L, Lp = (L + 3) / 4 * 4;
     return up(4LL * B * LL * 768) + up(4LL * B * 4 * LL) + up(4LL * B * 4 * L * Lp) + up(4LL * B * LL * 192);
 }
 
-extern "C" int abx_tri_attn_block_fwd(const AbxTriAttnPack* wp, float* z, const float* mask, int B, int L, int per_row, int exact,
-                                      void* workspace, int* range_flag, int range_tag, hipStream_t st) {
+namespace {
+int tri_attn_block_fwd(const AbxTriAttnPack* wp, float* z, const float* mask, int B, int L, int per_row, int exact, void* workspace,
+                       int bias_ready, const AbxLinearPack* next_pair, float* next_bias_out, int* range_flag, int range_tag, hipStream_t st) {
     ABX_REQUIRE(wp && z && mask && workspace && B > 0 && L > 0, "abx_tri_attn_block_fwd: bad args");
     const AbxLinearPack &qkv = wp->qkv, &gate = wp->gate, &pair = wp->pair, &out = wp->out;
     ABX_REQUIRE(qkv.csum && gate.csum && pair.csum && qkv.N == 576 && gate.N == 192 && pair.N == 4 && qkv.K == 192 && gate.K == 192 && pair.K == 192 &&
@@ -305,7 +347,10 @@
     static const bool kv_planes_on = getenv("ABX_KV_PLANES") != nullptr;
     const int planes = (kv_planes_on && !exact && !attn_exact && abx_gemm_planes_ok(M2)) ? 1 : 0;
     const bool rowfused = !exact && !attn_exact && !planes && wp->row.planes && abx_tri_attn_rowfused_ok(L);
-    if (rowfused) {
+    ABX_REQUIRE(rowfused || (!bias_ready && !next_pair),
+                "abx_tri_attn_block_bias_fwd: the bias fold needs the row-fused route (exact = 0, a row pack, abx_tri_attn_rowfused_ok(L))");
+    if (rowfused && bias_ready) {
+    } else if (rowfused) {
         AbxGemm s2 = {};
         s2.A = z; s2.sAb = LL * C; s2.sAm = C; s2.sAk = 1;
         s2.C = w.bT; s2.sCb = 4 * LL; s2.sCm = LL; s2.c_transposed = 1;
@@ -370,6 +415,7 @@
         g.bias2 = out.bias;
         g.resid = z; g.sRm = C;
         set_range(g, range_flag, range_tag, 0);
+        if (next_pair) set_bias_side(g, *next_pair, next_bias_out, LL);
         return abx_gemm(&g, st);
     }
     {
@@ -393,3 +439,21 @@
         return abx_gemm(&g, st);
     }
 }
+}
+
+extern "C" int abx_tri_attn_block_fwd(const AbxTriAttnPack* wp, float* z, const float* mask, int B, int L, int per_row, int exact,
+                                      void* workspace, int* range_flag, int range_tag, hipStream_t st) {
+    return tri_attn_block_fwd(wp, z, mask, B, L, per_row, exact, workspace, 0, nullptr, nullptr, range_flag, range_tag, st);
+}
+
+extern "C" int abx_tri_attn_block_bias_fwd(const AbxTriAttnPack* wp, float* z, const float* mask, int B, int L, int per_row, int exact,
+                                           void* workspace, int bias_ready, const AbxLinearPack* next_pair, float* next_bias_out,
+                                           int* range_flag, int range_tag, hipStream_t st) {
+    ABX_REQUIRE(!next_pair || (pair_pack_ok(next_pair) && next_bias_out),
+                "abx_tri_attn_block_bias_fwd: next_pair = a LayerNorm-folded 192 -> 4 pack, with its destination");
+    if ((bias_ready || next_pair) && abx_tri_attn_rowfused_ok(L) && !abx_tri_bias_fold_ok(L)) {
+        bias_ready = 0;
+        next_pair = nullptr;
+    }
+    return tri_attn_block_fwd(wp, z, mask, B, L, per_row, exact, workspace, bias_ready ? 1 : 0, next_pair, next_bias_out, range_flag, range_tag, st);
+}
diff --git a/abx_amd/csrc/gemm.hip b/abx_amd/csrc/gemm.hip
--- a/abx_amd/csrc/gemm.hip
+++ b/abx_amd/csrc/gemm.hip
@@ -473,6 +473,7 @@
 }
 
 extern "C" int abx_gemm_side(const AbxGemm* main_gemm, const AbxGemm* side_gemm, hipStream_t st) {
+    ABX_REQUIRE(!(main_gemm && main_gemm->side_out) && !(side_gemm && side_gemm->side_out), "abx_gemm_side: no side_out (AbxGemm.side_out) in a pair launch");
     ABX_REQUIRE(main_gemm && side_gemm, "abx_gemm_side: null descriptor");
     AbxGemm g, s2;
     if (int rc = gemm_prepare(main_gemm, g)) return rc;
@@ -494,6 +495,17 @@
     auto al16 = [](const void* p) { return (reinterpret_cast<uintptr_t>(p) & 15) == 0; };
     (void)al16;
     const bool akc = g.sAk == 1;
+    if (g.side_out) {
+        ABX_REQUIRE(g.side_Wt && g.side_csum && g.side_bias && g.side_n >= 1 && g.side_n <= 4 && g.side_rows >= 0 && g.side_sb >= 0 && g.side_sn >= 0,
+                    "abx_gemm: side_out needs side_Wt / side_csum / side_bias, 1 <= side_n <= 4, non-negative strides");
+        if (g.side_eps == 0.f) g.side_eps = 1e-5f;
+        int rc = 0;
+        if (g.exact != 1 && g.A2 && !abx_gemm_as_dispatch(g, nullptr, st, &rc)) return rc;
+        if (g.exact != 1 && g.mlp == 2 && !(g.tune & 64) && !abx_gemm3_dispatch(g, st, &rc)) return rc;
+        abx_set_error("abx_gemm: side_out is written by gemm_as_dual_kernel (the out-of-place dual tail, K = 128, K2 = N = 192; tune bit 14 below "
+                      "1 024 blocks) and gemm3_gtail_kernel (mlp = 2, N = N2 = 192) only - this descriptor is dispatched to neither");
+        return ABX_ERR_ARG;
+    }
     if (g.exact != 1) {
         int rc = 0;
         if (!abx_gemm_as_dispatch(g, nullptr, st, &rc)) return rc;
diff --git a/abx_amd/csrc/gemm3.hip b/abx_amd/csrc/gemm3.hip
--- a/abx_amd/csrc/gemm3.hip
+++ b/abx_amd/csrc/gemm3.hip
@@ -826,7 +826,8 @@
 constexpr int GT1_W2 = 2 * 96 * 32;
 constexpr int GT1_OFF_G = GT1_G1, GT1_OFF_W2 = GT1_OFF_G + 3 * 128 * 64, GT1_OFF_CST = GT1_OFF_W2 + 2 * GT1_W2;
 constexpr int GT1_LDS = GT1_OFF_CST + 2 * GT_NG * 4;
-template <bool EDGE>
+__device__ __forceinline__ bool al16d(const void* p) { return (reinterpret_cast<uintptr_t>(p) & 15) == 0; }
+template <bool EDGE, bool SIDEO = false>
 __device__ __forceinline__ void gemm3_gtail_block(const AbxGemm& g, float* smem, int mt, int b) {
     constexpr int BM = 128, BN = 192, WM = 32, BH = 96, TH = BH / 32, NKT = BN / 16;
     char* lds = reinterpret_cast<char*>(smem);
@@ -889,6 +890,20 @@
     const float cs2 = __builtin_ldexpf(1.0f, -4 - g.b2_exp);
     u32x4 hfa[NKT][2];
     constexpr int TA[3] = {1, 0, 0}, TB[3] = {0, 1, 0};
+    float sp[6] = {0.f, 0.f, 0.f, 0.f, 0.f, 0.f};
+    const float sshift = lsh[0] + dmean;
+    float* sw_lds = reinterpret_cast<float*>(lds + 1024 + 4 * 32 * 100 * 4);
+    static_assert(1024 + 4 * 32 * 100 * 4 + 192 * 16 <= GT1_OFF_W2, "side weights: between the epilogue scratch and the W_o stages");
+    f32x4 swreg = {0.f, 0.f, 0.f, 0.f};
+    if constexpr (SIDEO) {
+        if (threadIdx.x < 192) {
+            if (g.side_n == 4 && al16d(g.side_Wt)) swreg = *reinterpret_cast<const f32x4*>(g.side_Wt + threadIdx.x * 4);
+            else {
+#pragma unroll
+                for (int e = 0; e < 4; ++e) if (e < g.side_n) swreg[e] = g.side_Wt[threadIdx.x * g.side_n + e];
+            }
+        }
+    }
 #pragma unroll
     for (int half = 0; half < 2; ++half) {
         f32x16 acc2[1][TH];
@@ -945,9 +960,50 @@
         }
 #pragma unroll
         for (int t = 0; t < TH; ++t) acc2[0][t] *= cs2;
-        gemm_epilogue<BM, BH, WM, BH, EDGE, false>(g2, smem, smem + 2 * BM, acc2, m0, half * BH, b, false);
+        if constexpr (SIDEO) {
+            if (half == 0) {
+                if (threadIdx.x < 192) *reinterpret_cast<f32x4*>(sw_lds + threadIdx.x * 4) = swreg;
+                __syncthreads();
+            }
+            gemm_epilogue<BM, BH, WM, BH, EDGE, false, false, true, 0, true>(g2, smem, smem + 2 * BM, acc2, m0, half * BH, b, false, nullptr, nullptr, nullptr, sp, sshift, sw_lds);
+        }
+        else gemm_epilogue<BM, BH, WM, BH, EDGE, false>(g2, smem, smem + 2 * BM, acc2, m0, half * BH, b, false);
         if (half == 0) __syncthreads();
     }
+    if constexpr (SIDEO) {
+        float t[6];
+#pragma unroll
+        for (int k = 0; k < 6; ++k) t[k] = sp[k] + __shfl_xor(sp[k], 32, 64);
+        const float invN = 1.0f / (float)BN;
+        const float dm = t[0] * invN;
+        const float rs = 1.0f / sqrtf(fmaxf(t[1] * invN - dm * dm, 0.f) + g.side_eps);
+        const long long m = (long long)m0 + wave * WM + lane;
+        if (lane < 32 && m < g.M) {
+            long long sb = b, r = m;
+            if (g.side_rows > 0) {
+                const long long per = ((long long)g.M + g.side_rows - 1) / g.side_rows;
+                sb = (long long)b * per + m / g.side_rows;
+                r = m % g.side_rows;
+            }
+            float* so = g.side_out + sb * g.side_sb + r;
+#pragma unroll
+            for (int e = 0; e < 4; ++e)
+                if (e < g.side_n) so[e * g.side_sn] = g.side_alpha * (rs * (t[2 + e] - dm * g.side_csum[e]) + g.side_bias[e]);
+        }
+    }
+}
+
+__global__ __launch_bounds__(256, 2) void gemm3_gtail_side_kernel(const AbxGemm g) {
+    extern __shared__ __attribute__((aligned(16))) float gt_smem[];
+    const int ntm = (g.M + 127) / 128;
+    const unsigned nwg = gridDim.x, bid = blockIdx.x;
+    const unsigned q = nwg >> 3, r = nwg & 7, xcd = bid & 7, loc = bid >> 3;
+    const unsigned wgid = (xcd < r ? xcd * (q + 1) : r * (q + 1) + (xcd - r) * q) + loc;
+    const int b = (int)(wgid / (unsigned)ntm), mt = (int)(wgid - (unsigned)b * (unsigned)ntm);
+    const ClockProbe probe(g.clock_probe);
+    if ((mt + 1) * 128 <= g.M) gemm3_gtail_block<false, true>(g, gt_smem, mt, b);
+    else gemm3_gtail_block<true, true>(g, gt_smem, mt, b);
+    probe.finish();
 }
 
 __global__ __launch_bounds__(256, 2) void gemm3_gtail_kernel(const AbxGemm g) {
@@ -1286,6 +1342,7 @@
 
 int abx_gemm3_dispatch(const AbxGemm& g, hipStream_t st, int* rc) {
     auto al16 = [](const void* p) { return (reinterpret_cast<uintptr_t>(p) & 15) == 0; };
+    if (g.side_out && g.mlp != 2) return 1;
     const bool narrow = g.B_split && g.N <= 32 && !g.A_split && g.sAk == 1 && !g.glu && !g.C_split && !g.A2 && !g.out_ln_w &&
                         g.a_pair_transpose <= 0 && g.pair_Lp == 0;
     if (!g.B_split || g.K % 16 != 0 || (g.N <= 64 && !narrow)) return 1;
@@ -1341,6 +1398,17 @@
             if (int e = abx_ensure_dynamic_lds(reinterpret_cast<const void*>(&gemm3_gtail2w_kernel), GT_LDS, "abx_gemm(gated tail)")) { *rc = e; return 0; }
             hipLaunchKernelGGL(gemm3_gtail2w_kernel, dim3((unsigned)(mt * g.batch)), dim3(256), GT_LDS, st, g);
             *rc = abx_check_launch("abx_gemm(gated tail, two walks)");
+            return 0;
+        }
+        if (g.side_out) {
+            if (g.N != 192 || g.N2 != 192) {
+                abx_set_error("abx_gemm: side_out on the gated tail needs N = N2 = 192");
+                *rc = ABX_ERR_ARG;
+                return 0;
+            }
+            if (int e = abx_ensure_dynamic_lds(reinterpret_cast<const void*>(&gemm3_gtail_side_kernel), GT1_LDS, "abx_gemm(gated tail, side)")) { *rc = e; return 0; }
+            hipLaunchKernelGGL(gemm3_gtail_side_kernel, dim3((unsigned)(mt * g.batch)), dim3(256), GT1_LDS, st, g);
+            *rc = abx_check_launch("abx_gemm(gated tail, side)");
             return 0;
         }
         if (int e = abx_ensure_dynamic_lds(reinterpret_cast<const void*>(&gemm3_gtail_kernel), GT1_LDS, "abx_gemm(gated tail)")) { *rc = e; return 0; }
diff --git a/abx_amd/csrc/gemm_as.hip b/abx_amd/csrc/gemm_as.hip
--- a/abx_amd/csrc/gemm_as.hip
+++ b/abx_amd/csrc/gemm_as.hip
@@ -584,6 +584,9 @@
 constexpr int AD_OFF_CONST = AD_OFF_ST + 4 * 64 * 4;
 constexpr int AD_LDS = AD_OFF_CONST + 4 * AD_BN * 4;
 static_assert(AD_LDS <= 81920, "two blocks per CU");
+constexpr int AD_OFF_SW = AD_LDS;
+constexpr int AD_LDS_SIDE = AD_OFF_SW + AD_BN * 16;
+static_assert(AD_LDS_SIDE <= 81920, "two blocks per CU");
 constexpr int AD_P0 = 4;
 constexpr int ad_wslot(int t) { return t < 4 ? AD_OFF_RING + (t & 1) * AD_STAGE : ((t - 4) % 3 == 0 ? AD_OFF_RING : ((t - 4) % 3 == 1 ? 0 : AD_OFF_RING + AD_STAGE)); }
 
@@ -635,7 +638,7 @@
                  : "memory");
 }
 
-template <bool EDGE>
+template <bool EDGE, bool SIDE = false>
 __device__ __forceinline__ void as_dual_block(const AbxGemm& g, char* lds, int mt, int b) {
     const int lane = threadIdx.x & 63, wave = __builtin_amdgcn_readfirstlane(threadIdx.x >> 6);
     const int wm = wave >> 1, wn = wave & 1, h = lane >> 5;
@@ -697,6 +700,11 @@
         as_conv_ktile<true>(cz, a_half);
         as_conv_ktile<false>(cz, a_half + AS_KT);
     } else {
+        if constexpr (SIDE) {
+#pragma unroll
+            for (int i = 0; i < 2; ++i)
+                if (2 * wm + i < 3) as_glds16(reinterpret_cast<const char*>(g.side_Wt) + (2 * wm + i) * 1024 + lane * 16, lds + AD_OFF_SW + (2 * wm + i) * 1024);
+        }
         const float* c0 = wm ? g.ln_csum : g.ln2_csum;
         const float* c1 = wm ? g.bias : g.bias2;
 #pragma unroll
@@ -746,6 +754,7 @@
     f32x4 rv[4][3];
     long long row_off_c[4];
     bool row_ok[4];
+    float sh[4] = {0.f, 0.f, 0.f, 0.f};
     auto load_resid = [&]() __attribute__((always_inline)) {
         const float* rd = g.resid + (long long)b * g.sRb;
 #pragma unroll
@@ -760,6 +769,9 @@
             }
             row_ok[rq] = ok;
             row_off_c[rq] = mo * g.sCm;
+            if constexpr (SIDE) {
+                if (ok) sh[rq] = rd[mo * g.sRm] + st[wm * 32 + 8 * rq + 4 * h + (lane & 3)];
+            }
 #pragma unroll
             for (int j = 0; j < 3; ++j) {
                 const int n = wn * 96 + j * 32 + ((lane & 31) >> 2) * 4;
@@ -836,11 +848,24 @@
     float* Cb = g.C + (long long)b * g.sCb;
     bool bad = false;
     load_resid();
+    float ps[4][6];
+    if constexpr (SIDE) {
+#pragma unroll
+        for (int rq = 0; rq < 4; ++rq)
+#pragma unroll
+            for (int k = 0; k < 6; ++k) ps[rq][k] = 0.f;
+    }
+    constexpr int sn = 4;
 #pragma unroll
     for (int j = 0; j < 3; ++j) {
         const int nl = wn * 96 + j * 32 + (lane & 31);
         const float csum1 = cc[2 * AD_BN + nl] * inv_cs1, bias1 = cc[3 * AD_BN + nl];
         const int n = wn * 96 + j * 32 + ((lane & 31) >> 2) * 4;
+        f32x4 sw[4];
+        if constexpr (SIDE) {
+#pragma unroll
+            for (int c = 0; c < 4; ++c) sw[c] = *reinterpret_cast<const f32x4*>(lds + AD_OFF_SW + (n + c) * 16);
+        }
 #pragma unroll
         for (int rq = 0; rq < 4; ++rq) {
             const f32x4 dm4 = *reinterpret_cast<const f32x4*>(st_w + 128 + 8 * rq), rs4 = *reinterpret_cast<const f32x4*>(st_w + 192 + 8 * rq);
@@ -859,9 +884,60 @@
                 bad |= row_ok[rq] && __builtin_amdgcn_classf(ov[c], 0x207);
             }
             if (row_ok[rq]) *reinterpret_cast<f32x4*>(Cb + row_off_c[rq] + n) = ov;
+            if constexpr (SIDE) {
+                f32x2 asq = {ps[rq][0], ps[rq][1]}, a01 = {ps[rq][2], ps[rq][3]}, a23 = {ps[rq][4], ps[rq][5]};
+#pragma unroll
+                for (int c = 0; c < 4; ++c) {
+                    const float d = ov[c] - sh[rq];
+                    const f32x2 d2 = {d, d};
+                    asq = __builtin_elementwise_fma(d2, (f32x2){1.0f, d}, asq);
+                    a01 = __builtin_elementwise_fma(d2, (f32x2){sw[c][0], sw[c][1]}, a01);
+                    a23 = __builtin_elementwise_fma(d2, (f32x2){sw[c][2], sw[c][3]}, a23);
+                }
+                ps[rq][0] = asq[0]; ps[rq][1] = asq[1];
+                ps[rq][2] = a01[0]; ps[rq][3] = a01[1];
+                ps[rq][4] = a23[0]; ps[rq][5] = a23[1];
+            }
         }
     }
     if (g.range_flag && __any(bad) && lane == 0) atomicOr(g.range_flag, g.range_tag);
+    if constexpr (SIDE) {
+        float* part = reinterpret_cast<float*>(lds);
+#pragma unroll
+        for (int rq = 0; rq < 4; ++rq) {
+#pragma unroll
+            for (int k = 0; k < 6; ++k) {
+                float v = ps[rq][k];
+                v += __builtin_bit_cast(float, __builtin_amdgcn_update_dpp(0, __builtin_bit_cast(int, v), 0x124, 0xf, 0xf, false));
+                v += __builtin_bit_cast(float, __builtin_amdgcn_update_dpp(0, __builtin_bit_cast(int, v), 0x128, 0xf, 0xf, false));
+                v += __shfl_xor(v, 16, 64);
+                if ((lane & 28) == 0) part[(wn * 6 + k) * 64 + wm * 32 + 8 * rq + 4 * h + (lane & 3)] = v;
+            }
+        }
+        __syncthreads();
+        if (threadIdx.x < 64) {
+            const int r = threadIdx.x, m = m0 + r;
+            bool ok = m < g.M;
+            long long mo = m;
+            if (g.c_pair) {
+                const int pi = m / g.pair_Lp, pj = m - pi * g.pair_Lp;
+                ok = ok && pj < g.pair_L;
+                mo = (long long)pi * g.pair_L + pj;
+            }
+            float t[6];
+#pragma unroll
+            for (int k = 0; k < 6; ++k) t[k] = part[k * 64 + r] + part[(6 + k) * 64 + r];
+            const float invN = 1.0f / (float)AD_BN;
+            const float dm = t[0] * invN;
+            const float rstd = 1.0f / sqrtf(fmaxf(t[1] * invN - dm * dm, 0.f) + g.side_eps);
+            if (ok) {
+                float* so = g.side_out + (long long)b * g.side_sb + mo;
+#pragma unroll
+                for (int e = 0; e < 4; ++e)
+                    if (e < sn) so[e * g.side_sn] = g.side_alpha * (rstd * (t[2 + e] - dm * g.side_csum[e]) + g.side_bias[e]);
+            }
+        }
+    }
 }
 
 __global__ __launch_bounds__(256, 2) void gemm_as_dual_kernel(const AbxGemm g) {
@@ -875,6 +951,20 @@
     const int b = (int)(wgid / ntm), mt = (int)(wgid - (unsigned)b * ntm);
     if ((mt + 1) * AS_BM > g.M) as_dual_block<true>(g, lds, mt, b);
     else as_dual_block<false>(g, lds, mt, b);
+    probe.finish();
+}
+
+__global__ __launch_bounds__(256, 2) void gemm_as_dual_side_kernel(const AbxGemm g) {
+    extern __shared__ __attribute__((aligned(16))) float as_smem[];
+    char* lds = reinterpret_cast<char*>(as_smem);
+    const ClockProbe probe(g.clock_probe);
+    const unsigned ntm = (unsigned)((g.M + AS_BM - 1) / AS_BM);
+    const unsigned nwg = gridDim.x, bid = blockIdx.x;
+    const unsigned q = nwg >> 3, r = nwg & 7, xcd = bid & 7, loc = bid >> 3;
+    const unsigned wgid = (xcd < r ? xcd * (q + 1) : r * (q + 1) + (xcd - r) * q) + loc;
+    const int b = (int)(wgid / ntm), mt = (int)(wgid - (unsigned)b * ntm);
+    if ((mt + 1) * AS_BM > g.M) as_dual_block<true, true>(g, lds, mt, b);
+    else as_dual_block<false, true>(g, lds, mt, b);
     probe.finish();
 }
 
@@ -910,6 +1000,17 @@
     const long long ntm = ((long long)g.M + AS_BM - 1) / AS_BM;
     if (ntm * g.batch >= (1LL << 31)) return 1;
     if (!(g.tune & 16384) && ntm * g.batch < 1024) return 1;
+    if (g.side_out) {
+        if (g.side_rows != 0 && g.side_rows != rows_c) return 1;
+        if (g.side_n != 4 || !al16(g.side_Wt)) return 1;
+        if (int e = abx_ensure_dynamic_lds(reinterpret_cast<const void*>(&gemm_as_dual_side_kernel), AD_LDS_SIDE, "abx_gemm(as, dual, side)")) {
+            *rc = e;
+            return 0;
+        }
+        hipLaunchKernelGGL(gemm_as_dual_side_kernel, dim3((unsigned)(ntm * g.batch)), dim3(256), AD_LDS_SIDE, st, g);
+        *rc = abx_check_launch("abx_gemm(as, dual, side)");
+        return 0;
+    }
     if (int e = abx_ensure_dynamic_lds(reinterpret_cast<const void*>(&gemm_as_dual_kernel), AD_LDS, "abx_gemm(as, dual)")) {
         *rc = e;
         return 0;
diff --git a/abx_amd/csrc/gemm_epilogue.h b/abx_amd/csrc/gemm_epilogue.h
--- a/abx_amd/csrc/gemm_epilogue.h
+++ b/abx_amd/csrc/gemm_epilogue.h
@@ -2,11 +2,12 @@
 #include "common.h"
 #include "abx_hip.h"
 
-template <int BM, int BN, int WM, int WN, bool EDGE, bool TS, bool OLN = false, bool PROBE = true, int TGO = 0>
+template <int BM, int BN, int WM, int WN, bool EDGE, bool TS, bool OLN = false, bool PROBE = true, int TGO = 0, bool SIDEO = false>
 __device__ __forceinline__ void gemm_epilogue(const AbxGemm& g, const float* __restrict__ st_lds, float* __restrict__ scratch,
                                               f32x16 (&acc)[WM / 32][WN / 32], int m0, int n0, int b, bool stats,
                                               f32x16 (*acc2)[WM / 32][WN / 32] = nullptr, const float* __restrict__ st2_lds = nullptr,
-                                              const f32x16 (*gatev)[WM / 32][WN / 32] = nullptr) {
+                                              const f32x16 (*gatev)[WM / 32][WN / 32] = nullptr, float* side_part = nullptr,
+                                              float side_shift = 0.f, const float* side_w_lds = nullptr) {
     constexpr int TM = WM / 32, TN = WN / 32;
     constexpr int WAVES_N = BN / WN;
     const int lane = threadIdx.x & 63, wave = threadIdx.x >> 6;
@@ -43,7 +44,7 @@
         }
         return r;
     };
-    auto epi2_store = [&](f32x4 v, long long off_c, long long off_g, long long off_r, int cnt, int m_idx, int n_idx) {
+    auto epi2_store = [&](f32x4& v, long long off_c, long long off_g, long long off_r, int cnt, int m_idx, int n_idx) {
         if (gt) {
             f32x4 gv = load4(gt + off_g, g_vec, cnt);
             if (gsig) {
@@ -207,6 +208,31 @@
                         mo = (long long)pi * g.pair_L + pj;
                     }
                     epi2_store(v, mo * g.sCm + n, mo * g.sGm + n, mo * g.sRm + n, cnt, m, n);
+                    if constexpr (SIDEO) *reinterpret_cast<f32x4*>(&wsc[row * LW + c4 * 4]) = v;
+                }
+                if constexpr (SIDEO) {
+                    static_assert(TM == 1 && TN == TG && GW == 96 && WAVES_N == 1, "side output: one band, one column group of 96 per wave");
+                    __builtin_amdgcn_fence(__ATOMIC_RELEASE, "wavefront");
+                    __builtin_amdgcn_wave_barrier();
+                    const int srow = lane & 31, shalf = lane >> 5;
+                    const float* wrow = side_w_lds + (n0 + shalf * 48) * 4;
+                    f32x2 asq = {side_part[0], side_part[1]}, a01 = {side_part[2], side_part[3]}, a23 = {side_part[4], side_part[5]};
+#pragma unroll 4
+                    for (int k4 = 0; k4 < 12; ++k4) {
+                        const f32x4 x = *reinterpret_cast<const f32x4*>(&wsc[srow * LW + shalf * 48 + k4 * 4]);
+#pragma unroll
+                        for (int c = 0; c < 4; ++c) {
+                            const f32x4 w = *reinterpret_cast<const f32x4*>(wrow + (k4 * 4 + c) * 4);
+                            const float d = x[c] - side_shift;
+                            const f32x2 d2 = {d, d};
+                            asq = __builtin_elementwise_fma(d2, (f32x2){1.0f, d}, asq);
+                            a01 = __builtin_elementwise_fma(d2, (f32x2){w[0], w[1]}, a01);
+                            a23 = __builtin_elementwise_fma(d2, (f32x2){w[2], w[3]}, a23);
+                        }
+                    }
+                    side_part[0] = asq[0]; side_part[1] = asq[1];
+                    side_part[2] = a01[0]; side_part[3] = a01[1];
+                    side_part[4] = a23[0]; side_part[5] = a23[1];
                 }
                 __builtin_amdgcn_wave_barrier();
                 __builtin_amdgcn_fence(__ATOMIC_ACQUIRE, "wavefront");
diff --git a/abx_amd/model/forward.py b/abx_amd/model/forward.py
--- a/abx_amd/model/forward.py
+++ b/abx_amd/model/forward.py
@@ -397,12 +397,23 @@
         Lp = (L + 3) // 4 * 4
         LLp = L * Lp
         pad = (L, Lp) if Lp != L else None
+        ta_names = ('triangle_attention_starting_node', 'triangle_attention_ending_node')
+        ta_flagged = bool(P.exact_tags & ops.RANGE_TAGS['tri_attn'])
+        fold = (planes and not P.exact('tri_attn') and not (ops.GEMM_EXACT or ta_flagged) and not ops.KV_PLANES and ops._tri_bias_fold_ok(L)
+                and all(getattr(packs[n], '_row', None) is not None for n in ta_names))
+        if fold:
+            fold_bT = ops._tri_attn_block_bias(attn_ws, Bc, L) if self.block_api else ws.get('biasT', (Bc, 4, LL))
+            fold_pair = [packs[n]._keep[2] for n in ta_names]
         for name, outgoing in (('triangle_multiplication_outgoing', True), ('triangle_multiplication_incoming', False)):
             pre = P_BLK + name + '.'
             if blocks is not None and planes:
                 zb = w768.view(-1)[:Bc * LL * 192].view(Bc, LL, 192)
                 zin, zout = (z3, zb) if outgoing else (zb, z3)
-                ops.tri_mul_fwd(blocks[name], zin, zout, mask_f, Bc, L, outgoing, self._block_workspace('mul', Bc, L))
+                if fold and not outgoing:
+                    ops.tri_mul_fwd(blocks[name], zin, zout, mask_f, Bc, L, outgoing, self._block_workspace('mul', Bc, L),
+                                    next_pair=fold_pair[0], bias_out=fold_bT)
+                else:
+                    ops.tri_mul_fwd(blocks[name], zin, zout, mask_f, Bc, L, outgoing, self._block_workspace('mul', Bc, L))
                 continue
             GT = w768.view(-1)[:Bc * 256 * LL].view(Bc, 256, LL)
             Gf = w768.view(-1)[Bc * 256 * LL:Bc * 448 * LL].view(Bc, LL, 192)
@@ -422,8 +433,9 @@
                 tz = tt.as_strided((Bc * 128, L, L), (LLp, Lp, 1))
                 ops.gemm(lrp[:, 0:128], lrp[:, 128:256], tz, exact=2)
                 gw, gcs, gb, gw3 = P.ln_linear(pre + 'final_gate', pre + 'norm')
+                fp = fold_pair[0] if (fold and not outgoing) else None
                 _ln_lin(P, pre + 'proj_out', pre + 'final_norm', None, tt.transpose(1, 2), zout, resid=zin, pair=pad, c_pair=pad is not None,
-                        dual=(zin, gw3, gcs, gb))
+                        dual=(zin, gw3, gcs, gb), side=(fp.Wt, fp.csum, fp.bias, fold_bT, ops.TRI_BIAS_LOG2) if fp is not None else None)
             else:
                 _ln_lin(P, pre + 'final_gate', pre + 'norm', None, z3, Gf, act=2)
                 tt = w384[2 * Bc * 128 * LL:3 * Bc * 128 * LL].view(Bc, 128, LL)
@@ -448,7 +460,11 @@
             ax = P.exact('tri_attn')
             if blocks is not None:
                 flagged = bool(P.exact_tags & ops.RANGE_TAGS['tri_attn'])
-                ops.tri_attn_block_fwd(blocks[name], z2, mask_f, Bc, L, per_row, attn_ws, exact=ax, attn_exact=ops.GEMM_EXACT or flagged)
+                if fold:
+                    ops.tri_attn_block_fwd(blocks[name], z2, mask_f, Bc, L, per_row, attn_ws, exact=ax, attn_exact=ops.GEMM_EXACT or flagged,
+                                           bias_ready=True, next_pair=fold_pair[1] if per_row else None, next_bias_out=fold_bT if per_row else None)
+                else:
+                    ops.tri_attn_block_fwd(blocks[name], z2, mask_f, Bc, L, per_row, attn_ws, exact=ax, attn_exact=ops.GEMM_EXACT or flagged)
                 continue
             am = 1 if ax else 2
             ae = True if (P.exact_tags & ops.RANGE_TAGS['tri_attn']) else None
@@ -457,7 +473,9 @@
             bl2 = not (ops.GEMM_EXACT if ae is None else ae)
             kvp = ops.KV_PLANES and am == 2 and bl2 and ops.kv_planes_ok(M2)
             rowp = getattr(P.block_packs()[name], '_row', None) if (am == 2 and bl2 and not kvp) else None
-            if rowp is not None and ops._tri_rowfused_ok(L):
+            if fold:
+                assert rowp is not None
+            elif rowp is not None and ops._tri_rowfused_ok(L):
                 _ln_lin(P, pre + 'proj_pair', pre + 'norm', None, z3, bT.transpose(1, 2), narrow=True, exact=am, alpha=ops.TRI_BIAS_LOG2,
                         range_class='tri_attn')
             else:
@@ -478,7 +496,9 @@
             else:
                 ops.tri_attn(qkv, bT, mask_f, o, Bc, L, per_row, bias_is_qk=True, exact=ae, bias_log2=bl2, kv_planes=kvp)
             if not ax:
-                _ln_lin(P, pre + 'attn.gate', pre + 'norm', None, z2, z2, act=2, gate=o, resid=z2, mlp=P.mlp_second(pre + 'attn.proj_out'), exact=2)
+                fp = fold_pair[1] if (fold and per_row) else None
+                _ln_lin(P, pre + 'attn.gate', pre + 'norm', None, z2, z2, act=2, gate=o, resid=z2, mlp=P.mlp_second(pre + 'attn.proj_out'), exact=2,
+                        side=(fp.Wt, fp.csum, fp.bias, fold_bT, ops.TRI_BIAS_LOG2) if fp is not None else None)
             else:
                 hid = w768.view(-1)[M2 * 576:M2 * 768].view(M2, 192)
                 _ln_lin(P, pre + 'attn.gate', pre + 'norm', None, z2, hid, act=2, gate=o, gate_sigmoid=False, exact=1)
diff --git a/abx_amd/ops.py b/abx_amd/ops.py
--- a/abx_amd/ops.py
+++ b/abx_amd/ops.py
@@ -197,7 +197,7 @@
 
 def gemm(A, B, Cout, *, ln=None, a_relu=False, bias=None, alpha=1.0, act=0, rowscale=None, gate=None, gate_sigmoid=True,
          resid=None, tune=None, B3=None, exact=None, a_pair_transpose=0, glu=False, pair=None, a_pair=False, c_pair=False, dual=None, out_ln=None, clock_probe=None, mlp=None, c_split_nA=0, c_split_tile=False,
-         defer=False, range_class=None, c_plane_cols=None):
+         defer=False, range_class=None, c_plane_cols=None, side=None):
     lib = _lib.load()
     g = AbxGemm()
     a_planes, b_planes, c_planes = A.dtype == torch.int16, B.dtype == torch.int16, Cout.dtype == torch.int16
@@ -339,6 +339,14 @@
         cd, sd = (1, 2) if g.c_transposed else (2, 1)
         assert resid.shape == (nb, M if c_planes else Cout.shape[1], No if mlp is not None else N) and resid.stride(cd) == 1, 'resid must be laid out like Cout'
         g.resid, g.sRb, g.sRm = _p(_f32(resid)), (resid.stride(0) if nb > 1 else 0), resid.stride(sd)
+    if side is not None:
+        sWt, scs, sbi, sout, salpha = side
+        assert sWt.is_contiguous() and sWt.dim() == 2 and sout.dim() == 3 and sout.shape[1] == sWt.shape[1] and sout.stride(2) == 1
+        g.side_Wt, g.side_csum, g.side_bias = _p(_f32(sWt)), _p(_f32(scs)), _p(_f32(sbi))
+        g.side_eps, g.side_alpha, g.side_n = 1e-5, float(salpha), int(sWt.shape[1])
+        g.side_out, g.side_sb, g.side_sn, g.side_rows = _p(_f32(sout)), sout.stride(0), sout.stride(1), int(sout.shape[2])
+        if dual is not None:
+            g.tune |= 16384
     if defer:
         return g
     check(lib.abx_gemm(C.byref(g), _stream()), 'abx_gemm')
@@ -473,10 +481,15 @@
     check(_lib.load().abx_tri_mul_workspace_init(_p(ws), B, L, _stream()), 'abx_tri_mul_workspace_init')
 
 
-def tri_mul_fwd(pack, z_in, z_out, mask_f, B, L, outgoing, workspace):
+def tri_mul_fwd(pack, z_in, z_out, mask_f, B, L, outgoing, workspace, next_pair=None, bias_out=None):
     lib = _lib.load()
     assert z_in.is_contiguous() and z_out.is_contiguous() and z_in.data_ptr() != z_out.data_ptr()
     rf, rt = _range_args(False, 'contraction')
+    if next_pair is not None:
+        assert bias_out is not None and bias_out.is_contiguous() and bias_out.numel() == B * 4 * L * L
+        check(lib.abx_tri_mul_bias_fwd(C.byref(pack), _p(z_in), _p(z_out), _p(_f32(mask_f)), B, L, int(bool(outgoing)), _p(workspace),
+                                       C.byref(next_pair.c), _p(_f32(bias_out)), rf, rt, _stream()), 'abx_tri_mul_bias_fwd')
+        return z_out
     check(lib.abx_tri_mul_fwd(C.byref(pack), _p(z_in), _p(z_out), _p(_f32(mask_f)), B, L, int(bool(outgoing)), _p(workspace), rf, rt, _stream()),
           'abx_tri_mul_fwd')
     return z_out
@@ -510,14 +523,30 @@
     return ws[(-ws.data_ptr()) % 256:]
 
 
-def tri_attn_block_fwd(pack, z, mask_f, B, L, per_row, workspace, exact=False, attn_exact=None):
+def tri_attn_block_fwd(pack, z, mask_f, B, L, per_row, workspace, exact=False, attn_exact=None, bias_ready=False, next_pair=None, next_bias_out=None):
     lib = _lib.load()
     ax = bool(GEMM_EXACT if attn_exact is None else attn_exact)
     ex = int(bool(exact)) | (2 if ax else 0)
     rf, rt = _range_args(ex == 3, 'tri_attn')
+    if bias_ready or next_pair is not None:
+        assert next_pair is None or (next_bias_out is not None and next_bias_out.is_contiguous() and next_bias_out.numel() == B * 4 * L * L)
+        check(lib.abx_tri_attn_block_bias_fwd(C.byref(pack), _p(z), _p(_f32(mask_f)), B, L, int(bool(per_row)), ex, _p(workspace), int(bool(bias_ready)),
+                                              C.byref(next_pair.c) if next_pair is not None else None,
+                                              _p(_f32(next_bias_out)) if next_pair is not None else None, rf, rt, _stream()),
+              'abx_tri_attn_block_bias_fwd')
+        return z
     check(lib.abx_tri_attn_block_fwd(C.byref(pack), _p(z), _p(_f32(mask_f)), B, L, int(bool(per_row)), ex, _p(workspace), rf, rt, _stream()),
           'abx_tri_attn_block_fwd')
     return z
+
+
+def _tri_bias_fold_ok(L):
+    return bool(_lib.load().abx_tri_bias_fold_ok(int(L)))
+
+
+def _tri_attn_block_bias(workspace, B, L):
+    off = int(_lib.load().abx_tri_attn_block_bias_offset(B, L))
+    return workspace[off:off + 4 * B * 4 * L * L].view(torch.float32).view(B, 4, L * L)
 
 
 def _tri_rowfused_ok(L):
diff --git a/include/abx_hip.h b/include/abx_hip.h
--- a/include/abx_hip.h
+++ b/include/abx_hip.h
@@ -59,6 +59,10 @@
     unsigned long long* clock_probe;
     int a_vec_ok, b_vec_ok, fast_ok;
     int c_vec_ok, g_vec_ok, r_vec_ok, rs_vec_ok;
+    const float* side_Wt; const float* side_csum; const float* side_bias;
+    float side_eps, side_alpha;
+    int side_n;
+    float* side_out; long long side_sb, side_sn, side_rows;
 } AbxGemm;
 int abx_gemm(const AbxGemm* desc, hipStream_t stream);
 int abx_gemm_side(const AbxGemm* main_gemm, const AbxGemm* side_gemm, hipStream_t stream);
@@ -360,6 +364,15 @@
 int abx_tri_attn_block_fwd(const AbxTriAttnPack* w, float* z, const float* mask, int B, int L, int per_row, int exact, void* workspace,
                            int* range_flag, int range_tag, hipStream_t stream);
 
+int abx_tri_bias_fold_ok(int L);
+long long abx_tri_attn_block_bias_offset(int B, int L);
+int abx_tri_mul_bias_fwd(const AbxTriMulPack* w, const float* z_in, float* z_out, const float* mask, int B, int L, int outgoing,
+                         void* workspace, const AbxLinearPack* next_pair, float* bias_out, int* range_flag, int range_tag,
+                         hipStream_t stream);
+int abx_tri_attn_block_bias_fwd(const AbxTriAttnPack* w, float* z, const float* mask, int B, int L, int per_row, int exact, void* workspace,
+                                int bias_ready, const AbxLinearPack* next_pair, float* next_bias_out, int* range_flag, int range_tag,
+                                hipStream_t stream);
+
 #ifdef __cplusplus
 }
 #endif
```

Result: no change. 170.0 sample-steps/s, median of 6 (+0.6%).
